# lunarring/latentblending

Measured on AMD Instinct MI355X. Metric: transition frames/sec, SDXL-Turbo 512x512 4-step 15-branch, higher is better.
Workload: dtype f16; 1 GPU; SDXL-Turbo 512x512, num_inference_steps=4, nmb_max_branches=15 (17 frames/transition), fp16, fixed_seeds=[420,421], anchors not recycled; frontier_width=16, hipgraphs=True, parallelism=single GPU

## Files before the change

include/lb_hip.h:

```cpp
#ifndef LB_HIP_H
#define LB_HIP_H

#include <stdint.h>

#ifdef __cplusplus
extern "C" {
#endif

typedef uint16_t lb_half;

int lb_version(void);
const char* lb_last_error_string(void);
int lb_device_info(int device, int* cu_count, long* lds_per_cu, char* arch, int arch_len);

int lb_slerp_pairs_f16(const void* const* p0, const void* const* p1, void* const* out,
                       const double* fracts, int npairs, long n, void* stream);
int lb_slerp_pairs_f32(const void* const* p0, const void* const* p1, void* const* out,
                       const double* fracts, int npairs, long n, void* stream);
int lb_slerp_pairs_f64(const void* const* p0, const void* const* p1, void* const* out,
                       const double* fracts, int npairs, long n, void* stream);
int lb_slerp_batched_f16(const void* p0, const void* p1, void* out, const double* fracts_dev,
                         long npairs, long n, void* stream);
int lb_slerp_strided_f16(const void* p0, long stride0, const void* p1, long stride1, void* out,
                         const double* fracts_dev, long npairs, long n, void* stream);


int lb_lerp_f16(const void* p0, const void* p1, void* out, long n, double fract, void* stream);
int lb_lerp_f32(const void* p0, const void* p1, void* out, long n, double fract, void* stream);

int lb_scale_model_input_f16(const void* x, void* out, const float* params_dev, long per_sample,
                             int batch, int dup_for_cfg, void* stream);
int lb_euler_step_f16(const void* x, const void* eps, const void* noise, void* out,
                      const float* params_dev, long per_sample, int batch, int cfg, int ancestral,
                      void* stream);
int lb_ddim_step_f16(const void* x, const void* eps, void* out, const float* params_dev, long per_sample, int batch,
                     int cfg, void* stream);

enum {
    LB_GEMM_OUT_F32 = 1,
    LB_GEMM_RES_F32 = 2,
    LB_GEMM_GEGLU = 4,
    LB_GEMM_TRANS_OUT = 8,
    LB_GEMM_SILU = 16,
    LB_GEMM_RELU = 32,
    LB_GEMM_QUICK_GELU = 128,
    LB_GEMM_GELU = 256,
    LB_GEMM_CH_STATS = 512,
    LB_GEMM_HALO_RAGGED = 1024,
    LB_GEMM_HALO_KSPLIT = 4096,
    LB_GEMM_C64 = 2048,
    LB_GEMM_LN_A = 64
};

typedef struct LbGemmParams {
    const lb_half* A;
    const lb_half* W;
    void* C;
    const float* bias;
    const void* residual;
    const lb_half* rowvec;
    float* partial;
    int M, N, K;
    int lda, ldw, ldc, ldr, ld_rowvec, rows_per_batch;
    float alpha;
    int flags;
    int conv;
    int Hin, Win, Cin, Hout, Wout, KH, KW, stride, pad;
    int ups;
    int ldx;
    int splitk;
    const void* zero_page;
    int scatter, sc_py, sc_px, reserved_;
    const float* ln_colsum;
    float ln_eps;
    int reserved2_;
    float* ch_stats;
    int ch_stats_rows;
} LbGemmParams;

int lb_gemm_f16(const LbGemmParams* params, void* stream);
long lb_gemm_workspace_bytes(int M, int N);
void lb_gemm_set_tuning(int tile, int splitk);
void lb_gemm_set_pp_auto(int on);
void lb_gemm_pp_set_group(int gm);
void lb_gemm_set_depth(int depth);
int lb_gemm_plan(const LbGemmParams* p, int* tile, int* splitk, long* blocks);
int lb_conv3x3_halo_f16(const LbGemmParams* params, void* stream);
int lb_conv3x3_narrow_f16(const LbGemmParams* params, void* stream);
void lb_conv_halo_set_persistent(int on);
void lb_conv_halo_plan(const LbGemmParams* params, int* kind, int* tile_w, long* items, long* grid);
#include "lb_hip_ksplit.h"
int lb_gemm_ch_stat_rows(const LbGemmParams* params);
int lb_upconv2x_halo_f16(const LbGemmParams* params, void* stream);
void lb_gemm_set_halo(int mode);
void lb_gemm_set_wide_store(int on);
void lb_gemm_set_t192_waves8(int on);
void lb_gemm_set_kgroups(int on);
void lb_gemm_set_lean_epilogue(int on);
void lb_gemm_set_variant(int variant, int stages);

void lb_groupnorm_set_l3_chunk(long bytes);
int lb_groupnorm_from_stats(const void* x, void* y, const float* gamma, const float* beta, const float* ch_stats,
                            void* workspace, int B, int HW, int C, int ldx, int ldy, int groups, float eps, int silu,
                            int x_is_f32, int stat_rows_per_sample, void* stream);
long lb_groupnorm_workspace_bytes(int B, int groups);
int lb_groupnorm_nhwc(const void* x, void* y, const float* gamma, const float* beta, void* workspace,
                      int B, int HW, int C, int ldx, int ldy, int groups, float eps, int silu,
                      int x_is_f32, void* stream);
int lb_groupnorm_plan(int HW, int C, int groups, int x_is_f32);
void lb_groupnorm_set_fused(int on);
int lb_layernorm_f16(const void* x, void* y, const float* gamma, const float* beta, int M, int C,
                     int ldx, int ldy, float eps, void* stream);
void lb_layernorm_set_form(int form);

typedef struct LbAttnParams {
    const lb_half* Q;
    const lb_half* K;
    const lb_half* V;
    lb_half* O;
    int B, H, Sq, Skv, Skv_valid;
    int ldq, ldk, ldv, ldo;
    float scale;
    int causal;
    const void* zero_page;
    int reserved_;
} LbAttnParams;
int lb_attn_fwd_d64(const LbAttnParams* params, void* stream);
int lb_attn_fwd_d512(const LbAttnParams* params, void* stream);
void lb_attn_set_tuning(int force);
int lb_softmax_rows_f16(void* x, int M, int N, int ld, float scale, void* stream);

int lb_sinusoid_f16(const float* vals_dev, int rows, int per_row, int val_stride, int dim, void* out,
                    int ld_out, int col_off, void* stream);
int lb_copy_cols_f16(const void* src, void* dst, long rows, int cols, int ld_src, int ld_dst,
                     int dst_off, void* stream);
int lb_cast_f16_to_f32(const void* x, void* y, long n, void* stream);
int lb_cast_f32_to_f16(const void* x, void* y, long n, float mul, void* stream);
int lb_nchw_to_nhwc_f16(const void* x, void* y, int B, int C, int HW, int ld, float mul, void* stream);
int lb_nhwc_to_nchw_f16(const void* x, void* y, int B, int C, int HW, int ld, void* stream);
int lb_postprocess_u8(const void* x, void* out_u8, long pixels, int ld, int x_is_f32, void* stream);
int lb_lpips_prep_u8(const void* img_u8, void* out_f16, long pixels, void* stream);
int lb_maxpool3s2_nhwc_f16(const void* x, void* y, int N, int H, int W, int C, void* stream);
int lb_lpips_tap(const void* const* feats_a, const void* const* feats_b, const float* lin, float* acc,
                 float* workspace, int npairs, int HW, int C, void* stream);
int lb_fill_f32(void* x, long n, float v, void* stream);
int lb_embed_tokens_f16(const int* ids_dev, const void* tok_emb, const void* pos_emb, void* out, int rows, int seq, int C,
                        int vocab, void* stream);
int lb_gather_rows_f16(const void* src, const int* rows_idx_dev, void* out, int n, int C, int ld_src, void* stream);
int lb_frames_lerp_u8(const void* frames, const int* left_dev, const double* w_dev, void* out, long n_out,
                      long frame_bytes, void* stream);
int lb_copy_d2d(void* dst, const void* src, long bytes, void* stream);

int lb_jpeg_dct_quant_u8(const void* frames_u8, const void* qtables_u16, void* coef_i16, int n, int H, int W, int subsampling,
                         void* stream);
long lb_jpeg_coefficient_count(int n, int H, int W, int subsampling);
int lb_jpeg_entropy(const void* coef_i16, void* workspace, void* out, long out_capacity, void* frame_bytes_i32, int n, int H, int W,
                    int subsampling, void* stream);
long lb_jpeg_workspace_bytes(int n, int H, int W, int subsampling);

int lb_resample_u8(const void* src, void* tmp, void* dst, int n, int Hin, int Win, int Hout, int Wout,
                   const int* start_x, const int* count_x, const int* coef_x, int kmax_x,
                   const int* start_y, const int* count_y, const int* coef_y, int kmax_y, void* stream);

void* lb_program_create(void);
void lb_program_destroy(void* prog);
int lb_program_begin_record(void* prog);
int lb_program_end_record(void* prog);
int lb_program_recording(void);
int lb_program_num_ops(void* prog);
const char* lb_program_op_name(void* prog, int i);
int lb_program_run(void* prog, void* stream);
int lb_program_run_range(void* prog, int begin, int end, void* stream);
int lb_program_instantiate(void* prog);
int lb_program_launch(void* prog, void* stream);
int lb_program_time_ops(void* prog, void* stream, float* ms_out);

#ifdef LB_STUDY_BUILD
void lb_slerp_set_study(int variant);
void lb_conv_halo_set_study(int bits);
void lb_gemm_set_policy(int disable_mask);
#endif

#ifdef __cplusplus
}
#endif
#endif
```

latentblending_amd/csrc/conv3_halo.hip:

```cpp
#include <type_traits>
#include "lb_common.h"
#include "lb_gemm.h"

typedef __attribute__((address_space(1))) const void* gptr_t;
typedef __attribute__((address_space(3))) void* lptr_t;

#ifndef LB_HALO_LEAN_ADDR
#define LB_HALO_LEAN_ADDR 1
#endif

template <int N> __device__ __forceinline__ void halo_wait_barrier() {
    asm volatile("s_waitcnt vmcnt(%0)\n\ts_barrier" ::"n"(N) : "memory");
}

template <int KS, int J> struct HaloSched {
    static constexpr int tap = KS == 3 ? J : (J < 3 ? 0 : 1);
};
template <int KS, int NR, int TAP> constexpr int halo_full_rounds_in_tap() {
    int n = 0;
    for (int j = 0; j < NR - 1; ++j) n += ((KS == 3 ? j : (j < 3 ? 0 : 1)) == TAP) ? 1 : 0;
    return n;
}

template <int BN, int TW, int KS = 3, bool RAG = false, bool KSP = false>
__global__ void __launch_bounds__(512) conv3x3_halo_kernel(const LbGemmParams p) {
    static_assert(!RAG || KS == 3, "ragged tiles exist for the 3x3 form only");
    static_assert(!KSP || (KS == 3 && !RAG), "the K-split form exists for the whole-tile 3x3 form only");
    constexpr int TH = 256 / TW;
    constexpr int NTAP = KS * KS;
    constexpr int HWP = TW + KS - 1;
    constexpr int HR = (TH + KS - 1) * HWP;
    constexpr int HRG = (HR + 7) / 8;
    constexpr int HRP = HRG * 8;
    constexpr int NR = (HRG + 7) / 8;
    constexpr int EXTRA = HRG - 8 * (NR - 1);
    constexpr int WI = BN * 8 / 512;
    constexpr int TM = 4, TN = BN / 32;
    static_assert(NR == (KS == 3 ? 6 : 5), "halo rounds: 6 for the 3x3 form, 5 for the 2x2 form");
    static_assert(EXTRA >= 1 && EXTRA <= 8, "the last halo round is a partial one");
    static_assert(WI == 2, "the vmcnt schedule assumes two weight loads per thread and step");
    extern __shared__ __attribute__((aligned(16))) f16 lds[];
    f16* const halo0 = lds;
    f16* const wring = lds + 2 * HRP * 64;

    const int tid = threadIdx.x, lane = tid & 63;
    const int wave = LB_HALO_LEAN_ADDR ? __builtin_amdgcn_readfirstlane(tid >> 6) : tid >> 6;
    const int wave_m = wave >> 1, wave_n = wave & 1;
    const int g = lane >> 4, l16 = lane & 15;

    const int n_blocks = (p.N + BN - 1) / BN;
    const int tiles_x = RAG ? (p.Win + TW - 1) / TW : p.Win / TW, tiles_y = RAG ? (p.Hin + TH - 1) / TH : p.Hin / TH;
    const int n_items = (p.M / (p.Hin * p.Win)) * tiles_x * tiles_y * (KS == 2 ? 4 : 1) * n_blocks;
    const int G = gridDim.x;
    int bid = blockIdx.x;
    {
        const int q = G / 8, r = G % 8, xcd = bid % 8, idx = bid / 8;
        bid = (xcd < r ? xcd * (q + 1) : r * (q + 1) + (xcd - r) * q) + idx;
    }
    const int n_tiles = KSP ? n_items / n_blocks : 0;
    const long n_units = KSP ? (long)n_items * (p.Cin / 64) : 0;
    const long u_lo = KSP ? (long)bid * n_units / G : 0, u_hi = KSP ? (long)(bid + 1) * n_units / G : 0;
    if constexpr (KSP)
        if (u_lo >= u_hi) return;
    const int first_item = KSP ? (int)(u_lo / (p.Cin / 64)) : bid;
    const int block_n = KSP ? first_item / n_tiles : bid % n_blocks;
    const int par_x = KS == 2 ? (bid / n_blocks) & 1 : 0;
    const int par_y = KS == 2 ? ((bid / n_blocks) >> 1) & 1 : 0;
    int n0 = block_n * BN;
    const int org_y = KS == 3 ? 1 : 1 - par_y, org_x = KS == 3 ? 1 : 1 - par_x;
    const lb_half* Wp = p.W + (KS == 2 ? (long)(par_y * 2 + par_x) * p.N * p.ldw : 0);
    const int nchunks = p.Cin / 64;
    const lb_half* zero = reinterpret_cast<const lb_half*>(p.zero_page);

    struct TileAt { int b, y0, x0; };
    auto tile_of = [&](int item) {
        int tile = KSP ? item % n_tiles : item / n_blocks;
        if (KS == 2) tile >>= 2;
        TileAt t;
        t.x0 = (tile % tiles_x) * TW;
        tile /= tiles_x;
        t.y0 = (tile % tiles_y) * TH;
        t.b = tile / tiles_y;
        return t;
    };

    const int r8 = lane >> 3;
    const int cl = (lane & 7) ^ r8;
    long h_off[NR];
    auto set_halo_offsets = [&](const TileAt& t, bool exists) {
#pragma unroll
        for (int j = 0; j < NR; ++j) {
            const int gidx = j * 8 + wave;
            const int row = gidx * 8 + r8;
            const int hy = row / HWP, hx = row - hy * HWP;
            const int y = t.y0 + hy - org_y, x = t.x0 + hx - org_x;
            const bool ok = exists && (j < NR - 1 || wave < EXTRA) && row < HR && y >= 0 && y < p.Hin && x >= 0 && x < p.Win;
            h_off[j] = ok ? ((long)(t.b * p.Hin + y) * p.Win + x) * p.ldx + cl * 8 : -1;
        }
    };
    long w_off[WI], w_offn[WI];
    unsigned w_off32[WI], w_off32n[WI];
    auto set_w_offsets = [&](int col_base, long (&o64)[WI], unsigned (&o32)[WI]) {
#pragma unroll
        for (int i = 0; i < WI; ++i) {
            const int n = col_base + (tid >> 3) + i * 64;
            o64[i] = n < p.N ? (long)n * p.ldw + cl * 8 : -1;
            o32[i] = (unsigned)(((long)(n < p.N ? n : p.N - 1) * p.ldw + cl * 8) * 2);
        }
    };
    set_w_offsets(n0, w_off, w_off32);
    if constexpr (KSP) set_w_offsets(n0, w_offn, w_off32n);

#ifdef LB_STUDY_BUILD
    const int study = p.reserved_;
#else
    constexpr int study = 0;
#endif
    auto issue_halo = [&](int j, int src_chunk, int buf) {
        const lb_half* src = h_off[j] >= 0 && !(study & 2) ? p.A + h_off[j] + (long)src_chunk * 64 : zero;
        const int gidx = j * 8 + wave;
        f16* dst = halo0 + buf * (HRP * 64) + gidx * 8 * 64;
        __builtin_amdgcn_global_load_lds((gptr_t)src, (lptr_t)dst, 16, 0, 0);
    };
    auto issue_weight = [&](int i, int chunk, bool exists, int tap, int slot, bool nxt_slab = false) {
        f16* dst = wring + slot * (BN * 64) + (wave * 8 + i * 64) * 64;
        if constexpr (LB_HALO_LEAN_ADDR) {
            if (!(study & 4)) {
                const char* base = reinterpret_cast<const char*>(Wp) + ((long)tap * p.Cin + (long)chunk * 64) * 2;
                const unsigned o32 = KSP && nxt_slab ? w_off32n[i] : w_off32[i];
                __builtin_amdgcn_global_load_lds((gptr_t)(base + (size_t)o32), (lptr_t)dst, 16, 0, 0);
                return;
            }
        }
        const long o64 = KSP && nxt_slab ? w_offn[i] : w_off[i];
        const bool live = o64 >= 0 && exists && !(study & 4);
        const lb_half* src = live ? Wp + o64 + (long)tap * p.Cin + (long)chunk * 64 : zero;
        __builtin_amdgcn_global_load_lds((gptr_t)src, (lptr_t)dst, 16, 0, 0);
    };

    int hbase[TM];
    int mloc[TM];
#pragma unroll
    for (int i = 0; i < TM; ++i) {
        const int m = wave_m * 64 + i * 16 + l16;
        const int py = m / TW, px = m - py * TW;
        hbase[i] = py * HWP + px;
        mloc[i] = py * p.Win + px;
    }
    f32x4 acc[TM][TN];
#pragma unroll
    for (int i = 0; i < TM; ++i)
#pragma unroll
        for (int j = 0; j < TN; ++j) acc[i][j] = (f32x4){0.f, 0.f, 0.f, 0.f};

    auto read_frags = [&](const f16* hb, const f16* wb, int shift, int s, f16x8 (&af)[TM], f16x8 (&wf)[TN]) {
        const int chunk = s * 4 + g;
        if constexpr (LB_HALO_LEAN_ADDR && TW == 32) {
            static_assert(TM == 4, "pairs (0, 1) and (2, 3)");
#pragma unroll
            for (int i = 0; i < TM; i += 2) {
                const int r = hbase[i] + shift;
                const f16* a = hb + r * 64 + ((chunk ^ (r & 7)) << 3);
                af[i] = *reinterpret_cast<const f16x8*>(a);
                af[i + 1] = *reinterpret_cast<const f16x8*>(a + 16 * 64);
            }
        } else {
#pragma unroll
            for (int i = 0; i < TM; ++i) {
                const int r = hbase[i] + shift;
                af[i] = *reinterpret_cast<const f16x8*>(hb + r * 64 + ((chunk ^ (r & 7)) << 3));
            }
        }
#pragma unroll
        for (int j = 0; j < TN; ++j) {
            const int r = j * 16 + l16;
            wf[j] = *reinterpret_cast<const f16x8*>(wb + (wave_n * (BN / 2) + r) * 64 + ((chunk ^ (r & 7)) << 3));
        }
    };
    auto mma_rows = [&](const f16x8 (&af)[TM], const f16x8 (&wf)[TN], int i_lo, int i_hi) {
#pragma unroll
        for (int i = i_lo; i < i_hi; ++i)
#pragma unroll
            for (int j = 0; j < TN; ++j)
                acc[i][j] = __builtin_amdgcn_mfma_f32_16x16x32_f16(wf[j], af[i], acc[i][j], 0, 0, 0);
    };

    int item = first_item;
    int c_lo = 0, c_end = nchunks;
    if constexpr (KSP) {
        c_lo = (int)(u_lo - (long)item * nchunks);
        c_end = (int)(u_hi - (long)item * nchunks < nchunks ? u_hi - (long)item * nchunks : nchunks);
    }
    TileAt cur = tile_of(item);
    set_halo_offsets(cur, true);
#pragma unroll
    for (int j = 0; j < NR; ++j)
        if (j < NR - 1 || wave < EXTRA) issue_halo(j, c_lo, 0);
#pragma unroll
    for (int t = 0; t < 3; ++t)
#pragma unroll
        for (int i = 0; i < WI; ++i) issue_weight(i, c_lo, true, t, t);

    auto step = [&](auto tap_c, int c, int cc, bool more) {
        constexpr int TAP = decltype(tap_c)::value;
        constexpr int P1 = (TAP + NTAP - 1) % NTAP, P2 = (TAP + NTAP - 2) % NTAP;
        constexpr int CNT = (2 + halo_full_rounds_in_tap<KS, NR, P1>()) + (2 + halo_full_rounds_in_tap<KS, NR, P2>());
        halo_wait_barrier<CNT>();
        const int slot = KS == 3 ? ((cc + TAP) & 3) : TAP;
        const f16* hb = halo0 + (cc & 1) * (HRP * 64);
        const f16* wb = wring + slot * (BN * 64);
        constexpr int KY = TAP / KS, KX = TAP % KS;
        int shift = KY * HWP + KX;
        asm volatile("" : "+v"(shift));
        const bool last = c + 1 == c_end;
        const int hc = last ? 0 : c + 1, hbuf = (cc + 1) & 1;
        constexpr int TAP3 = (TAP + 3) % NTAP;
        const bool wrap = (TAP + 3 >= NTAP) && last;
        const int c3 = wrap ? 0 : c + (TAP + 3) / NTAP;
        const bool w_exists = !wrap || more;
        const int slot3 = (slot + 3) & 3;
        f16x8 a0[TM], w0[TN], a1[TM], w1[TN];
        read_frags(hb, wb, shift, 0, a0, w0);
        if constexpr (HaloSched<KS, 0>::tap == TAP) issue_halo(0, hc, hbuf);
        if constexpr (NR > 2 && HaloSched<KS, 1>::tap == TAP) issue_halo(1, hc, hbuf);
        if constexpr (NR > 3 && HaloSched<KS, 2>::tap == TAP) issue_halo(2, hc, hbuf);
        if constexpr (NR > 4 && HaloSched<KS, 3>::tap == TAP) { if (NR - 1 > 3 || wave < EXTRA) issue_halo(3, hc, hbuf); }
        if constexpr (NR > 4 && HaloSched<KS, 4>::tap == TAP) { if (NR - 1 > 4 || wave < EXTRA) issue_halo(4, hc, hbuf); }
        if constexpr (NR > 5 && HaloSched<KS, 5>::tap == TAP) { if (wave < EXTRA) issue_halo(5, hc, hbuf); }
        __builtin_amdgcn_sched_barrier(0);
        mma_rows(a0, w0, 0, TM / 2);
        read_frags(hb, wb, shift, 1, a1, w1);
        __builtin_amdgcn_sched_barrier(0);
        issue_weight(0, c3, w_exists, TAP3, slot3, wrap);
        __builtin_amdgcn_sched_barrier(0);
        mma_rows(a0, w0, TM / 2, TM);
        __builtin_amdgcn_sched_barrier(0);
        issue_weight(1, c3, w_exists, TAP3, slot3, wrap);
        __builtin_amdgcn_sched_barrier(0);
        mma_rows(a1, w1, 0, TM);
    };

    LbGemmParams q = p;
    if constexpr (KS == 2) {
        q.scatter = 1;
        q.sc_py = par_y;
        q.sc_px = par_x;
    }

    int cc = 0;
    for (;;) {
        const int next_item = KSP ? item + 1 : item + G;
        const bool more = KSP ? (long)next_item * nchunks < u_hi : next_item < n_items;
        const TileAt nxt = tile_of(more ? next_item : item);
        const int n0_next = KSP && more ? (next_item / n_tiles) * BN : n0;
        for (int c = c_lo; c < c_end; ++c, ++cc) {
            if (c + 1 == c_end) {
                set_halo_offsets(nxt, more);
                if constexpr (KSP) set_w_offsets(n0_next, w_offn, w_off32n);
            }
            step(std::integral_constant<int, 0>{}, c, cc, more);
            step(std::integral_constant<int, 1>{}, c, cc, more);
            step(std::integral_constant<int, 2>{}, c, cc, more);
            step(std::integral_constant<int, 3>{}, c, cc, more);
            if constexpr (KS == 3) {
                step(std::integral_constant<int, 4>{}, c, cc, more);
                step(std::integral_constant<int, 5>{}, c, cc, more);
                step(std::integral_constant<int, 6>{}, c, cc, more);
                step(std::integral_constant<int, 7>{}, c, cc, more);
                step(std::integral_constant<int, 8>{}, c, cc, more);
            }
        }
        if constexpr (KSP) {
            if (c_lo != 0 || c_end != nchunks) {
                const long t0 = (long)item * nchunks;
                const int b_first = (int)(((t0 + 1) * G - 1) / n_units), b_last = (int)(((t0 + nchunks) * G - 1) / n_units);
                constexpr long SLAB = 256l * BN;
                int* const counters = reinterpret_cast<int*>(p.partial);
                float* const slabs = p.partial + (((long)n_items * 4 + 255) / 256) * 64;
                int tid_s = tid;
                asm volatile("" : "+v"(tid_s));
                typedef unsigned u32x4 __attribute__((ext_vector_type(4)));
                const __amdgpu_buffer_rsrc_t srs = __builtin_amdgcn_make_buffer_rsrc(slabs, 0, (int)(unsigned)(2l * G * SLAB * 4), 0x00020000);
                const int voff = tid_s * 16;
                const int mine = (2 * bid + (item == first_item ? 0 : 1)) * (int)(SLAB * 4);
#pragma unroll
                for (int i = 0; i < TM; ++i)
#pragma unroll
                    for (int j = 0; j < TN; ++j)
                        __builtin_amdgcn_raw_buffer_store_b128(__builtin_bit_cast(u32x4, acc[i][j]), srs, voff, mine + (i * TN + j) * 8192, 16);
                volatile int* const flag = reinterpret_cast<volatile int*>(lds + 2 * HRP * 64 + 4 * BN * 64);
                asm volatile("s_waitcnt vmcnt(0)" ::: "memory");
                __syncthreads();
                if (tid == 0) {
                    const int ticket = __hip_atomic_fetch_add(counters + item, 1, __ATOMIC_RELAXED, __HIP_MEMORY_SCOPE_AGENT);
                    const bool last_one = ticket == b_last - b_first;
                    if (last_one) __hip_atomic_store(counters + item, 0, __ATOMIC_RELAXED, __HIP_MEMORY_SCOPE_AGENT);
                    *flag = last_one ? 1 : 0;
                }
                __syncthreads();
                const bool reduce = __builtin_amdgcn_readfirstlane(*flag) != 0;
                if (!reduce) {
                    if (!more) break;
#pragma unroll
                    for (int i = 0; i < TM; ++i)
#pragma unroll
                        for (int j = 0; j < TN; ++j) acc[i][j] = (f32x4){0.f, 0.f, 0.f, 0.f};
                    item = next_item;
                    cur = nxt;
                    n0 = n0_next;
                    set_w_offsets(n0, w_off, w_off32);
                    c_lo = 0;
                    c_end = (int)(u_hi - (long)item * nchunks < nchunks ? u_hi - (long)item * nchunks : nchunks);
                    continue;
                }
#pragma unroll
                for (int i = 0; i < TM; ++i)
#pragma unroll
                    for (int j = 0; j < TN; ++j) acc[i][j] = (f32x4){0.f, 0.f, 0.f, 0.f};
                for (int b = b_first; b <= b_last; ++b) {
                    const bool first_tile_of_b = (long)b * n_units / G / nchunks == item;
                    const int src = (2 * b + (first_tile_of_b ? 0 : 1)) * (int)(SLAB * 4);
#pragma unroll
                    for (int i = 0; i < TM; ++i) {
                        f32x4 part[TN];
#pragma unroll
                        for (int j = 0; j < TN; ++j)
                            part[j] = __builtin_bit_cast(f32x4, __builtin_amdgcn_raw_buffer_load_b128(srs, voff, src + (i * TN + j) * 8192, 16));
#pragma unroll
                        for (int j = 0; j < TN; ++j) acc[i][j] += part[j];
                    }
                }
            }
        }
        const int mbase = (cur.b * p.Hin + cur.y0) * p.Win + cur.x0;
        int col0 = n0 + wave_n * (BN / 2) + 4 * g;
        asm volatile("" : "+v"(col0));
        bool overhang = false;
        if constexpr (RAG) overhang = cur.y0 + TH > p.Hin || cur.x0 + TW > p.Win;
        if (RAG && overhang && !(study & 1)) {
            int tid_o = tid;
            asm volatile("" : "+v"(tid_o));
            auto row_of = [&](int i) {
                const int ml = (tid_o >> 7) * 64 + i * 16 + (tid_o & 15), ly = ml / TW, lx = ml - ly * TW;
                return cur.y0 + ly < p.Hin && cur.x0 + lx < p.Win ? mbase + mloc[i] : p.M;
            };
            if (p.flags & LB_GEMM_CH_STATS) {
                const long stat_rows = (long)(n_items / n_blocks) * 4;
                float2* chst = reinterpret_cast<float2*>(p.ch_stats) + ((long)(KSP ? item % n_tiles : item / n_blocks) * 4 + wave_m);
                lb_gemm_tile_epilogue_rows_ln<TM, TN, false, false, true, true>(q, acc, row_of, col0, 0, (const LbLnRows<TM>*)nullptr, chst, stat_rows);
            } else {
                lb_gemm_tile_epilogue_rows<TM, TN, false>(q, acc, row_of, col0, 0);
            }
        } else if (!(study & 1)) {
            int tid_o = tid;
            asm volatile("" : "+v"(tid_o));
            auto out_rel = [&](int i) {
                if constexpr (KS == 3) return mloc[i];
                const int ml = (tid_o >> 7) * 64 + i * 16 + (tid_o & 15), ly = ml / TW, lx = ml - ly * TW;
                return 4 * ly * p.Win + 2 * lx;
            };
            const long out_lo = KS == 3 ? (long)mbase
                                        : ((long)(cur.b * 2 * p.Hin + 2 * cur.y0 + par_y)) * (2 * p.Win) + 2 * cur.x0 + par_x;
            const int row_hi = mbase + (TH - 1) * p.Win + TW;
            const int colw = col0 - 4 * ((tid_o & 63) >> 4);
            if (p.flags & LB_GEMM_CH_STATS) {
                const long stat_rows = (long)(n_items / n_blocks) * 4;
                float2* chst = reinterpret_cast<float2*>(p.ch_stats) + ((long)(KSP ? item % n_tiles : item / n_blocks) * 4 + wave_m);
                if (!lb_gemm_tile_epilogue_lean<TM, TN, true, true>(q, acc, [&](int i) { return mbase + mloc[i]; }, mbase, row_hi, out_rel,
                                                                    out_lo, cur.b, colw, chst, stat_rows))
                    lb_gemm_tile_epilogue_rows_ln<TM, TN, false, false, true>(q, acc, [&](int i) { return mbase + mloc[i]; }, col0, 0,
                                                                              (const LbLnRows<TM>*)nullptr, chst, stat_rows);
            } else {
                if (!lb_gemm_tile_epilogue_lean<TM, TN, false, true>(q, acc, [&](int i) { return mbase + mloc[i]; }, mbase, row_hi, out_rel,
                                                                     out_lo, cur.b, colw))
                    lb_gemm_tile_epilogue_rows<TM, TN, false>(q, acc, [&](int i) { return mbase + mloc[i]; }, col0, 0);
            }
        }
        else if (acc[0][0][0] == 12345.678f) *(float*)p.C = acc[1][1][1] + acc[2][2][2] + acc[3][3][3];
        if (!more) break;
#pragma unroll
        for (int i = 0; i < TM; ++i)
#pragma unroll
            for (int j = 0; j < TN; ++j) acc[i][j] = (f32x4){0.f, 0.f, 0.f, 0.f};
        item = next_item;
        cur = nxt;
        if constexpr (KSP) {
            n0 = n0_next;
            set_w_offsets(n0, w_off, w_off32);
            c_lo = 0;
            c_end = (int)(u_hi - (long)item * nchunks < nchunks ? u_hi - (long)item * nchunks : nchunks);
        }
    }
    asm volatile("s_waitcnt vmcnt(0)" ::: "memory");
}

static int g_halo_persistent = 1;
extern "C" void lb_conv_halo_set_persistent(int on) { g_halo_persistent = on; }
#ifdef LB_STUDY_BUILD
static int g_halo_study = 0;
extern "C" void lb_conv_halo_set_study(int bits) { g_halo_study = bits; }
#endif
static int halo_num_cus() {
    static int n = 0;
    if (!n) {
        int dev = 0;
        hipDeviceProp_t prop;
        n = (hipGetDevice(&dev) == hipSuccess && hipGetDeviceProperties(&prop, dev) == hipSuccess && prop.multiProcessorCount > 0)
                ? prop.multiProcessorCount : 256;
    }
    return n;
}

static void halo_grid(const LbGemmParams& p, int tw, int ks, long& items, long& grid) {
    const int th = 256 / tw;
    const long tiles = (long)(p.M / (p.Hin * p.Win)) * ((p.Hin + th - 1) / th) * ((p.Win + tw - 1) / tw) * (ks == 2 ? 4 : 1);
    const int n_blocks = (p.N + 127) / 128;
    items = tiles * n_blocks;
    const int period = n_blocks * (ks == 2 ? 4 : 1);
    grid = items;
    if (g_halo_persistent && period <= halo_num_cus() && items > halo_num_cus())
        grid = (long)(halo_num_cus() / period) * period;
}

int lb_upconv_halo_eligible(const LbGemmParams& p);
int lb_conv3x3_halo_eligible(const LbGemmParams& p);
long lb_conv_halo_stat_rows_total(const LbGemmParams& p) {
    int tw = 0, ks = 0;
    if ((tw = lb_upconv_halo_eligible(p)) != 0) ks = 2;
    else if ((tw = lb_conv3x3_halo_eligible(p)) != 0) ks = 3;
    if (!ks) return 0;
    long items, grid;
    halo_grid(p, tw, ks, items, grid);
    return items / ((p.N + 127) / 128) * 4;
}

template <int BN, int TW, int KS = 3, bool RAG = false, bool KSP = false>
static int launch_halo(const LbGemmParams& p, hipStream_t stream, long ksp_grid = 0) {
    constexpr int TH = 256 / TW;
    constexpr int HRP = (((TH + KS - 1) * (TW + KS - 1) + 7) / 8) * 8;
    constexpr int SMEM = (2 * HRP * 64 + 4 * BN * 64) * (int)sizeof(f16) + (KSP ? 16 : 0);
    static unsigned long long seen = 0;
    LB_ONCE_PER_DEVICE(seen)
        (void)hipFuncSetAttribute(reinterpret_cast<const void*>(conv3x3_halo_kernel<BN, TW, KS, RAG, KSP>),
                                  hipFuncAttributeMaxDynamicSharedMemorySize, SMEM);
    static_assert(BN == 128, "halo_grid assumes 128-channel blocks");
    long nblk, grid;
    halo_grid(p, TW, KS, nblk, grid);
    if (KSP) grid = ksp_grid;
    LbGemmParams pk = p;
#ifdef LB_STUDY_BUILD
    pk.reserved_ = g_halo_study;
#endif
    hipLaunchKernelGGL((conv3x3_halo_kernel<BN, TW, KS, RAG, KSP>), dim3((unsigned)grid), dim3(512), SMEM, stream, pk);
    return lb_check_launch(KS == 2 ? "lb_upconv2x_halo_f16" : "lb_conv3x3_halo_f16");
}

int lb_upconv_halo_eligible(const LbGemmParams& p) {
    if (!p.conv || p.scatter != 2 || p.KH != 2 || p.KW != 2 || p.stride != 1 || p.ups) return 0;
    if (p.Hout != p.Hin || p.Wout != p.Win || p.Cin % 64 != 0 || p.K != 4 * p.Cin) return 0;
    if (p.zero_page == nullptr || (p.flags & (LB_GEMM_GEGLU | LB_GEMM_TRANS_OUT)) || p.N % 4 != 0 || p.residual != nullptr) return 0;
    if (p.M % (p.Hin * p.Win) != 0) return 0;
    if ((long)p.N * p.ldw * 2 >= (1l << 32)) return 0;
    if (p.Win % 32 == 0 && p.Hin % 8 == 0) return 32;
    if (p.Win % 16 == 0 && p.Hin % 16 == 0) return 16;
    return 0;
}

static int halo_tiles_check(const LbGemmParams& p, int tw, int ks) {
    long items, grid;
    halo_grid(p, tw, ks, items, grid);
    LB_REQUIRE(items < (1l << 30), "halo conv: too many tiles for one launch");
    return 0;
}

int lb_upconv_halo_check(const LbGemmParams& p) {
    LB_REQUIRE(!(p.flags & LB_GEMM_CH_STATS) || (p.ch_stats != nullptr && p.ch_stats_rows == lb_conv_halo_stat_rows_total(p)),
               "halo upconv: LB_GEMM_CH_STATS needs ch_stats with ch_stats_rows = B * lb_gemm_ch_stat_rows()");
    return halo_tiles_check(p, lb_upconv_halo_eligible(p), 2);
}

int lb_upconv_halo_launch(LbGemmParams p, hipStream_t stream) {
    if (p.alpha == 0.f) p.alpha = 1.f;
    p.splitk = 1;
    return lb_upconv_halo_eligible(p) == 32 ? launch_halo<128, 32, 2>(p, stream) : launch_halo<128, 16, 2>(p, stream);
}

extern int g_lb_wide_store, g_lb_lean_epilogue;
extern "C" int lb_upconv2x_halo_f16(const LbGemmParams* pp, void* stream) {
    LbGemmParams p = *pp;
    p.flags &= ~LB_GEMM_C64;
    p.reserved2_ = (g_lb_wide_store & 1) | (g_lb_lean_epilogue ? 2 : 0);
    LB_REQUIRE(p.M > 0 && p.N > 0 && p.K > 0, "lb_upconv2x_halo_f16: empty problem");
    LB_REQUIRE(lb_upconv_halo_eligible(p) != 0,
               "lb_upconv2x_halo_f16: needs scatter = 2, KH = KW = 2, stride 1, Cin % 64 == 0, W % 16 == 0, zero page, no residual");
    LB_REQUIRE(p.ldw % 8 == 0 && p.ldx % 8 == 0 && p.ldc % 4 == 0, "lb_upconv2x_halo_f16: ldw / ldx multiples of 8, ldc multiple of 4");
    if (const int rc = lb_upconv_halo_check(p)) return rc;
    LB_DISPATCH("lb_upconv2x_halo_f16", lb_upconv_halo_launch(p, s));
}

int lb_conv3x3_halo_eligible(const LbGemmParams& p) {
    if (!p.conv || p.KH != 3 || p.KW != 3 || p.stride != 1 || p.pad != 1 || p.ups || p.scatter) return 0;
    if (p.Hout != p.Hin || p.Wout != p.Win || p.Cin % 64 != 0 || p.K != 9 * p.Cin) return 0;
    if (p.zero_page == nullptr || (p.flags & LB_GEMM_GEGLU) || p.N % 4 != 0) return 0;
    if (p.M % (p.Hin * p.Win) != 0) return 0;
    if ((long)p.N * p.ldw * 2 >= (1l << 32)) return 0;
    if (p.Win % 32 == 0 && p.Hin % 8 == 0) return 32;
    if (p.Win % 16 == 0 && p.Hin % 16 == 0) return 16;
    if (!(p.flags & LB_GEMM_HALO_RAGGED)) return 0;
    const long t32 = (long)((p.Win + 31) / 32) * ((p.Hin + 7) / 8), t16 = (long)((p.Win + 15) / 16) * ((p.Hin + 15) / 16);
    return t16 < t32 ? 16 : 32;
}
static bool halo3_ragged(const LbGemmParams& p, int tw) { return p.Win % tw != 0 || p.Hin % (256 / tw) != 0; }

static int g_halo_ksplit_mode = 1, g_halo_ksplit_grid = 0;
extern "C" void lb_conv_halo_set_ksplit(int mode, int grid) {
    g_halo_ksplit_mode = mode < 0 ? 1 : mode;
    g_halo_ksplit_grid = grid > 0 ? grid : 0;
}
static constexpr long HALO_KSPLIT_FIXUP_STEPS = 20;
static constexpr long HALO_KSPLIT_MARGIN_PCT = 5;
static void halo_ksplit_plan(const LbGemmParams& p, long& units, long& grid, int& split) {
    units = grid = 0;
    split = 0;
    if (!(p.flags & LB_GEMM_HALO_KSPLIT) || (p.flags & LB_GEMM_C64) || g_halo_ksplit_mode == 0) return;
    const int tw = lb_conv3x3_halo_eligible(p);
    if (!tw || halo3_ragged(p, tw) || p.Cin < 128) return;
    long items, ugrid;
    halo_grid(p, tw, 3, items, ugrid);
    const long nchunks = p.Cin / 64;
    if (items * nchunks >= (1l << 31)) return;
    units = items * nchunks;
    grid = g_halo_ksplit_grid > 0 ? g_halo_ksplit_grid : halo_num_cus();
    if (grid > units) grid = units;
    if (2 * grid * 256l * 128 * 4 >= (1l << 31)) {
        units = grid = 0;
        return;
    }
    if (g_halo_ksplit_mode >= 2) {
        split = 1;
        return;
    }
    const long unsplit_steps = (items + ugrid - 1) / ugrid * 9 * nchunks;
    const long split_steps = (units + grid - 1) / grid * 9 + HALO_KSPLIT_FIXUP_STEPS;
    split = split_steps * (100 + HALO_KSPLIT_MARGIN_PCT) <= unsplit_steps * 100 ? 1 : 0;
}
static long halo_ksplit_counter_bytes(long items) { return (items * 4 + 255) / 256 * 256; }
extern "C" void lb_conv_halo_ksplit_plan(const LbGemmParams* pp, long* units, long* grid, int* split) {
    long u = 0, g = 0;
    int s = 0;
    if (pp != nullptr && pp->M > 0 && pp->Hin > 0 && pp->Win > 0) halo_ksplit_plan(*pp, u, g, s);
    if (units) *units = u;
    if (grid) *grid = g;
    if (split) *split = s;
}
extern "C" long lb_conv_halo_ksplit_workspace_bytes(const LbGemmParams* pp) {
    long u = 0, g = 0;
    int s = 0;
    if (pp != nullptr && pp->M > 0 && pp->Hin > 0 && pp->Win > 0) halo_ksplit_plan(*pp, u, g, s);
    if (!s) return 0;
    return halo_ksplit_counter_bytes(u / (pp->Cin / 64)) + 2 * g * 256l * 128 * (long)sizeof(float);
}

long lb_conv3x3_halo_blocks(const LbGemmParams& p) {
    long tiles = (long)p.M / 256;
    if (const int tw = (p.flags & LB_GEMM_HALO_RAGGED) ? lb_conv3x3_halo_eligible(p) : 0)
        tiles = (long)(p.M / (p.Hin * p.Win)) * ((p.Hin + 256 / tw - 1) / (256 / tw)) * ((p.Win + tw - 1) / tw);
    return tiles * ((p.N + 127) / 128);
}

int lb_conv3x3_halo_check(const LbGemmParams& p) {
    LB_REQUIRE(!(p.flags & LB_GEMM_CH_STATS) || (p.ch_stats != nullptr && !(p.flags & LB_GEMM_TRANS_OUT)),
               "halo conv: LB_GEMM_CH_STATS needs ch_stats and a row-major output");
    LB_REQUIRE(!(p.flags & LB_GEMM_CH_STATS) || p.ch_stats_rows == lb_conv_halo_stat_rows_total(p),
               "halo conv: ch_stats_rows must be B * lb_gemm_ch_stat_rows() (the row blocks this launch writes per channel)");
    {
        long units, grid;
        int split;
        halo_ksplit_plan(p, units, grid, split);
        LB_REQUIRE(!split || p.partial != nullptr,
                   "halo conv: LB_GEMM_HALO_KSPLIT needs partial = a zeroed workspace of lb_conv_halo_ksplit_workspace_bytes()");
    }
    return halo_tiles_check(p, lb_conv3x3_halo_eligible(p), 3);
}

int lb_conv3x3_halo_launch(LbGemmParams p, hipStream_t stream) {
    if (p.alpha == 0.f) p.alpha = 1.f;
    p.splitk = 1;
    const int tw = lb_conv3x3_halo_eligible(p);
    if (halo3_ragged(p, tw)) return tw == 32 ? launch_halo<128, 32, 3, true>(p, stream) : launch_halo<128, 16, 3, true>(p, stream);
    long units, grid;
    int split;
    halo_ksplit_plan(p, units, grid, split);
    if (split && p.partial != nullptr)
        return tw == 32 ? launch_halo<128, 32, 3, false, true>(p, stream, grid) : launch_halo<128, 16, 3, false, true>(p, stream, grid);
    return tw == 32 ? launch_halo<128, 32>(p, stream) : launch_halo<128, 16>(p, stream);
}

extern "C" int lb_conv3x3_halo_f16(const LbGemmParams* pp, void* stream) {
    LbGemmParams p = *pp;
    p.flags &= ~LB_GEMM_C64;
    p.reserved2_ = (g_lb_wide_store & 1) | (g_lb_lean_epilogue ? 2 : 0);
    LB_REQUIRE(p.M > 0 && p.N > 0 && p.K > 0, "lb_conv3x3_halo_f16: empty problem");
    LB_REQUIRE(lb_conv3x3_halo_eligible(p) != 0,
               "lb_conv3x3_halo_f16: needs a 3x3 / stride 1 / pad 1 conv, Cin % 64 == 0, W % 16 == 0 (or LB_GEMM_HALO_RAGGED), zero page");
    LB_REQUIRE(p.ldw % 8 == 0 && p.ldx % 8 == 0 && (p.ldc % 4 == 0 || (p.flags & LB_GEMM_TRANS_OUT)),
               "lb_conv3x3_halo_f16: ldw / ldx multiples of 8, ldc multiple of 4");
    if (const int rc = lb_conv3x3_halo_check(p)) return rc;
    LB_DISPATCH("lb_conv3x3_halo_f16", lb_conv3x3_halo_launch(p, s));
}

extern "C" void lb_conv_halo_plan(const LbGemmParams* pp, int* kind, int* tile_w, long* items, long* grid) {
    LbGemmParams p = *pp;
    int k = 0, tw = 0;
    if (p.flags & LB_GEMM_C64) tw = 0;
    else if ((tw = lb_upconv_halo_eligible(p)) != 0) k = 2;
    else if ((tw = lb_conv3x3_halo_eligible(p)) != 0) k = 3;
    long it = 0, gr = 0;
    if (k) halo_grid(p, tw, k, it, gr);
    if (kind) *kind = k;
    if (tile_w) *tile_w = tw;
    if (items) *items = it;
    if (grid) *grid = gr;
}
```

latentblending_amd/csrc/conv3_narrow.hip:

```cpp
#include "lb_common.h"
#include "lb_gemm.h"

typedef __attribute__((address_space(1))) const void* gptr_t;
typedef __attribute__((address_space(3))) void* lptr_t;

#define NARROW_T 16
#define NARROW_HW (NARROW_T + 2)
#define NARROW_HR (NARROW_HW * NARROW_HW)
#define NARROW_HRG ((NARROW_HR + 7) / 8)
#define NARROW_LDS (NARROW_HRG * 8 * 64)

__global__ void __launch_bounds__(256, 2) conv3x3_narrow_kernel(const LbGemmParams p) {
    __shared__ __attribute__((aligned(16))) f16 halo[NARROW_LDS];
    const int tid = threadIdx.x, lane = tid & 63, wave = tid >> 6;
    const int g = lane >> 4, l16 = lane & 15;
    const int tiles_x = p.Win / NARROW_T, tiles_y = p.Hin / NARROW_T;
    int tile = blockIdx.x;
    const int x0 = (tile % tiles_x) * NARROW_T;
    tile /= tiles_x;
    const int y0 = (tile % tiles_y) * NARROW_T;
    const int b = tile / tiles_y;
    const lb_half* zero = reinterpret_cast<const lb_half*>(p.zero_page);
    const int nchunks = p.Cin / 64;

    constexpr int NR = (NARROW_HRG + 3) / 4;
    const int r8 = lane >> 3, cl = (lane & 7) ^ r8;
    int h_off[NR];
#pragma unroll
    for (int j = 0; j < NR; ++j) {
        const int gidx = j * 4 + wave;
        const int row = gidx * 8 + r8;
        const int hy = row / NARROW_HW, hx = row - hy * NARROW_HW;
        const int y = y0 + hy - 1, x = x0 + hx - 1;
        const bool ok = gidx < NARROW_HRG && row < NARROW_HR && y >= 0 && y < p.Hin && x >= 0 && x < p.Win;
        h_off[j] = ok ? (int)((((long)(b * p.Hin + y) * p.Win + x) * p.ldx >> 3) + cl) : -1;
    }
    const bool n_ok = l16 < p.N;
    const lb_half* wrow = p.W + (long)(n_ok ? l16 : 0) * p.ldw + g * 8;

    f32x4 acc[4];
#pragma unroll
    for (int i = 0; i < 4; ++i) acc[i] = (f32x4){0.f, 0.f, 0.f, 0.f};
    int hbase[4];
#pragma unroll
    for (int i = 0; i < 4; ++i) hbase[i] = (wave * 4 + i) * NARROW_HW + l16;

    const f16x8 zero8 = {0, 0, 0, 0, 0, 0, 0, 0};
    for (int c = 0; c < nchunks; ++c) {
        if (c) __syncthreads();
#pragma unroll
        for (int j = 0; j < NR; ++j) {
            const int gidx = j * 4 + wave;
            if (gidx < NARROW_HRG) {
                const lb_half* src = h_off[j] >= 0 ? p.A + (long)h_off[j] * 8 + (long)c * 64 : zero;
                __builtin_amdgcn_global_load_lds((gptr_t)src, (lptr_t)(halo + gidx * 8 * 64), 16, 0, 0);
            }
        }
        f16x8 wf[9][2];
#pragma unroll
        for (int tap = 0; tap < 9; ++tap)
#pragma unroll
            for (int s = 0; s < 2; ++s)
                wf[tap][s] = n_ok ? *reinterpret_cast<const f16x8*>(wrow + (long)tap * p.Cin + c * 64 + s * 32) : zero8;
        asm volatile("s_waitcnt vmcnt(0)" ::: "memory");
        __syncthreads();
#pragma unroll
        for (int tap = 0; tap < 9; ++tap) {
            const int shift = (tap / 3) * NARROW_HW + tap % 3;
#pragma unroll
            for (int s = 0; s < 2; ++s) {
                const int chunk = s * 4 + g;
#pragma unroll
                for (int i = 0; i < 4; ++i) {
                    const int r = hbase[i] + shift;
                    const f16x8 af = *reinterpret_cast<const f16x8*>(halo + r * 64 + ((chunk ^ (r & 7)) << 3));
                    acc[i] = __builtin_amdgcn_mfma_f32_16x16x32_f16(wf[tap][s], af, acc[i], 0, 0, 0);
                }
            }
        }
    }
    const int n = 4 * g;
    if (n < p.N) {
        f32x4 bias = {0.f, 0.f, 0.f, 0.f};
        if (p.bias) bias = *reinterpret_cast<const f32x4*>(p.bias + n);
#pragma unroll
        for (int i = 0; i < 4; ++i) {
            const long m = ((long)(b * p.Hin + y0 + wave * 4 + i)) * p.Win + x0 + l16;
            float o[4];
#pragma unroll
            for (int r = 0; r < 4; ++r) o[r] = acc[i][r] * p.alpha + bias[r];
            if (p.flags & LB_GEMM_OUT_F32)
                *reinterpret_cast<f32x4*>((float*)p.C + m * p.ldc + n) = (f32x4){o[0], o[1], o[2], o[3]};
            else
                *reinterpret_cast<f16x4*>((f16*)p.C + m * p.ldc + n) = (f16x4){(f16)o[0], (f16)o[1], (f16)o[2], (f16)o[3]};
        }
    }
}

int lb_conv3x3_narrow_eligible(const LbGemmParams& p) {
    if (!p.conv || p.KH != 3 || p.KW != 3 || p.stride != 1 || p.pad != 1 || p.ups || p.scatter) return 0;
    if (p.Hout != p.Hin || p.Wout != p.Win || p.Cin % 64 != 0 || p.K != 9 * p.Cin) return 0;
    if (p.N > 16 || p.N % 4 != 0 || p.zero_page == nullptr) return 0;
    if (p.flags & ~(LB_GEMM_OUT_F32 | LB_GEMM_HALO_KSPLIT)) return 0;
    if (p.residual != nullptr || p.rowvec != nullptr) return 0;
    if (p.Win % NARROW_T != 0 || p.Hin % NARROW_T != 0 || p.M % (p.Hin * p.Win) != 0) return 0;
    if ((long)p.M * p.ldx >= (1l << 34)) return 0;
    return 1;
}

static long narrow_tiles(const LbGemmParams& p) {
    return (long)(p.M / (p.Hin * p.Win)) * (p.Hin / NARROW_T) * (p.Win / NARROW_T);
}

int lb_conv3x3_narrow_check(const LbGemmParams& p) {
    LB_REQUIRE(narrow_tiles(p) < (1l << 31), "conv3x3 narrow: too many tiles for one launch");
    return 0;
}

int lb_conv3x3_narrow_launch(LbGemmParams p, hipStream_t stream) {
    if (p.alpha == 0.f) p.alpha = 1.f;
    const long tiles = narrow_tiles(p);
    hipLaunchKernelGGL(conv3x3_narrow_kernel, dim3((unsigned)tiles), dim3(256), 0, stream, p);
    return lb_check_launch("lb_conv3x3_narrow_f16");
}

extern "C" int lb_conv3x3_narrow_f16(const LbGemmParams* pp, void* stream) {
    LbGemmParams p = *pp;
    p.flags &= ~LB_GEMM_C64;
    LB_REQUIRE(p.M > 0 && p.N > 0 && p.K > 0, "lb_conv3x3_narrow_f16: empty problem");
    LB_REQUIRE(lb_conv3x3_narrow_eligible(p) != 0,
               "lb_conv3x3_narrow_f16: needs a 3x3 / stride 1 / pad 1 conv, N <= 16, Cin % 64 == 0, H and W multiples of 16, bias-only epilogue");
    LB_REQUIRE(p.ldw % 8 == 0 && p.ldx % 8 == 0 && p.ldc % 4 == 0, "lb_conv3x3_narrow_f16: ldw / ldx multiples of 8, ldc multiple of 4");
    if (const int rc = lb_conv3x3_narrow_check(p)) return rc;
    LB_DISPATCH("lb_conv3x3_narrow_f16", lb_conv3x3_narrow_launch(p, s));
}
```

latentblending_amd/csrc/gemm.hip:

```cpp
#include "lb_common.h"
#include "lb_gemm.h"

#define BK 64

template <int N> struct Int { static constexpr int value = N; };

template <int BM, int BN, bool CONV, bool GEGLU, int D>
__global__ void __launch_bounds__(256) gemm_f16_kernel(const LbGemmParams p) {
    constexpr int AI = BM * 8 / 256;
    constexpr int WI = BN * 8 / 256;
    constexpr int TM = BM / 32;
    constexpr int TN = BN / 32;
    __shared__ __attribute__((aligned(16))) f16 lds[2 * (BM + BN) * BK];
    f16* const As = lds;
    f16* const Ws = lds + 2 * BM * BK;

    const int tid = threadIdx.x;
    const int lane = tid & 63, wave = tid >> 6;
    const int wave_m = wave >> 1, wave_n = wave & 1;
    const int g = lane >> 4, l16 = lane & 15;

    const int n_blocks = GEGLU ? (p.N / 2 + BN / 2 - 1) / (BN / 2) : (p.N + BN - 1) / BN;
    int bid = blockIdx.x;
    {
// ... 297 lines not shown
    switch (depth) {
        case 1: launch_variant<BM, BN, 1>(p, grid, stream); break;
        case 2: launch_variant<BM, BN, 2>(p, grid, stream); break;
        case 3: launch_variant<BM, BN, 3>(p, grid, stream); break;
        default: launch_variant<BM, BN, 4>(p, grid, stream); break;
    }
}

static int default_depth(const LbGemmParams& p, int tile) {
    if (tile == 1) return p.conv ? 1 : 3;
    if (tile == 2) return 3;
    return 4;
}

static int gemm_launch_impl(LbGemmParams p, int tile, int depth, int variant, int stages, dim3 grid,
                            hipStream_t stream) {
    if (tile == 9) {
        lb_gemm_launch_pp(p, grid, stream);
    } else if (variant == 1 && p.zero_page != nullptr) {
        lb_gemm_launch_glds(p, tile, stages, grid, stream);
    } else {
        if (depth <= 0) depth = default_depth(p, tile);
        if (tile == 1) launch_depth<128, 128>(p, depth, grid, stream);
        else if (tile == 2) launch_depth<128, 64>(p, depth, grid, stream);
        else launch_depth<64, 64>(p, depth, grid, stream);
    }
    int rc = lb_check_launch("lb_gemm_f16");
    if (rc) return rc;
    if (p.splitk > 1) {
        const long quads = (long)p.M * (p.N / 4);
        long gsz = (quads + 255) / 256;
        if (gsz > 2048) gsz = 2048;
        hipLaunchKernelGGL(gemm_splitk_reduce_kernel, dim3((unsigned)gsz), dim3(256), 0, stream, p);
        rc = lb_check_launch("lb_gemm_f16(split-K reduce)");
    }
    return rc;
}

static void gemm_plan(const LbGemmParams& p, int& tile_out, int& splitk_out, long& nblk_out) {
    const bool geglu = (p.flags & LB_GEMM_GEGLU) != 0;
    const int n_eff = geglu ? p.N / 2 : p.N;

    auto blocks = [&](int bm, int bn) {
        const int bn_eff = geglu ? bn / 2 : bn;
        return (long)((p.M + bm - 1) / bm) * ((n_eff + bn_eff - 1) / bn_eff);
    };
    int tile = g_force_tile;
    if (tile == 9 && !lb_gemm_pp_eligible(p)) tile = 0;
    if (!tile) {
        const long b128 = blocks(128, 128);
        tile = b128 >= 700 ? 1 : (b128 >= 224 ? (g_variant == 1 ? 2 : 1) : 3);
        if (n_eff <= 64) tile = 3;
        if (g_variant == 1 && p.zero_page != nullptr) {
            const long b256 = blocks(256, 128);
            const int unit = geglu ? 64 : 128;
            const int n_pad = (n_eff + unit - 1) / unit * unit;
            const bool n_fits = (long)n_pad * 10 <= (long)n_eff * 11;
            const bool allow4 = !(g_policy_off & 1) && !(p.conv && (g_policy_off & 16));
            const bool allow5 = !(g_policy_off & 2) && !(p.conv ? (g_policy_off & 4) : (g_policy_off & 8));
            if (allow4 && n_fits && (b256 >= 1024 || (!p.conv && b256 >= 160 && p.K >= 1024))) tile = 4;
            const long b512 = blocks(256, 256);
            const long rounds4 = (b256 + 255) / 256, rounds5 = (b512 + 255) / 256;
            if (allow5 && (b512 >= 1024 || (b512 >= 160 && p.K >= 1024)) && rounds5 * 174 < rounds4 * 100) tile = 5;
            if ((g_policy_off & 32) && !geglu && !p.conv && (tile == 4 || tile == 5) && n_fits) {
                const long b192 = blocks(192, 128);
                const long rounds7 = (b192 + 255) / 256;
                const long cur = tile == 5 ? rounds5 * 174 : rounds4 * 100;
                if (b192 >= 160 && rounds7 * 78 < cur) tile = g_t192_waves8 ? 10 : 7;
            }
            if (!(g_policy_off & 64) && !geglu && !p.conv && tile == 4 && n_fits && b256 < 224) {
                const long b192 = blocks(192, 128);
                if (b192 <= 256 && b192 * 10 >= b256 * 13) tile = g_t192_waves8 ? 10 : 7;
            }
        }
    }
    if (!g_force_tile && g_t192_waves8 && geglu && !p.conv && (tile == 1 || tile == 2 || tile == 4) && p.M <= 2048 && g_variant == 1 &&
        p.zero_page != nullptr && blocks(192, 128) <= 448 && p.K >= 512)
        tile = 10;
    if (tile >= 4 && tile != 9 && (g_variant != 1 || p.zero_page == nullptr)) tile = 1;
    if (!g_force_tile && g_pp_auto && lb_gemm_pp_eligible(p)) {
        const int bn_out = geglu ? 128 : 256;
        const long n_pad = (long)((n_eff + bn_out - 1) / bn_out) * bn_out;
        const long b9 = blocks(256, 256);
        if (b9 >= 192 && (p.K >= 1024 || b9 >= 1024) && n_pad * 4 <= (long)n_eff * 5) tile = 9;
    }
    if (!g_force_tile && tile == 3 && !geglu && p.partial != nullptr && (p.K + BK - 1) / BK >= 64) {
        const long b64 = blocks(64, 64);
        if (b64 > 256 && b64 <= 640 && blocks(128, 64) <= 256) tile = 2;
    }
    const int bm = (tile == 7 || tile == 10) ? 192 : (tile == 11 ? 64 : (tile >= 4 ? 256 : (tile == 3 ? 64 : 128)));
    const int bn = (tile == 5 || tile == 9) ? 256 : ((tile == 1 || tile == 4 || tile == 7 || tile == 10) ? 128 : 64);
    const long nblk = blocks(bm, bn);
    int splitk = 1;
    if (!geglu && p.partial != nullptr && !(p.flags & LB_GEMM_LN_A)) {
        const int k_tiles = (p.K + BK - 1) / BK;
        if (g_force_splitk) splitk = g_force_splitk;
        else if (nblk <= 256) {
            splitk = (int)((640 + nblk - 1) / nblk);
            const int max_by_k = k_tiles / 16 > 0 ? k_tiles / 16 : 1;
            if (splitk > max_by_k) splitk = max_by_k;
            if (splitk > 16) splitk = 16;
        }
        if (splitk > k_tiles) splitk = k_tiles;
        if (splitk < 1) splitk = 1;
        if (tile == 9 && !g_force_splitk) splitk = 1;
        if (tile >= 4 && tile != 11 && !g_force_splitk) splitk = 1;
    }
    if (!g_force_tile && g_kgroups && tile == 3 && splitk == 1 && !p.conv && g_variant == 1 && p.zero_page != nullptr && nblk <= 200 &&
        (p.K + BK - 1) / BK >= 8)
        tile = 11;
    tile_out = tile;
    splitk_out = splitk;
    nblk_out = nblk;
}

extern "C" int lb_gemm_plan(const LbGemmParams* pp, int* tile, int* splitk, long* blocks) {
    LB_REQUIRE(pp != nullptr && pp->M > 0 && pp->N > 0 && pp->K > 0, "lb_gemm_plan: empty problem");
    int t = 0, sk = 1;
    long nb = 0;
    if (pp->flags & LB_GEMM_C64) {
        if (const int rc = lb_conv3_c64_check(*pp)) return rc;
        long items = 0;
        t = 12;
        lb_conv3_c64_grid(*pp, items, nb);
    }
    else if (g_halo != 0 && !g_force_tile && lb_conv3x3_narrow_eligible(*pp)) { t = 8; nb = (long)pp->M / 256; }
    else if (use_halo(*pp)) { t = 6; nb = lb_conv3x3_halo_blocks(*pp); }
    else if (pp->flags & LB_GEMM_HALO_KSPLIT) {
        LbGemmParams q = *pp;
        q.flags &= ~LB_GEMM_HALO_KSPLIT;
        q.partial = nullptr;
        gemm_plan(q, t, sk, nb);
    }
    else gemm_plan(*pp, t, sk, nb);
    if (tile) *tile = t;
    if (splitk) *splitk = sk;
    if (blocks) *blocks = nb;
    return 0;
}

long lb_conv_halo_stat_rows_total(const LbGemmParams& p);
extern "C" int lb_gemm_ch_stat_rows(const LbGemmParams* pp) {
    if (pp == nullptr || !pp->conv || pp->M <= 0 || pp->Hout <= 0 || pp->Wout <= 0) return 0;
    if (pp->flags & LB_GEMM_C64) return 0;
    const LbGemmParams& p = *pp;
    bool halo;
    if (p.scatter == 2) halo = lb_upconv_halo_eligible(p) != 0;
    else halo = !(g_halo != 0 && !g_force_tile && lb_conv3x3_narrow_eligible(p)) && use_halo(p);
    if (!halo) return 0;
    const long samples = (long)p.M / ((long)p.Hout * p.Wout);
    return samples > 0 ? (int)(lb_conv_halo_stat_rows_total(p) / samples) : 0;
}

extern "C" int lb_gemm_f16(const LbGemmParams* pp, void* stream) {
    LbGemmParams p = *pp;
    const bool geglu = (p.flags & LB_GEMM_GEGLU) != 0;
    LB_REQUIRE(p.M > 0 && p.N > 0 && p.K > 0, "lb_gemm_f16: empty problem");
    LB_REQUIRE(p.K % 8 == 0 && p.ldw % 8 == 0, "lb_gemm_f16: K and ldw must be multiples of 8");
    LB_REQUIRE(p.N % 4 == 0 && (geglu ? p.N % 8 == 0 : true), "lb_gemm_f16: N must be a multiple of 4");
    LB_REQUIRE(p.ldc % 4 == 0 || (p.flags & LB_GEMM_TRANS_OUT), "lb_gemm_f16: ldc must be a multiple of 4");
    if (p.conv) {
        LB_REQUIRE(p.Cin % 8 == 0 && p.ldx % 8 == 0, "lb_gemm_f16: conv Cin/ldx must be multiples of 8");
        LB_REQUIRE(p.K == p.KH * p.KW * p.Cin, "lb_gemm_f16: conv K != KH*KW*Cin");
        LB_REQUIRE(p.M % (p.Hout * p.Wout) == 0, "lb_gemm_f16: conv M must be B*Hout*Wout");
        if (p.scatter)
            LB_REQUIRE(p.KH == 2 && p.KW == 2 && p.stride == 1 && p.ups == 0 && p.Hout == p.Hin && p.Wout == p.Win &&
                           !(p.flags & (LB_GEMM_TRANS_OUT | LB_GEMM_GEGLU)) && p.residual == nullptr,
                       "lb_gemm_f16: sub-pixel conv needs KH=KW=2, stride 1, Hout=Hin, no residual");
    } else {
        LB_REQUIRE(p.lda % 8 == 0, "lb_gemm_f16: lda must be a multiple of 8");
    }
    if (p.flags & LB_GEMM_LN_A) {
        LB_REQUIRE(!p.conv && p.ln_colsum != nullptr && p.zero_page != nullptr && g_variant == 1,
                   "lb_gemm_f16: LB_GEMM_LN_A needs a plain / GEGLU GEMM of the direct-to-LDS family with ln_colsum");
        LB_REQUIRE(p.lda >= p.K && !(p.flags & LB_GEMM_TRANS_OUT), "lb_gemm_f16: LB_GEMM_LN_A normalises whole rows of A");
    }
    if (p.alpha == 0.f) p.alpha = 1.f;
    p.reserved2_ = (g_lb_wide_store & 1) | (g_lb_lean_epilogue ? 2 : 0);
    if (p.flags & LB_GEMM_C64) {
        if (const int rc = lb_conv3_c64_check(p)) return rc;
        LB_DISPATCH("conv3x3_c64", lb_conv3_c64_launch(p, s));
    }
    if (p.scatter == 2) {
        LB_REQUIRE(lb_upconv_halo_eligible(p) != 0, "lb_gemm_f16: scatter = 2 needs Cin % 64 == 0, W % 16 == 0, stacked [4][N][K] weights");
        if (const int rc = lb_upconv_halo_check(p)) return rc;
        LB_DISPATCH("lb_upconv2x_halo_f16", lb_upconv_halo_launch(p, s));
    }
    if (g_halo != 0 && !g_force_tile && lb_conv3x3_narrow_eligible(p)) {
        if (const int rc = lb_conv3x3_narrow_check(p)) return rc;
        LB_DISPATCH("lb_conv3x3_narrow_f16", lb_conv3x3_narrow_launch(p, s));
    }
    if (use_halo(p)) {
        if (const int rc = lb_conv3x3_halo_check(p)) return rc;
        LB_DISPATCH("lb_conv3x3_halo_f16", lb_conv3x3_halo_launch(p, s));
    }
    if (p.flags & LB_GEMM_HALO_KSPLIT) {
        p.flags &= ~LB_GEMM_HALO_KSPLIT;
        p.partial = nullptr;
    }
    LB_REQUIRE(!(p.flags & LB_GEMM_CH_STATS), "lb_gemm_f16: LB_GEMM_CH_STATS is implemented by the halo-tile conv kernels only "
                                              "(check lb_gemm_plan == 6 / lb_conv_halo_plan before asking for it)");
    int tile = 0, splitk = 1;
    long nblk = 0;
    gemm_plan(p, tile, splitk, nblk);
    p.splitk = splitk;
    const int depth = g_depth, variant = g_variant;
    int stages = g_stages;
    if (variant == 1) {
        lb_gemm_glds_init();
        if (stages == 0)
            stages = (tile == 3 || tile == 4 || tile == 7 || tile == 10 || tile == 11) ? 3 : 2;
    }
    const dim3 grid((unsigned)nblk, 1, (unsigned)splitk);
    LB_DISPATCH("lb_gemm_f16", gemm_launch_impl(p, tile, depth, variant, stages, grid, s));
}
```

latentblending_amd/csrc/lb_common.h:

```cpp
#pragma once
#include <hip/hip_runtime.h>
#include <hip/hip_fp16.h>
#include <stdint.h>

#define LB_WAVE 64

typedef _Float16 f16;
typedef f16 f16x4 __attribute__((ext_vector_type(4)));
typedef f16 f16x8 __attribute__((ext_vector_type(8)));
typedef float f32x4 __attribute__((ext_vector_type(4)));

extern "C" const char* lb_last_error_string(void);
void lb_set_error(const char* what, hipError_t e);

#ifdef __cplusplus
#include <functional>
#include <mutex>
bool lb_recording();
void lb_record(const char* name, std::function<int(hipStream_t)> fn);
#define LB_DISPATCH(NAME, CALL)                                                   \
    do {                                                                          \
        if (lb_recording()) {                                                     \
            lb_record(NAME, [=](hipStream_t s) -> int { return CALL; });          \
            return 0;                                                             \
        }                                                                         \
        hipStream_t s = (hipStream_t)stream;                                      \
        return CALL;                                                              \
    } while (0)
#define LB_DISPATCH_STMT(NAME, STMT) \
    LB_DISPATCH(NAME, ([&]() -> int { STMT; return lb_check_launch(NAME); })())
#endif

static inline int lb_check_launch(const char* what) {
    hipError_t e = hipGetLastError();
    if (e != hipSuccess) lb_set_error(what, e);
    return (int)e;
}

struct LbFirstCallOnDevice {
    std::unique_lock<std::mutex> lock;
    bool first;
    explicit LbFirstCallOnDevice(unsigned long long& seen) : lock(mutex()) {
        int dev = 0;
        (void)hipGetDevice(&dev);
        const unsigned long long bit = 1ull << (dev & 63);
        first = (seen & bit) == 0;
        seen |= bit;
    }
    static std::mutex& mutex() {
        static std::mutex m;
        return m;
    }
};
#define LB_ONCE_PER_DEVICE(seen) if (LbFirstCallOnDevice lb_once_guard_{seen}; lb_once_guard_.first)

#define LB_REQUIRE(cond, what)                                   \
    do {                                                         \
        if (!(cond)) {                                           \
            lb_set_error(what, hipErrorInvalidValue);            \
            return (int)hipErrorInvalidValue;                    \
        }                                                        \
    } while (0)

__device__ __forceinline__ float lb_wave_sum(float v) {
#pragma unroll
    for (int off = 32; off > 0; off >>= 1) v += __shfl_xor(v, off, LB_WAVE);
    return v;
}

__device__ __forceinline__ float lb_wave_sum_dpp(float v) {
    {
        const unsigned u = __float_as_uint(v);
        const auto r = __builtin_amdgcn_permlane32_swap(u, u, false, false);
        v = __uint_as_float(r[0]) + __uint_as_float(r[1]);
    }
    {
        const unsigned u = __float_as_uint(v);
        const auto r = __builtin_amdgcn_permlane16_swap(u, u, false, false);
        v = __uint_as_float(r[0]) + __uint_as_float(r[1]);
    }
    v += __uint_as_float(__builtin_amdgcn_update_dpp(0u, __float_as_uint(v), 0x128, 0xf, 0xf, false));
    v += __uint_as_float(__builtin_amdgcn_update_dpp(0u, __float_as_uint(v), 0x124, 0xf, 0xf, false));
    v += __uint_as_float(__builtin_amdgcn_update_dpp(0u, __float_as_uint(v), 0x4e, 0xf, 0xf, false));
    v += __uint_as_float(__builtin_amdgcn_update_dpp(0u, __float_as_uint(v), 0xb1, 0xf, 0xf, false));
    return v;
}

__device__ __forceinline__ double lb_wave_sum(double v) {
#pragma unroll
    for (int off = 32; off > 0; off >>= 1) v += __shfl_xor(v, off, LB_WAVE);
    return v;
}

__device__ __forceinline__ float lb_wave_max(float v) {
#pragma unroll
    for (int off = 32; off > 0; off >>= 1) v = fmaxf(v, __shfl_xor(v, off, LB_WAVE));
    return v;
}

__device__ __forceinline__ f16 lb_f64_to_f16(double x) {
    const float f = (float)x;
    const double r = x - (double)f;
    unsigned u = __float_as_uint(f);
    const bool finite_nz = (u & 0x7fffffffu) - 1u < 0x7f7fffffu;
    if (finite_nz && r != 0.0) {
        if ((r < 0.0) != (f < 0.0f)) u -= 1u;
        u |= 1u;
    }
    return (f16)__uint_as_float(u);
}

__device__ __forceinline__ float lb_silu(float x) {
    return x * __builtin_amdgcn_rcpf(1.0f + __builtin_amdgcn_exp2f(x * -1.44269504088896340736f));
}

__device__ __forceinline__ float lb_erf(float x) {
    const float ax = __builtin_fabsf(x);
    const float t = __builtin_amdgcn_rcpf(__builtin_fmaf(0.3275911f, ax, 1.0f));
    float p = __builtin_fmaf(1.061405429f, t, -1.453152027f);
    p = __builtin_fmaf(p, t, 1.421413741f);
    p = __builtin_fmaf(p, t, -0.284496736f);
    p = __builtin_fmaf(p, t, 0.254829592f);
    const float e = __builtin_amdgcn_exp2f(ax * ax * -1.44269504088896340736f);
    const float r = __builtin_fmaf(-p * t, e, 1.0f);
    return __builtin_copysignf(r, x);
}

__device__ __forceinline__ float lb_quick_gelu(float x) {
    return x * __builtin_amdgcn_rcpf(1.0f + __builtin_amdgcn_exp2f(x * (-1.702f * 1.44269504088896340736f)));
}

__device__ __forceinline__ float lb_gelu_erf(float x) {
    return 0.5f * x * (1.0f + lb_erf(x * 0.70710678118654752440f));
}
```

latentblending_amd/csrc/norm.hip:

```cpp
#include "lb_common.h"

#define GN_MAX_GROUPS 32
#define GN_MAX_CHUNKS 256

template <typename T> struct Vec8 { typedef T type __attribute__((ext_vector_type(8))); };

template <typename T>
__device__ __forceinline__ void load8(const T* p, float (&v)[8]);
template <>
__device__ __forceinline__ void load8<f16>(const f16* p, float (&v)[8]) {
    const f16x8 x = *reinterpret_cast<const f16x8*>(p);
#pragma unroll
    for (int j = 0; j < 8; ++j) v[j] = (float)x[j];
}
template <>
__device__ __forceinline__ void load8<float>(const float* p, float (&v)[8]) {
    const f32x4 a = *reinterpret_cast<const f32x4*>(p);
    const f32x4 b = *reinterpret_cast<const f32x4*>(p + 4);
#pragma unroll
    for (int j = 0; j < 4; ++j) { v[j] = a[j]; v[4 + j] = b[j]; }
}

template <typename T, int VPT>
__global__ void __launch_bounds__(256) gn_partial_kernel(const T* __restrict__ x,
                                                         double* __restrict__ partial, int HW, int C,
                                                         int ldx, int groups, int chunk_px) {
    extern __shared__ __attribute__((aligned(16))) float gn_lds[];
    const int vecs = C >> 3;
    const int rows = VPT == 1 ? 256 / vecs : 1;
    const int tid = threadIdx.x;
    const int chunk = blockIdx.x, b = blockIdx.y, nchunk = gridDim.x;
    const int px_begin = chunk * chunk_px;
    int px_end = px_begin + chunk_px;
    if (px_end > HW) px_end = HW;
    const int r = VPT == 1 ? tid / vecs : 0;
    const bool active = VPT == 1 ? tid < rows * vecs : true;
    float* lsum = gn_lds;
    float* lsq = gn_lds + rows * C;

#pragma unroll
    for (int j = 0; j < VPT; ++j) {
        const int v = VPT == 1 ? tid % vecs : tid + j * 256;
        float s[8] = {0, 0, 0, 0, 0, 0, 0, 0}, q[8] = {0, 0, 0, 0, 0, 0, 0, 0};
        if (active && v < vecs) {
            const T* base = x + ((long)b * HW) * ldx + v * 8;
            int px = px_begin + r;
            for (; px + 3 * rows < px_end; px += 4 * rows) {
                float v0[8], v1[8], v2[8], v3[8];
                load8<T>(base + (long)px * ldx, v0);
                load8<T>(base + (long)(px + rows) * ldx, v1);
                load8<T>(base + (long)(px + 2 * rows) * ldx, v2);
                load8<T>(base + (long)(px + 3 * rows) * ldx, v3);
#pragma unroll
                for (int e = 0; e < 8; ++e) {
                    s[e] += v0[e]; q[e] += v0[e] * v0[e];
                    s[e] += v1[e]; q[e] += v1[e] * v1[e];
                    s[e] += v2[e]; q[e] += v2[e] * v2[e];
                    s[e] += v3[e]; q[e] += v3[e] * v3[e];
                }
            }
            for (; px < px_end; px += rows) {
                float val[8];
                load8<T>(base + (long)px * ldx, val);
#pragma unroll
                for (int e = 0; e < 8; ++e) { s[e] += val[e]; q[e] += val[e] * val[e]; }
            }
#pragma unroll
            for (int e = 0; e < 8; ++e) {
                lsum[r * C + v * 8 + e] = s[e];
                lsq[r * C + v * 8 + e] = q[e];
            }
        }
    }
    __syncthreads();
    if (tid < groups) {
        const int cpg = C / groups;
        double s = 0, q = 0;
        for (int rr = 0; rr < rows; ++rr)
            for (int c = tid * cpg; c < (tid + 1) * cpg; ++c) {
                s += (double)lsum[rr * C + c];
                q += (double)lsq[rr * C + c];
            }
        double* out = partial + (((long)b * nchunk + chunk) * groups + tid) * 2;
        out[0] = s;
        out[1] = q;
    }
}

template <typename T>
__global__ void __launch_bounds__(256) gn_apply_kernel(const T* __restrict__ x,
                                                       const double* __restrict__ partial,
                                                       const float* __restrict__ gamma,
                                                       const float* __restrict__ beta,
                                                       f16* __restrict__ y, int HW, int C, int ldx,
                                                       int ldy, int groups, int nchunk, float eps,
                                                       int silu, int chunk_px) {
    __shared__ float mean_s[GN_MAX_GROUPS], rstd_s[GN_MAX_GROUPS];
    __shared__ double fold_s[8][GN_MAX_GROUPS], fold_q[8][GN_MAX_GROUPS];
    const int b = blockIdx.y, tid = threadIdx.x;
    const int cpg = C / groups;
    {
        const int grp = tid & 31, sub = tid >> 5;
        if (grp < groups) {
            double s = 0, q = 0;
            for (int c = sub; c < nchunk; c += 8) {
                const double* pp = partial + (((long)b * nchunk + c) * groups + grp) * 2;
                s += pp[0];
                q += pp[1];
            }
            fold_s[sub][grp] = s;
            fold_q[sub][grp] = q;
        }
    }
    __syncthreads();
    if (tid < groups) {
        double s = 0, q = 0;
#pragma unroll
        for (int sub = 0; sub < 8; ++sub) { s += fold_s[sub][tid]; q += fold_q[sub][tid]; }
        const double cnt = (double)HW * cpg;
        const double mean = s / cnt;
        double var = q / cnt - mean * mean;
        if (var < 0) var = 0;
        mean_s[tid] = (float)mean;
        rstd_s[tid] = (float)(1.0 / sqrt(var + (double)eps));
    }
    __syncthreads();
    const int vecs = C >> 3;
    const int rows = vecs <= 256 ? 256 / vecs : 1;
    const int px_begin = blockIdx.x * chunk_px;
    int px_end = px_begin + chunk_px;
    if (px_end > HW) px_end = HW;
    const int r = vecs <= 256 ? tid / vecs : 0;
    if (vecs <= 256 && tid >= rows * vecs) return;
    for (int v = vecs <= 256 ? tid % vecs : tid; v < vecs; v += 256) {
        const int c0 = v * 8;
        float sc[8], sh[8];
#pragma unroll
        for (int e = 0; e < 8; ++e) {
            const int grp = (c0 + e) / cpg;
            const float a = rstd_s[grp] * gamma[c0 + e];
            sc[e] = a;
            sh[e] = beta[c0 + e] - mean_s[grp] * a;
        }
        const T* src = x + ((long)b * HW) * ldx + c0;
        f16* dst = y + ((long)b * HW) * ldy + c0;
        auto finish = [&](const float (&val)[8], int px) {
            f16x8 o;
#pragma unroll
            for (int e = 0; e < 8; ++e) {
                float t = __builtin_fmaf(val[e], sc[e], sh[e]);
                if (silu) t = lb_silu(t);
                o[e] = (f16)t;
            }
            *reinterpret_cast<f16x8*>(dst + (long)px * ldy) = o;
        };
        int px = px_begin + r;
        for (; px + 3 * rows < px_end; px += 4 * rows) {
            float v0[8], v1[8], v2[8], v3[8];
            load8<T>(src + (long)px * ldx, v0);
            load8<T>(src + (long)(px + rows) * ldx, v1);
            load8<T>(src + (long)(px + 2 * rows) * ldx, v2);
            load8<T>(src + (long)(px + 3 * rows) * ldx, v3);
            finish(v0, px);
            finish(v1, px + rows);
            finish(v2, px + 2 * rows);
            finish(v3, px + 3 * rows);
        }
        for (; px < px_end; px += rows) {
            float val[8];
            load8<T>(src + (long)px * ldx, val);
            finish(val, px);
        }
        if (vecs <= 256) break;
    }
}

extern "C" long lb_groupnorm_workspace_bytes(int B, int groups) {
    return (long)B * GN_MAX_CHUNKS * groups * 2 * (long)sizeof(double);
}

static int groupnorm_impl(const void* x, void* y, const float* gamma, const float* beta,
                          void* workspace, int B, int HW, int C, int ldx, int ldy, int groups,
                          float eps, int silu, int x_is_f32, hipStream_t stream) {
    LB_REQUIRE(C % 8 == 0 && ldx % 8 == 0 && ldy % 8 == 0, "lb_groupnorm_nhwc: C/ld multiple of 8");
    LB_REQUIRE(groups > 0 && groups <= GN_MAX_GROUPS && C % groups == 0, "lb_groupnorm_nhwc: groups");
    const int vecs = C / 8;
    int want = (2048 + B - 1) / B;
    if (want > GN_MAX_CHUNKS) want = GN_MAX_CHUNKS;
    if (want < 16) want = 16;
    int chunk_px = (HW + want - 1) / want;
    if (chunk_px < 32) chunk_px = 32;
    const int nchunk = (HW + chunk_px - 1) / chunk_px;
    double* partial = (double*)workspace;
    const int vpt = vecs <= 256 ? 1 : 2;
    const int rows = vpt == 1 ? 256 / vecs : 1;
    const size_t lds = (size_t)2 * rows * C * sizeof(float);
    dim3 grid1(nchunk, B);
#define GN_PART(T, V) hipLaunchKernelGGL((gn_partial_kernel<T, V>), grid1, dim3(256), lds, stream, \
                                         (const T*)x, partial, HW, C, ldx, groups, chunk_px)
    if (x_is_f32) { if (vpt == 1) GN_PART(float, 1); else GN_PART(float, 2); }
    else          { if (vpt == 1) GN_PART(f16, 1);   else GN_PART(f16, 2); }
#undef GN_PART
    int rc = lb_check_launch("lb_groupnorm_nhwc(partial)");
    if (rc) return rc;
    int want2 = (4096 + B - 1) / B;
    int apx = (HW + want2 - 1) / want2;
    const int min_px = 4 * rows;
    if (apx < min_px) apx = min_px;
    const int achunks = (HW + apx - 1) / apx;
    dim3 grid2((unsigned)achunks, B);
    if (x_is_f32)
        hipLaunchKernelGGL((gn_apply_kernel<float>), grid2, dim3(256), 0, stream, (const float*)x,
                           partial, gamma, beta, (f16*)y, HW, C, ldx, ldy, groups, nchunk, eps, silu, apx);
    else
        hipLaunchKernelGGL((gn_apply_kernel<f16>), grid2, dim3(256), 0, stream, (const f16*)x,
                           partial, gamma, beta, (f16*)y, HW, C, ldx, ldy, groups, nchunk, eps, silu, apx);
    return lb_check_launch("lb_groupnorm_nhwc(apply)");
}

static long g_gn_l3_bytes = 0;
extern "C" void lb_groupnorm_set_l3_chunk(long bytes) { g_gn_l3_bytes = bytes; }

static int groupnorm_chunked(const void* x, void* y, const float* gamma, const float* beta, void* workspace,
                             int B, int HW, int C, int ldx, int ldy, int groups, float eps, int silu,
                             int x_is_f32, hipStream_t stream) {
    const long elt = x_is_f32 ? 4 : 2;
    const long sample_bytes = (long)HW * ldx * elt;
    long nb = B;
    if (g_gn_l3_bytes > 0 && sample_bytes * B > g_gn_l3_bytes) {
        nb = g_gn_l3_bytes / sample_bytes;
        if (nb < 1) nb = 1;
    }
    for (long b0 = 0; b0 < B; b0 += nb) {
        const int bn = (int)(B - b0 < nb ? B - b0 : nb);
        const int rc = groupnorm_impl((const char*)x + b0 * sample_bytes, (f16*)y + b0 * (long)HW * ldy, gamma, beta,
                                      (double*)workspace + b0 * GN_MAX_CHUNKS * groups * 2, bn, HW, C, ldx, ldy,
                                      groups, eps, silu, x_is_f32, stream);
        if (rc) return rc;
    }
    return 0;
}

template <int NPX>
__global__ void __launch_bounds__(256) gn_fused_kernel(const f16* __restrict__ x, const float* __restrict__ gamma,
                                                       const float* __restrict__ beta, f16* __restrict__ y, int HW, int C, int ldx,
                                                       int ldy, int cpg, int SL, float eps, int silu) {
    extern __shared__ __attribute__((aligned(16))) double gnf_lds[];
    const int vps = SL >> 3, rows = 256 / vps;
    const int tid = threadIdx.x, b = blockIdx.y, c_slab = blockIdx.x * SL;
    const bool active = tid < rows * vps;
    const int r = active ? tid / vps : 0, slot = active ? tid - r * vps : 0;
    const int c0 = c_slab + slot * 8;
    const f16* src = x + ((long)b * HW) * ldx + c0;
    f16x8 raw[NPX];
#pragma unroll
    for (int k = 0; k < NPX; ++k) {
        const int px = min(r + k * rows, HW - 1);
        raw[k] = *reinterpret_cast<const f16x8*>(src + (long)px * ldx);
    }
    __builtin_amdgcn_sched_barrier(0);
    const f32x4 g0 = *reinterpret_cast<const f32x4*>(gamma + c0), g1 = *reinterpret_cast<const f32x4*>(gamma + c0 + 4);
    const f32x4 b0 = *reinterpret_cast<const f32x4*>(beta + c0), b1 = *reinterpret_cast<const f32x4*>(beta + c0 + 4);
    __builtin_amdgcn_sched_barrier(0);
    float sm[8] = {0, 0, 0, 0, 0, 0, 0, 0}, sq[8] = {0, 0, 0, 0, 0, 0, 0, 0};
#pragma unroll
    for (int k = 0; k < NPX; ++k) {
        const bool ok = active && r + k * rows < HW;
#pragma unroll
        for (int e = 0; e < 8; ++e) {
            const float v = ok ? (float)raw[k][e] : 0.f;
            sm[e] += v;
            sq[e] += v * v;
        }
    }
    double* lsum = gnf_lds;
    double* lsq = gnf_lds + rows * SL;
    if (active) {
#pragma unroll
        for (int e = 0; e < 8; ++e) {
            lsum[r * SL + slot * 8 + e] = (double)sm[e];
            lsq[r * SL + slot * 8 + e] = (double)sq[e];
        }
    }
    __syncthreads();
    double* csum = gnf_lds + 2 * rows * SL;
    if (tid < 2 * SL) {
        const double* col = (tid < SL ? lsum : lsq) + (tid < SL ? tid : tid - SL);
        double a = 0;
        for (int rr = 0; rr < rows; ++rr) a += col[rr * SL];
        csum[tid] = a;
    }
    __syncthreads();
    const int ngrp = SL / cpg;
    float* stat = reinterpret_cast<float*>(csum + 2 * SL);
    if (tid < ngrp) {
        double a = 0, q = 0;
        for (int c = tid * cpg; c < (tid + 1) * cpg; ++c) { a += csum[c]; q += csum[SL + c]; }
        const double cnt = (double)HW * cpg;
        const double mean = a / cnt;
        double var = q / cnt - mean * mean;
        if (var < 0) var = 0;
        stat[2 * tid] = (float)mean;
        stat[2 * tid + 1] = (float)(1.0 / sqrt(var + (double)eps));
    }
    __syncthreads();
    if (!active) return;
    float sc[8], sh[8];
#pragma unroll
    for (int e = 0; e < 8; ++e) {
        const int grp = (slot * 8 + e) / cpg;
        const float gam = e < 4 ? g0[e & 3] : g1[e & 3], bet = e < 4 ? b0[e & 3] : b1[e & 3];
        const float a = stat[2 * grp + 1] * gam;
        sc[e] = a;
        sh[e] = bet - stat[2 * grp] * a;
    }
    f16* dst = y + ((long)b * HW) * ldy + c0;
#pragma unroll
    for (int k = 0; k < NPX; ++k) {
        const int px = r + k * rows;
        f16x8 o;
#pragma unroll
        for (int e = 0; e < 8; ++e) {
            float t = __builtin_fmaf((float)raw[k][e], sc[e], sh[e]);
            if (silu) t = lb_silu(t);
            o[e] = (f16)t;
        }
        if (px < HW) *reinterpret_cast<f16x8*>(dst + (long)px * ldy) = o;
    }
}

static int g_gn_fused = 1;
extern "C" void lb_groupnorm_set_fused(int on) { g_gn_fused = on; }

static int gn_fused_plan(int HW, int C, int groups, int x_is_f32, int* npx_out) {
    if (!g_gn_fused || x_is_f32) return 0;
    const int cpg = C / groups;
    int SL = cpg;
    while (SL % 8) SL += cpg;
    if (SL > 120 || C % SL) return 0;
    const int rows = 256 / (SL / 8);
    const int npx = (HW + rows - 1) / rows;
    if (npx > 24) return 0;
    *npx_out = npx <= 8 ? 8 : (npx <= 16 ? 16 : 24);
    return SL;
}

extern "C" int lb_groupnorm_plan(int HW, int C, int groups, int x_is_f32) {
    int npx = 0;
    return (groups > 0 && C > 0 && C % groups == 0 && C % 8 == 0 && gn_fused_plan(HW, C, groups, x_is_f32, &npx)) ? 1 : 0;
}

static int groupnorm_fused(const void* x, void* y, const float* gamma, const float* beta, int B, int HW, int C, int ldx, int ldy,
                           int groups, float eps, int silu, int SL, int npx, hipStream_t s) {
    const int cpg = C / groups, rows = 256 / (SL / 8);
    const size_t smem = (size_t)(2 * rows * SL + 2 * SL) * sizeof(double) + 16 * sizeof(float);
    const dim3 grid(C / SL, B);
#define LB_GNF_ARGS (const f16*)x, gamma, beta, (f16*)y, HW, C, ldx, ldy, cpg, SL, eps, silu
    if (npx == 8) hipLaunchKernelGGL(gn_fused_kernel<8>, grid, dim3(256), smem, s, LB_GNF_ARGS);
    else if (npx == 16) hipLaunchKernelGGL(gn_fused_kernel<16>, grid, dim3(256), smem, s, LB_GNF_ARGS);
    else hipLaunchKernelGGL(gn_fused_kernel<24>, grid, dim3(256), smem, s, LB_GNF_ARGS);
#undef LB_GNF_ARGS
    return lb_check_launch("lb_groupnorm_nhwc(fused)");
}

extern "C" int lb_groupnorm_nhwc(const void* x, void* y, const float* gamma, const float* beta,
                                 void* workspace, int B, int HW, int C, int ldx, int ldy, int groups,
                                 float eps, int silu, int x_is_f32, void* stream) {
    LB_REQUIRE(B > 0 && HW > 0 && C > 0, "lb_groupnorm_nhwc: sizes");
    LB_REQUIRE(C % 8 == 0 && ldx % 8 == 0 && ldy % 8 == 0, "lb_groupnorm_nhwc: C/ld multiple of 8");
    LB_REQUIRE(groups > 0 && groups <= GN_MAX_GROUPS && C % groups == 0, "lb_groupnorm_nhwc: groups");
    LB_REQUIRE(C <= 4096, "lb_groupnorm_nhwc: C <= 4096");
    int npx = 0;
    const int SL = gn_fused_plan(HW, C, groups, x_is_f32, &npx);
    if (SL) LB_DISPATCH("lb_groupnorm_nhwc", groupnorm_fused(x, y, gamma, beta, B, HW, C, ldx, ldy, groups, eps, silu, SL, npx, s));
    LB_DISPATCH("lb_groupnorm_nhwc", groupnorm_chunked(x, y, gamma, beta, workspace, B, HW, C, ldx, ldy, groups,
                                                       eps, silu, x_is_f32, s));
}

__global__ void __launch_bounds__(256) gn_fold_stats_kernel(const float2* __restrict__ ch_stats, double* __restrict__ partial,
                                                            int C, int groups, int rows_per_sample, long total_rows) {
    __shared__ double red_s[256], red_q[256];
    const int grp = blockIdx.x, b = blockIdx.y, tid = threadIdx.x;
    const int cpg = C / groups;
    double s = 0, q = 0;
    for (int c = 0; c < cpg; ++c) {
        const float2* run = ch_stats + (long)(grp * cpg + c) * total_rows + (long)b * rows_per_sample;
        for (int r = tid; r < rows_per_sample; r += 256) {
            const float2 v = run[r];
            s += (double)v.x;
            q += (double)v.y;
        }
    }
    red_s[tid] = s;
    red_q[tid] = q;
    __syncthreads();
    for (int w = 128; w > 0; w >>= 1) {
        if (tid < w) { red_s[tid] += red_s[tid + w]; red_q[tid] += red_q[tid + w]; }
        __syncthreads();
    }
    if (tid == 0) {
        double* out = partial + ((long)b * groups + grp) * 2;
        out[0] = red_s[0];
        out[1] = red_q[0];
    }
}

static int groupnorm_from_stats_impl(const void* x, void* y, const float* gamma, const float* beta, const float* ch_stats,
                                     void* workspace, int B, int HW, int C, int ldx, int ldy, int groups, float eps, int silu,
                                     int x_is_f32, int rows_per_sample, hipStream_t stream) {
    double* partial = (double*)workspace;
    hipLaunchKernelGGL(gn_fold_stats_kernel, dim3(groups, B), dim3(256), 0, stream, (const float2*)ch_stats, partial, C, groups,
                       rows_per_sample, (long)B * rows_per_sample);
    int rc = lb_check_launch("lb_groupnorm_from_stats(fold)");
    if (rc) return rc;
    const int vecs = C / 8;
    const int rows = vecs <= 256 ? 256 / vecs : 1;
    int want2 = (4096 + B - 1) / B;
    int apx = (HW + want2 - 1) / want2;
    const int min_px = 4 * rows;
    if (apx < min_px) apx = min_px;
    const int achunks = (HW + apx - 1) / apx;
    dim3 grid2((unsigned)achunks, B);
    if (x_is_f32)
        hipLaunchKernelGGL((gn_apply_kernel<float>), grid2, dim3(256), 0, stream, (const float*)x,
                           partial, gamma, beta, (f16*)y, HW, C, ldx, ldy, groups, 1, eps, silu, apx);
    else
        hipLaunchKernelGGL((gn_apply_kernel<f16>), grid2, dim3(256), 0, stream, (const f16*)x,
                           partial, gamma, beta, (f16*)y, HW, C, ldx, ldy, groups, 1, eps, silu, apx);
    return lb_check_launch("lb_groupnorm_from_stats(apply)");
}

extern "C" int lb_groupnorm_from_stats(const void* x, void* y, const float* gamma, const float* beta, const float* ch_stats,
                                       void* workspace, int B, int HW, int C, int ldx, int ldy, int groups, float eps,
                                       int silu, int x_is_f32, int stat_rows_per_sample, void* stream) {
    LB_REQUIRE(B > 0 && HW > 0 && C > 0 && stat_rows_per_sample > 0 && ch_stats != nullptr, "lb_groupnorm_from_stats: sizes");
    LB_REQUIRE(C % 8 == 0 && ldx % 8 == 0 && ldy % 8 == 0 && C <= 4096, "lb_groupnorm_from_stats: C/ld multiple of 8, C <= 4096");
    LB_REQUIRE(groups > 0 && groups <= GN_MAX_GROUPS && C % groups == 0, "lb_groupnorm_from_stats: groups");
    LB_DISPATCH("lb_groupnorm_from_stats", groupnorm_from_stats_impl(x, y, gamma, beta, ch_stats, workspace, B, HW, C, ldx, ldy,
                                                                     groups, eps, silu, x_is_f32, stat_rows_per_sample, s));
}

__global__ void __launch_bounds__(256) layernorm_kernel(const f16* __restrict__ x,
                                                        const float* __restrict__ gamma,
                                                        const float* __restrict__ beta,
                                                        f16* __restrict__ y, int M, int C, int ldx,
                                                        int ldy, float eps) {
    const int row = blockIdx.x * 4 + (threadIdx.x >> 6);
    const int lane = threadIdx.x & 63;
    if (row >= M) return;
    const int vecs = C >> 3;
    float val[4][8];
    float s = 0.f;
#pragma unroll
    for (int j = 0; j < 4; ++j) {
        const int v = lane + j * 64;
        if (v < vecs) {
            load8<f16>(x + (long)row * ldx + v * 8, val[j]);
#pragma unroll
            for (int e = 0; e < 8; ++e) s += val[j][e];
        }
    }
    const float mean = lb_wave_sum(s) / (float)C;
    float q = 0.f;
#pragma unroll
    for (int j = 0; j < 4; ++j) {
        const int v = lane + j * 64;
        if (v < vecs) {
#pragma unroll
            for (int e = 0; e < 8; ++e) { const float d = val[j][e] - mean; q += d * d; }
        }
    }
    const float rstd = rsqrtf(lb_wave_sum(q) / (float)C + eps);
#pragma unroll
    for (int j = 0; j < 4; ++j) {
        const int v = lane + j * 64;
        if (v < vecs) {
            const int c0 = v * 8;
            f16x8 o;
#pragma unroll
            for (int e = 0; e < 8; ++e)
                o[e] = (f16)((val[j][e] - mean) * rstd * gamma[c0 + e] + beta[c0 + e]);
            *reinterpret_cast<f16x8*>(y + (long)row * ldy + c0) = o;
        }
    }
}

template <int NV>
__global__ void __launch_bounds__(256) layernorm_rows_kernel(const f16* __restrict__ x, const float* __restrict__ gamma,
                                                             const float* __restrict__ beta, f16* __restrict__ y, int M, int C,
                                                             int ldx, int ldy, float eps) {
    const int row = blockIdx.x * 4 + (threadIdx.x >> 6);
    const int lane = threadIdx.x & 63;
    if (row >= M) return;
    const int vecs = C >> 3;
    f16x8 raw[NV];
    f32x4 gm[NV][2], bt[NV][2];
    bool ok[NV];
    int vc[NV];
#pragma unroll
    for (int j = 0; j < NV; ++j) {
        const int v = lane + j * 64;
        ok[j] = v < vecs;
        vc[j] = ok[j] ? v : 0;
        raw[j] = *reinterpret_cast<const f16x8*>(x + (long)row * ldx + vc[j] * 8);
    }
    __builtin_amdgcn_sched_barrier(0);
#pragma unroll
    for (int j = 0; j < NV; ++j) {
        gm[j][0] = *reinterpret_cast<const f32x4*>(gamma + vc[j] * 8);
        gm[j][1] = *reinterpret_cast<const f32x4*>(gamma + vc[j] * 8 + 4);
        bt[j][0] = *reinterpret_cast<const f32x4*>(beta + vc[j] * 8);
        bt[j][1] = *reinterpret_cast<const f32x4*>(beta + vc[j] * 8 + 4);
    }
    __builtin_amdgcn_sched_barrier(0);
    float val[NV][8];
    float s = 0.f;
#pragma unroll
    for (int j = 0; j < NV; ++j)
#pragma unroll
        for (int e = 0; e < 8; ++e) {
            val[j][e] = (float)raw[j][e];
            s += ok[j] ? val[j][e] : 0.f;
        }
    const float mean = lb_wave_sum_dpp(s) / (float)C;
    float q = 0.f;
#pragma unroll
    for (int j = 0; j < NV; ++j)
#pragma unroll
        for (int e = 0; e < 8; ++e) {
            const float d = val[j][e] - mean;
            q = ok[j] ? __builtin_fmaf(d, d, q) : q;
        }
    const float rstd = rsqrtf(lb_wave_sum_dpp(q) / (float)C + eps);
#pragma unroll
    for (int j = 0; j < NV; ++j) {
        f16x8 o;
#pragma unroll
        for (int e = 0; e < 8; ++e)
            o[e] = (f16)((val[j][e] - mean) * rstd * gm[j][e >> 2][e & 3] + bt[j][e >> 2][e & 3]);
        *reinterpret_cast<f16x8*>(y + (long)row * ldy + vc[j] * 8) = o;
    }
}

static int g_ln_form = 1;
extern "C" void lb_layernorm_set_form(int form) { g_ln_form = form; }

extern "C" int lb_layernorm_f16(const void* x, void* y, const float* gamma, const float* beta, int M,
                                int C, int ldx, int ldy, float eps, void* stream) {
    LB_REQUIRE(M > 0 && C > 0 && C % 8 == 0 && C <= 2048, "lb_layernorm_f16: C multiple of 8, <= 2048");
    LB_REQUIRE(ldx % 8 == 0 && ldy % 8 == 0, "lb_layernorm_f16: ld multiple of 8");
    const int form = g_ln_form;
    const int nv = (C / 8 + 63) / 64;
    const dim3 grid((M + 3) / 4), block(256);
#define LB_LN_ARGS (const f16*)x, gamma, beta, (f16*)y, M, C, ldx, ldy, eps
    if (form == 0) LB_DISPATCH_STMT("lb_layernorm_f16", hipLaunchKernelGGL(layernorm_kernel, grid, block, 0, s, LB_LN_ARGS));
    if (nv == 1) LB_DISPATCH_STMT("lb_layernorm_f16", hipLaunchKernelGGL(layernorm_rows_kernel<1>, grid, block, 0, s, LB_LN_ARGS));
    if (nv == 2) LB_DISPATCH_STMT("lb_layernorm_f16", hipLaunchKernelGGL(layernorm_rows_kernel<2>, grid, block, 0, s, LB_LN_ARGS));
    if (nv == 3) LB_DISPATCH_STMT("lb_layernorm_f16", hipLaunchKernelGGL(layernorm_rows_kernel<3>, grid, block, 0, s, LB_LN_ARGS));
    LB_DISPATCH_STMT("lb_layernorm_f16", hipLaunchKernelGGL(layernorm_rows_kernel<4>, grid, block, 0, s, LB_LN_ARGS));
#undef LB_LN_ARGS
}
```

latentblending_amd/hip/lib.py:

```python
from __future__ import annotations

import ctypes as C
import os

import torch

_HERE = os.path.dirname(os.path.abspath(__file__))
LIB_PATH = os.environ.get("LB_HIP_LIBRARY") or os.path.join(_HERE, "liblbhip.so")

c_void_pp = C.POINTER(C.c_void_p)


class LbGemmParams(C.Structure):
    _fields_ = [
        ("A", C.c_void_p), ("W", C.c_void_p), ("C", C.c_void_p), ("bias", C.c_void_p),
        ("residual", C.c_void_p), ("rowvec", C.c_void_p), ("partial", C.c_void_p),
        ("M", C.c_int), ("N", C.c_int), ("K", C.c_int),
        ("lda", C.c_int), ("ldw", C.c_int), ("ldc", C.c_int), ("ldr", C.c_int),
        ("ld_rowvec", C.c_int), ("rows_per_batch", C.c_int),
        ("alpha", C.c_float), ("flags", C.c_int),
        ("conv", C.c_int), ("Hin", C.c_int), ("Win", C.c_int), ("Cin", C.c_int),
        ("Hout", C.c_int), ("Wout", C.c_int), ("KH", C.c_int), ("KW", C.c_int),
        ("stride", C.c_int), ("pad", C.c_int), ("ups", C.c_int), ("ldx", C.c_int),
        ("splitk", C.c_int), ("zero_page", C.c_void_p),
        ("scatter", C.c_int), ("sc_py", C.c_int), ("sc_px", C.c_int), ("reserved_", C.c_int),
        ("ln_colsum", C.c_void_p), ("ln_eps", C.c_float), ("reserved2_", C.c_int), ("ch_stats", C.c_void_p), ("ch_stats_rows", C.c_int),
    ]


class LbAttnParams(C.Structure):
    _fields_ = [
        ("Q", C.c_void_p), ("K", C.c_void_p), ("V", C.c_void_p), ("O", C.c_void_p),
        ("B", C.c_int), ("H", C.c_int), ("Sq", C.c_int), ("Skv", C.c_int), ("Skv_valid", C.c_int),
        ("ldq", C.c_int), ("ldk", C.c_int), ("ldv", C.c_int), ("ldo", C.c_int),
        ("scale", C.c_float), ("causal", C.c_int), ("zero_page", C.c_void_p), ("reserved_", C.c_int),
    ]


GEMM_OUT_F32, GEMM_RES_F32, GEMM_GEGLU, GEMM_TRANS_OUT, GEMM_SILU, GEMM_RELU, GEMM_LN_A = 1, 2, 4, 8, 16, 32, 64
GEMM_QUICK_GELU, GEMM_GELU, GEMM_CH_STATS = 128, 256, 512
GEMM_HALO_RAGGED = 1024
GEMM_HALO_KSPLIT = 4096
GEMM_C64 = 2048

_vp, _i, _l, _f, _d = C.c_void_p, C.c_int, C.c_long, C.c_float, C.c_double

SIGNATURES = {
    "lb_version": (_i, []),
    "lb_last_error_string": (C.c_char_p, []),
    "lb_device_info": (_i, [_i, C.POINTER(_i), C.POINTER(_l), C.c_char_p, _i]),
    "lb_slerp_pairs_f16": (_i, [c_void_pp, c_void_pp, c_void_pp, C.POINTER(_d), _i, _l, _vp]),
    "lb_slerp_pairs_f32": (_i, [c_void_pp, c_void_pp, c_void_pp, C.POINTER(_d), _i, _l, _vp]),
    "lb_slerp_pairs_f64": (_i, [c_void_pp, c_void_pp, c_void_pp, C.POINTER(_d), _i, _l, _vp]),
    "lb_slerp_batched_f16": (_i, [_vp, _vp, _vp, _vp, _l, _l, _vp]),
    "lb_slerp_strided_f16": (_i, [_vp, _l, _vp, _l, _vp, _vp, _l, _l, _vp]),
    "lb_lerp_f16": (_i, [_vp, _vp, _vp, _l, _d, _vp]),
    "lb_lerp_f32": (_i, [_vp, _vp, _vp, _l, _d, _vp]),
    "lb_scale_model_input_f16": (_i, [_vp, _vp, _vp, _l, _i, _i, _vp]),
    "lb_euler_step_f16": (_i, [_vp, _vp, _vp, _vp, _vp, _l, _i, _i, _i, _vp]),
    "lb_ddim_step_f16": (_i, [_vp, _vp, _vp, _vp, _l, _i, _i, _vp]),
    "lb_gemm_f16": (_i, [C.POINTER(LbGemmParams), _vp]),
    "lb_gemm_workspace_bytes": (_l, [_i, _i]),
    "lb_gemm_set_tuning": (None, [_i, _i]),
    "lb_gemm_set_depth": (None, [_i]),
    "lb_gemm_set_variant": (None, [_i, _i]),
    "lb_gemm_set_wide_store": (None, [_i]),
    "lb_gemm_set_lean_epilogue": (None, [_i]),
    "lb_gemm_set_t192_waves8": (None, [_i]),
    "lb_gemm_set_kgroups": (None, [_i]),
    "lb_gemm_pp_set_group": (None, [_i]),
    "lb_gemm_set_pp_auto": (None, [_i]),
    "lb_gemm_set_halo": (None, [_i]),
    "lb_conv3x3_halo_f16": (_i, [C.POINTER(LbGemmParams), _vp]),
    "lb_conv3x3_narrow_f16": (_i, [C.POINTER(LbGemmParams), _vp]),
    "lb_upconv2x_halo_f16": (_i, [C.POINTER(LbGemmParams), _vp]),
    "lb_conv_halo_set_persistent": (None, [_i]),
    "lb_gemm_ch_stat_rows": (_i, [C.POINTER(LbGemmParams)]),
    "lb_conv_halo_plan": (None, [C.POINTER(LbGemmParams), C.POINTER(C.c_int), C.POINTER(C.c_int), C.POINTER(C.c_long), C.POINTER(C.c_long)]),
    "lb_gemm_plan": (_i, [C.POINTER(LbGemmParams), C.POINTER(C.c_int), C.POINTER(C.c_int), C.POINTER(C.c_long)]),
    "lb_groupnorm_workspace_bytes": (_l, [_i, _i]),
    "lb_groupnorm_set_l3_chunk": (None, [_l]),
    "lb_groupnorm_nhwc": (_i, [_vp, _vp, _vp, _vp, _vp, _i, _i, _i, _i, _i, _i, _f, _i, _i, _vp]),
    "lb_groupnorm_from_stats": (_i, [_vp, _vp, _vp, _vp, _vp, _vp, _i, _i, _i, _i, _i, _i, _f, _i, _i, _i, _vp]),
    "lb_layernorm_f16": (_i, [_vp, _vp, _vp, _vp, _i, _i, _i, _i, _f, _vp]),
    "lb_attn_fwd_d64": (_i, [C.POINTER(LbAttnParams), _vp]),
    "lb_attn_fwd_d512": (_i, [C.POINTER(LbAttnParams), _vp]),
    "lb_attn_set_tuning": (None, [_i]),
    "lb_layernorm_set_form": (None, [_i]),
    "lb_groupnorm_set_fused": (None, [_i]),
    "lb_groupnorm_plan": (_i, [_i, _i, _i, _i]),
    "lb_softmax_rows_f16": (_i, [_vp, _i, _i, _i, _f, _vp]),
    "lb_sinusoid_f16": (_i, [_vp, _i, _i, _i, _i, _vp, _i, _i, _vp]),
    "lb_copy_cols_f16": (_i, [_vp, _vp, _l, _i, _i, _i, _i, _vp]),
    "lb_cast_f16_to_f32": (_i, [_vp, _vp, _l, _vp]),
    "lb_cast_f32_to_f16": (_i, [_vp, _vp, _l, _f, _vp]),
    "lb_nchw_to_nhwc_f16": (_i, [_vp, _vp, _i, _i, _i, _i, _f, _vp]),
    "lb_nhwc_to_nchw_f16": (_i, [_vp, _vp, _i, _i, _i, _i, _vp]),
    "lb_postprocess_u8": (_i, [_vp, _vp, _l, _i, _i, _vp]),
    "lb_lpips_prep_u8": (_i, [_vp, _vp, _l, _vp]),
    "lb_maxpool3s2_nhwc_f16": (_i, [_vp, _vp, _i, _i, _i, _i, _vp]),
    "lb_lpips_tap": (_i, [c_void_pp, c_void_pp, _vp, _vp, _vp, _i, _i, _i, _vp]),
    "lb_fill_f32": (_i, [_vp, _l, _f, _vp]),
    "lb_embed_tokens_f16": (_i, [_vp, _vp, _vp, _vp, _i, _i, _i, _i, _vp]),
    "lb_frames_lerp_u8": (_i, [_vp, _vp, _vp, _vp, _l, _l, _vp]),
    "lb_gather_rows_f16": (_i, [_vp, _vp, _vp, _i, _i, _i, _vp]),
    "lb_copy_d2d": (_i, [_vp, _vp, _l, _vp]),
    "lb_jpeg_dct_quant_u8": (_i, [_vp, _vp, _vp, _i, _i, _i, _i, _vp]),
    "lb_jpeg_coefficient_count": (_l, [_i, _i, _i, _i]),
    "lb_jpeg_entropy": (_i, [_vp, _vp, _vp, _l, _vp, _i, _i, _i, _i, _vp]),
    "lb_jpeg_workspace_bytes": (_l, [_i, _i, _i, _i]),
    "lb_resample_u8": (_i, [_vp, _vp, _vp, _i, _i, _i, _i, _i, _vp, _vp, _vp, _i, _vp, _vp, _vp, _i, _vp]),
    "lb_program_create": (_vp, []),
    "lb_program_destroy": (None, [_vp]),
    "lb_program_begin_record": (_i, [_vp]),
    "lb_program_end_record": (_i, [_vp]),
    "lb_program_recording": (_i, []),
    "lb_program_num_ops": (_i, [_vp]),
    "lb_program_op_name": (C.c_char_p, [_vp, _i]),
    "lb_program_run": (_i, [_vp, _vp]),
    "lb_program_run_range": (_i, [_vp, _i, _i, _vp]),
    "lb_program_instantiate": (_i, [_vp]),
    "lb_program_launch": (_i, [_vp, _vp]),
    "lb_program_time_ops": (_i, [_vp, _vp, C.POINTER(C.c_float)]),
}

STUDY_SIGNATURES = {
    "lb_slerp_set_study": (None, [_i]),
    "lb_gemm_set_policy": (None, [_i]),
    "lb_conv_halo_set_study": (None, [_i]),
}

HOST_SIGNATURES = {
    "lb_conv_halo_ksplit_plan": (None, [C.POINTER(LbGemmParams), C.POINTER(C.c_long), C.POINTER(C.c_long), C.POINTER(C.c_int)]),
    "lb_conv_halo_ksplit_workspace_bytes": (_l, [C.POINTER(LbGemmParams)]),
    "lb_conv_halo_set_ksplit": (None, [_i, _i]),
}

_NO_CHECK = {"lb_version", "lb_last_error_string", "lb_gemm_workspace_bytes", "lb_jpeg_coefficient_count", "lb_jpeg_workspace_bytes",
             "lb_groupnorm_workspace_bytes", "lb_groupnorm_set_l3_chunk", "lb_conv_halo_set_persistent", "lb_conv_halo_plan","lb_gemm_ch_stat_rows", "lb_conv_halo_set_study", "lb_gemm_set_tuning", "lb_gemm_set_depth", "lb_gemm_set_variant", "lb_gemm_set_wide_store", "lb_gemm_set_lean_epilogue", "lb_gemm_set_t192_waves8", "lb_gemm_set_kgroups", "lb_gemm_pp_set_group", "lb_gemm_set_pp_auto", "lb_gemm_set_policy", "lb_gemm_set_halo", "lb_attn_set_tuning", "lb_layernorm_set_form", "lb_groupnorm_set_fused", "lb_groupnorm_plan", "lb_slerp_set_study", "lb_program_create",
             "lb_program_destroy", "lb_program_recording", "lb_program_num_ops", "lb_program_op_name"}


def _load():
    if not os.path.isfile(LIB_PATH):
        raise ImportError(
            f"latentblending_amd: {LIB_PATH} is missing. Build it with "
            "`python -c 'import __graft_entry__ as g; g.build()'` (hipcc, gfx950). "
            "There is no CPU fallback for the kernel path.")
    return C.CDLL(LIB_PATH, mode=C.RTLD_GLOBAL)


_lib = _load()


class _Api:
    pass


def _wrap(name, fn):
    def checked(*args):
        rc = fn(*args)
        if rc != 0:
            msg = _lib.lb_last_error_string()
            raise RuntimeError(f"{name} failed ({rc}): {msg.decode() if msg else '?'}")
        return rc
    checked.__name__ = name
    return checked


api = _Api()
for _name, (_res, _args) in SIGNATURES.items():
    _fn = getattr(_lib, _name)
    _fn.restype = _res
    _fn.argtypes = _args
    setattr(api, _name, _fn if _name in _NO_CHECK else _wrap(_name, _fn))
for _name, (_res, _args) in HOST_SIGNATURES.items():
    _fn = getattr(_lib, _name)
    _fn.restype = _res
    _fn.argtypes = _args
    setattr(api, _name, _fn)
for _name, (_res, _args) in STUDY_SIGNATURES.items():
    _fn = getattr(_lib, _name, None)
    if _fn is not None:
        _fn.restype = _res
        _fn.argtypes = _args
        setattr(api, _name, _fn)

if os.environ.get("LB_GEMM_WIDE_STORE"):
    api.lb_gemm_set_wide_store(int(os.environ["LB_GEMM_WIDE_STORE"]))
if os.environ.get("LB_GEMM_LEAN_EPILOGUE"):
    api.lb_gemm_set_lean_epilogue(int(os.environ["LB_GEMM_LEAN_EPILOGUE"]))
if os.environ.get("LB_GEMM_PP_AUTO"):
    api.lb_gemm_set_pp_auto(int(os.environ["LB_GEMM_PP_AUTO"]))
```

latentblending_amd/hip/ops.py:

```python
from __future__ import annotations

import ctypes as C
from typing import List, Optional, Sequence

import torch

from . import lib
from .lib import api, LbGemmParams, LbAttnParams

F16, F32, F64 = torch.float16, torch.float32, torch.float64


def stream_ptr() -> int:
    return torch.cuda.current_stream().cuda_stream


def _ptr(t: Optional[torch.Tensor]) -> Optional[int]:
    return None if t is None else t.data_ptr()


def _own_buffer(wrapper: str, what: str) -> None:
    if api.lb_program_recording():
        raise RuntimeError(f"{wrapper}: called while a program is recording without a caller-owned {what}; "
                           f"pass one in (and keep it alive as long as the program) or call lib.api directly")
# ... 165 lines not shown


def subpixel_upsample_weights(w: torch.Tensor, cin_pad: Optional[int] = None):
    cout, cin, _, _ = w.shape
    cp = cin_pad or (cin + 7) // 8 * 8
    w = w.float()
    rows = {0: [w[:, :, 0], w[:, :, 1] + w[:, :, 2]], 1: [w[:, :, 0] + w[:, :, 1], w[:, :, 2]]}
    out = {}
    for py in (0, 1):
        for px in (0, 1):
            k = torch.zeros(cout, 2, 2, cp, dtype=torch.float32, device=w.device)
            for a in (0, 1):
                r = rows[py][a]
                cols = [r[:, :, 0], r[:, :, 1] + r[:, :, 2]] if px == 0 else [r[:, :, 0] + r[:, :, 1], r[:, :, 2]]
                for b in (0, 1):
                    k[:, a, b, :cin] = cols[b]
            out[(py, px)] = k.reshape(cout, 4 * cp).to(F16).contiguous()
    return out


def gemm(A: torch.Tensor, W: torch.Tensor, bias=None, residual=None, rowvec=None, rows_per_batch=0,
         flags: int = 0, alpha: float = 1.0, out: Optional[torch.Tensor] = None, splitk_ws: bool = True,
         conv: Optional[dict] = None, M: Optional[int] = None, ln=None, ch_stats: Optional[torch.Tensor] = None,
         workspace: Optional[torch.Tensor] = None) -> torch.Tensor:
    p = LbGemmParams()
    N, K = W.shape
    dev = A.device
    if conv is not None:
        B, H, Wd, Cin = A.shape
        ups = int(conv.get("ups", 0))
        kh, kw, st, pad = conv["KH"], conv["KW"], conv.get("stride", 1), conv.get("pad", 0)
        hout = ((H << ups) + 2 * pad - kh) // st + 1
        wout = ((Wd << ups) + 2 * pad - kw) // st + 1
        Mv = B * hout * wout
        p.conv, p.Hin, p.Win, p.Cin, p.Hout, p.Wout = 1, H, Wd, Cin, hout, wout
        p.KH, p.KW, p.stride, p.pad, p.ups, p.ldx = kh, kw, st, pad, ups, A.stride(2)
        out_shape = (B, hout, wout)
        if "parity" in conv:
            if conv["parity"] == "all":
                p.scatter = 2
            else:
                p.scatter, p.sc_py, p.sc_px = 1, int(conv["parity"][0]), int(conv["parity"][1])
            hout, wout = H, Wd
            Mv = B * H * Wd
            p.Hout, p.Wout = H, Wd
    else:
        Mv = M if M is not None else A.shape[0]
        p.lda = A.stride(0)
        out_shape = (Mv,)
    n_out = N // 2 if flags & lib.GEMM_GEGLU else N
    if out is None:
        odt = F32 if flags & lib.GEMM_OUT_F32 else F16
        if flags & lib.GEMM_TRANS_OUT:
            out = torch.empty(n_out, Mv, dtype=odt, device=dev)
        else:
            out = torch.empty(out_shape + (n_out,), dtype=odt, device=dev)
    p.A, p.W, p.C = A.data_ptr(), W.data_ptr(), out.data_ptr()
    p.bias, p.residual, p.rowvec = _ptr(bias), _ptr(residual), _ptr(rowvec)
    p.M, p.N, p.K, p.ldw = Mv, N, K, W.stride(0)
    p.ldc = out.stride(0) if (flags & lib.GEMM_TRANS_OUT) else out.stride(-2)
    if residual is not None:
        p.ldr = residual.stride(-2)
    if rowvec is not None:
        p.ld_rowvec, p.rows_per_batch = rowvec.stride(0), rows_per_batch
    p.alpha, p.flags = alpha, flags
    zp = zero_page(dev)
    p.zero_page = zp.data_ptr()
    if ln is not None:
        p.flags |= lib.GEMM_LN_A
        p.ln_colsum, p.ln_eps = ln[0].data_ptr(), float(ln[1])
    if ch_stats is not None:
        p.flags |= lib.GEMM_CH_STATS
        p.ch_stats, p.ch_stats_rows = ch_stats.data_ptr(), ch_stats.shape[1]
    ws = None
    if splitk_ws and not (flags & lib.GEMM_GEGLU) and ln is None:
        ws = workspace
        if ws is None:
            _own_buffer("gemm", "split-K `workspace` (or splitk_ws=False)")
            ws = torch.empty(api.lb_gemm_workspace_bytes(Mv, N) // 4, dtype=F32, device=dev)
        assert ws.numel() * ws.element_size() >= api.lb_gemm_workspace_bytes(Mv, N), "gemm: split-K workspace too small"
        p.partial = ws.data_ptr()
    if conv is not None and conv.get("halo"):
        api.lb_conv3x3_halo_f16(C.byref(p), stream_ptr())
    else:
        api.lb_gemm_f16(C.byref(p), stream_ptr())
    return out


def fold_layernorm(w: torch.Tensor, bias: Optional[torch.Tensor], gamma: torch.Tensor, beta: torch.Tensor):
    wf = (w.double() * gamma.double()[None, :]).to(F16)
    b2 = w.double() @ beta.double()
    if bias is not None:
        b2 = b2 + bias.double()
    return wf, wf.double().sum(dim=1).to(F32), b2.to(F32)


def groupnorm_nhwc(x: torch.Tensor, gamma: torch.Tensor, beta: torch.Tensor, groups: int, eps: float,
                   silu: bool, ldx: Optional[int] = None, ldy: Optional[int] = None,
                   out: Optional[torch.Tensor] = None, workspace: Optional[torch.Tensor] = None) -> torch.Tensor:
    B, C = x.shape[0], x.shape[-1]
    HW = x.numel() // (B * C)
    y = torch.empty(x.shape, dtype=F16, device=x.device) if out is None else out
    ws = _groupnorm_workspace("groupnorm_nhwc", workspace, B, groups, x.device)
    api.lb_groupnorm_nhwc(x.data_ptr(), y.data_ptr(), gamma.data_ptr(), beta.data_ptr(), ws.data_ptr(),
                          B, HW, C, C if ldx is None else ldx, C if ldy is None else ldy, groups, eps, int(silu),
                          int(x.dtype == F32), stream_ptr())
    return y


def _groupnorm_workspace(wrapper: str, workspace: Optional[torch.Tensor], B: int, groups: int, device) -> torch.Tensor:
    nbytes = api.lb_groupnorm_workspace_bytes(B, groups)
    if workspace is None:
        _own_buffer(wrapper, "`workspace`")
        return torch.empty(nbytes // 8, dtype=F64, device=device)
    assert workspace.numel() * workspace.element_size() >= nbytes, f"{wrapper}: workspace too small"
    return workspace


def conv_halo_plan(B: int, H: int, W: int, cin: int, cout: int, ks: int = 3, flags: int = 0):
    p = LbGemmParams()
    p.flags = flags
    p.conv, p.M, p.N, p.K = 1, B * H * W, cout, ks * ks * cin
    p.Hin, p.Win, p.Hout, p.Wout, p.Cin, p.KH, p.KW, p.stride, p.ldx = H, W, H, W, cin, ks, ks, 1, cin
    p.pad, p.scatter = (1, 0) if ks == 3 else (0, 2)
    p.zero_page = 64
    kind, tw, items, grid = C.c_int(), C.c_int(), C.c_long(), C.c_long()
    api.lb_conv_halo_plan(C.byref(p), C.byref(kind), C.byref(tw), C.byref(items), C.byref(grid))
    return kind.value, tw.value, items.value, grid.value


def conv_ch_stat_rows(B: int, H: int, W: int, cin: int, cout: int, ks: int = 3, flags: int = 0) -> int:
    p = LbGemmParams()
    p.flags = flags
    p.conv, p.M, p.N, p.K = 1, B * H * W, cout, ks * ks * cin
    p.Hin, p.Win, p.Hout, p.Wout, p.Cin, p.KH, p.KW, p.stride, p.ldx = H, W, H, W, cin, ks, ks, 1, cin
    p.pad, p.scatter = (1, 0) if ks == 3 else (0, 2)
    p.zero_page = 64
    return int(api.lb_gemm_ch_stat_rows(C.byref(p)))


def groupnorm_from_stats(x: torch.Tensor, gamma: torch.Tensor, beta: torch.Tensor, groups: int, eps: float, silu: bool,
                         ch_stats: torch.Tensor, rows_per_sample: int, ldx: Optional[int] = None, ldy: Optional[int] = None,
                         out: Optional[torch.Tensor] = None, workspace: Optional[torch.Tensor] = None) -> torch.Tensor:
    B, C_ = x.shape[0], x.shape[-1]
    HW = x.numel() // (B * C_)
    y = torch.empty(x.shape, dtype=F16, device=x.device) if out is None else out
    ws = _groupnorm_workspace("groupnorm_from_stats", workspace, B, groups, x.device)
    api.lb_groupnorm_from_stats(x.data_ptr(), y.data_ptr(), gamma.data_ptr(), beta.data_ptr(), ch_stats.data_ptr(), ws.data_ptr(),
                                B, HW, C_, C_ if ldx is None else ldx, C_ if ldy is None else ldy, groups, eps, int(silu),
                                int(x.dtype == F32), rows_per_sample, stream_ptr())
    return y


def layernorm(x: torch.Tensor, gamma: torch.Tensor, beta: torch.Tensor, eps: float = 1e-5) -> torch.Tensor:
    M, Cc = x.shape
    y = torch.empty_like(x)
    api.lb_layernorm_f16(x.data_ptr(), y.data_ptr(), gamma.data_ptr(), beta.data_ptr(), M, Cc,
                         x.stride(0), y.stride(0), eps, stream_ptr())
    return y


_ZERO_PAGES = {}


def zero_page(device) -> torch.Tensor:
    key = str(device)
    if key not in _ZERO_PAGES:
        _ZERO_PAGES[key] = torch.zeros(64, dtype=torch.uint8, device=device)
    return _ZERO_PAGES[key]


def attention_d64(q: torch.Tensor, k: torch.Tensor, v: torch.Tensor, B: int, H: int, Sq: int, Skv: int,
                  skv_valid: Optional[int] = None, ldq=None, ldk=None, ldv=None,
                  out: Optional[torch.Tensor] = None, causal: bool = False) -> torch.Tensor:
    p = LbAttnParams()
    if out is None:
        out = torch.empty(B * Sq, H * 64, dtype=F16, device=q.device)
    p.Q, p.K, p.V, p.O = q.data_ptr(), k.data_ptr(), v.data_ptr(), out.data_ptr()
    p.B, p.H, p.Sq, p.Skv, p.Skv_valid = B, H, Sq, Skv, skv_valid or Skv
    p.ldq, p.ldk, p.ldv, p.ldo = ldq or q.stride(0), ldk or k.stride(0), ldv or v.stride(0), out.stride(0)
    p.scale = 0.125
    p.causal = int(causal)
    p.zero_page = zero_page(q.device).data_ptr()
    api.lb_attn_fwd_d64(C.byref(p), stream_ptr())
    return out


def attention_d512(q: torch.Tensor, k: torch.Tensor, v: torch.Tensor, B: int, H: int, Sq: int, Skv: int,
                   skv_valid: Optional[int] = None, out: Optional[torch.Tensor] = None) -> torch.Tensor:
    p = LbAttnParams()
    if out is None:
        out = torch.empty(B * Sq, H * 512, dtype=F16, device=q.device)
    p.Q, p.K, p.V, p.O = q.data_ptr(), k.data_ptr(), v.data_ptr(), out.data_ptr()
    p.B, p.H, p.Sq, p.Skv, p.Skv_valid = B, H, Sq, Skv, skv_valid or Skv
    p.ldq, p.ldk, p.ldv, p.ldo = q.stride(0), k.stride(0), v.stride(0), out.stride(0)
    p.scale = 512.0 ** -0.5
    p.causal = 0
    p.zero_page = zero_page(q.device).data_ptr()
    api.lb_attn_fwd_d512(C.byref(p), stream_ptr())
    return out


def softmax_rows_(x: torch.Tensor, scale: float = 1.0) -> torch.Tensor:
    M, N = x.shape
    api.lb_softmax_rows_f16(x.data_ptr(), M, N, x.stride(0), scale, stream_ptr())
    return x


def sinusoid(vals: torch.Tensor, dim: int, out: Optional[torch.Tensor] = None, col_off: int = 0) -> torch.Tensor:
    rows, per_row = vals.shape
    if out is None:
        out = torch.empty(rows, per_row * dim, dtype=F16, device=vals.device)
    api.lb_sinusoid_f16(vals.data_ptr(), rows, per_row, vals.stride(0), dim, out.data_ptr(), out.stride(0),
                        col_off, stream_ptr())
    return out


def copy_cols(src: torch.Tensor, dst: torch.Tensor, dst_off: int):
    rows = src.numel() // src.shape[-1]
    api.lb_copy_cols_f16(src.data_ptr(), dst.data_ptr(), rows, src.shape[-1], src.stride(-2), dst.stride(-2),
                         dst_off, stream_ptr())


def nchw_to_nhwc(x: torch.Tensor, ld: int, mul: float = 1.0) -> torch.Tensor:
    B, Cc, H, W = x.shape
    y = torch.empty(B, H, W, ld, dtype=F16, device=x.device)
    x = _operand("nchw_to_nhwc", x, x.contiguous())
    api.lb_nchw_to_nhwc_f16(x.data_ptr(), y.data_ptr(), B, Cc, H * W, ld, mul, stream_ptr())
    return y


def nhwc_to_nchw(x: torch.Tensor, channels: int) -> torch.Tensor:
    B, H, W, ld = x.shape
    y = torch.empty(B, channels, H, W, dtype=F16, device=x.device)
    api.lb_nhwc_to_nchw_f16(x.data_ptr(), y.data_ptr(), B, channels, H * W, ld, stream_ptr())
    return y


def postprocess_u8(x: torch.Tensor) -> torch.Tensor:
    B, H, W, ld = x.shape
    out = torch.empty(B, H, W, 3, dtype=torch.uint8, device=x.device)
    api.lb_postprocess_u8(x.data_ptr(), out.data_ptr(), B * H * W, ld, int(x.dtype == F32), stream_ptr())
    return out


def maxpool3s2(x: torch.Tensor) -> torch.Tensor:
    N, H, W, Cc = x.shape
    y = torch.empty(N, (H - 3) // 2 + 1, (W - 3) // 2 + 1, Cc, dtype=F16, device=x.device)
    api.lb_maxpool3s2_nhwc_f16(x.data_ptr(), y.data_ptr(), N, H, W, Cc, stream_ptr())
    return y


def frames_lerp_u8(frames: torch.Tensor, left, weights, out: Optional[torch.Tensor] = None, tables=None) -> torch.Tensor:
    assert frames.dtype == torch.uint8 and frames.is_contiguous()
    n_out = len(left)
    fb = frames[0].numel()
    if tables is None:
        _own_buffer("frames_lerp_u8", "`tables` (left, weights) on the device")
        left_d = torch.tensor(list(left), dtype=torch.int32, device=frames.device)
        w_d = torch.tensor(list(weights), dtype=F64, device=frames.device)
    else:
        left_d, w_d = tables
        assert left_d.dtype == torch.int32 and w_d.dtype == F64 and left_d.numel() >= n_out and w_d.numel() >= n_out
    if out is None:
        out = torch.empty((n_out,) + tuple(frames.shape[1:]), dtype=torch.uint8, device=frames.device)
    for k0 in range(0, n_out, 65535):
        k1 = min(n_out, k0 + 65535)
        api.lb_frames_lerp_u8(frames.data_ptr(), left_d[k0:].data_ptr(), w_d[k0:].data_ptr(), out[k0:].data_ptr(), k1 - k0, fb,
                              stream_ptr())
    return out


def cast_f16_to_f32(x: torch.Tensor, out: Optional[torch.Tensor] = None) -> torch.Tensor:
    assert x.dtype == F16 and x.is_contiguous()
    if out is None:
        out = torch.empty(x.shape, dtype=F32, device=x.device)
    api.lb_cast_f16_to_f32(x.data_ptr(), out.data_ptr(), x.numel(), stream_ptr())
    return out


def cast_f32_to_f16(x: torch.Tensor, mul: float = 1.0, out: Optional[torch.Tensor] = None) -> torch.Tensor:
    assert x.dtype == F32 and x.is_contiguous()
    if out is None:
        out = torch.empty(x.shape, dtype=F16, device=x.device)
    api.lb_cast_f32_to_f16(x.data_ptr(), out.data_ptr(), x.numel(), float(mul), stream_ptr())
    return out


def fill_f32_(x: torch.Tensor, value: float) -> torch.Tensor:
    assert x.dtype == F32 and x.is_contiguous()
    api.lb_fill_f32(x.data_ptr(), x.numel(), float(value), stream_ptr())
    return x


def lpips_prep_u8(img: torch.Tensor, out: Optional[torch.Tensor] = None) -> torch.Tensor:
    assert img.dtype == torch.uint8 and img.is_contiguous() and img.shape[-1] == 3
    if out is None:
        out = torch.empty(tuple(img.shape[:-1]) + (8,), dtype=F16, device=img.device)
    api.lb_lpips_prep_u8(img.data_ptr(), out.data_ptr(), img.numel() // 3, stream_ptr())
    return out


def lpips_tap(feats_a: Sequence[torch.Tensor], feats_b: Sequence[torch.Tensor], lin: torch.Tensor, acc: torch.Tensor,
              workspace: Optional[torch.Tensor] = None) -> torch.Tensor:
    assert len(feats_a) == len(feats_b) and 0 < len(feats_a) <= 16 and acc.dtype == F32 and acc.numel() >= len(feats_a)
    hw, c = feats_a[0].shape[-2], feats_a[0].shape[-1]
# ... 176 lines not shown
```

latentblending_amd/native/runtime.py:

```python
from __future__ import annotations

import contextlib
import ctypes as C
from typing import Dict, List, Optional, Tuple

import torch

from ..hip import lib
from ..hip.lib import api, LbGemmParams, LbAttnParams
from .geometry import use_ragged_halo

F16, F32 = torch.float16, torch.float32


class Arena:
    def __init__(self, device):
        self.device = device
        self.free: Dict[int, List[torch.Tensor]] = {}
        self.all: List[torch.Tensor] = []
        self.bytes_allocated = 0

    @staticmethod
    def _cls(nbytes: int) -> int:
        return max(512, (nbytes + 511) // 512 * 512)

    def alloc(self, shape, dtype=F16) -> torch.Tensor:
        n = 1
        for s in shape:
            n *= int(s)
        esz = torch.empty((), dtype=dtype).element_size()
        cls = self._cls(n * esz)
        pool = self.free.get(cls)
        if pool:
            raw = pool.pop()
        else:
            raw = torch.empty(cls, dtype=torch.uint8, device=self.device)
            self.all.append(raw)
            self.bytes_allocated += cls
        t = raw[: n * esz].view(dtype).view(*shape)
        t._lb_raw = raw
        return t

    def release(self, t: Optional[torch.Tensor]) -> None:
        if t is None:
            return
        st = getattr(t, "_lb_chstats", None)
        if st is not None:
            t._lb_chstats = None
            self.release(st[0])
        raw = getattr(t, "_lb_raw", None)
        if raw is None:
            return
        t._lb_raw = None
        self.free.setdefault(raw.numel(), []).append(raw)


class Program:
    def __init__(self, name: str = "program"):
        self.name = name
        self.handle = api.lb_program_create()
        self.keep: List[object] = []
        self.graph_ready = False

    def __del__(self):
        try:
            if self.handle:
                api.lb_program_destroy(self.handle)
                self.handle = None
        except Exception:
            pass

    @contextlib.contextmanager
    def record(self):
        api.lb_program_begin_record(self.handle)
        self.graph_ready = False
        try:
            yield self
        finally:
            api.lb_program_end_record(self.handle)

    @property
    def num_ops(self) -> int:
        return api.lb_program_num_ops(self.handle)

    def op_names(self) -> List[str]:
        return [api.lb_program_op_name(self.handle, i).decode() for i in range(self.num_ops)]

    def run(self, stream: Optional[int] = None) -> None:
        api.lb_program_run(self.handle, stream if stream is not None else _stream())

    def run_range(self, begin: int, end: int, stream: Optional[int] = None) -> None:
        api.lb_program_run_range(self.handle, begin, end, stream if stream is not None else _stream())

    def instantiate(self) -> None:
        api.lb_program_instantiate(self.handle)
        self.graph_ready = True

    def launch(self, stream: Optional[int] = None) -> None:
        api.lb_program_launch(self.handle, stream if stream is not None else _stream())

    def time_ops(self, stream: Optional[int] = None) -> List[float]:
        n = self.num_ops
        buf = (C.c_float * n)()
        api.lb_program_time_ops(self.handle, stream if stream is not None else _stream(), buf)
        return list(buf)


def _stream() -> int:
    return torch.cuda.current_stream().cuda_stream


def _p(t: Optional[torch.Tensor]) -> Optional[int]:
    return None if t is None else t.data_ptr()


class Emitter:

    def __init__(self, arena: Arena):
        self.arena = arena
        self.device = arena.device
        self.ws_gemm: Optional[torch.Tensor] = None
        self.ws_gn: Optional[torch.Tensor] = None
        self.gemm_log: List[dict] = []
        self.attn_log: List[dict] = []
        self.norm_log: List[dict] = []
        self._retired: List[torch.Tensor] = []
        self.zero_page = torch.zeros(64, dtype=torch.uint8, device=self.device)
        self.ragged_halo = False
        self.halo_ksplit = True
        self.ws_ksplit: Optional[torch.Tensor] = None

    def _ragged_flag(self, p: LbGemmParams) -> int:
        if not self.ragged_halo or not p.conv or p.KH != 3 or p.KW != 3 or p.stride != 1 or p.scatter or p.ups or p.N <= 16:
            return 0
        kind, tw = C.c_int(), C.c_int()
        flags = p.flags
        p.flags = flags & ~lib.GEMM_HALO_RAGGED
        api.lb_conv_halo_plan(C.byref(p), C.byref(kind), None, None, None)
        plain = kind.value
        p.flags = flags | lib.GEMM_HALO_RAGGED
        api.lb_conv_halo_plan(C.byref(p), C.byref(kind), C.byref(tw), None, None)
        p.flags = flags
        return lib.GEMM_HALO_RAGGED if use_ragged_halo(True, plain, kind.value, p.Hin, p.Win, tw.value) else 0

    def _gemm_ws(self, M: int, N: int) -> Optional[torch.Tensor]:
        if ((M + 63) // 64) * ((N + 63) // 64) > 640:
            return None
        need = api.lb_gemm_workspace_bytes(M, N) // 4
        if self.ws_gemm is None or self.ws_gemm.numel() < need:
            if self.ws_gemm is not None:
                self._retired.append(self.ws_gemm)
            self.ws_gemm = torch.empty(max(need, 1 << 22), dtype=F32, device=self.device)
        return self.ws_gemm

    _KSPLIT_COUNTER_BYTES = 1 << 20

    def _halo_ksplit(self, p: LbGemmParams) -> bool:
        if not self.halo_ksplit or not p.conv or p.KH != 3 or p.KW != 3 or p.stride != 1 or p.scatter or p.ups:
            return False
        tile, sk, nb = C.c_int(), C.c_int(), C.c_long()
        api.lb_gemm_plan(C.byref(p), C.byref(tile), C.byref(sk), C.byref(nb))
        if tile.value != 6:
            return False
        flags = p.flags
        p.flags = flags | lib.GEMM_HALO_KSPLIT
        units, grid, split = C.c_long(), C.c_long(), C.c_int()
        api.lb_conv_halo_ksplit_plan(C.byref(p), C.byref(units), C.byref(grid), C.byref(split))
        need = int(api.lb_conv_halo_ksplit_workspace_bytes(C.byref(p)))
        if not split.value or need <= 0:
            p.flags = flags
            return False
        counters = ((units.value // (p.Cin // 64)) * 4 + 255) // 256 * 256
        slabs = need - counters
        assert slabs > 0 and slabs % (256 * 128 * 4) == 0, (need, counters)
        if counters > self._KSPLIT_COUNTER_BYTES:
            p.flags = flags
            return False
        total = self._KSPLIT_COUNTER_BYTES + slabs
        if self.ws_ksplit is None or self.ws_ksplit.numel() < total:
            if self.ws_ksplit is not None:
                self._retired.append(self.ws_ksplit)
            self.ws_ksplit = torch.zeros(total, dtype=torch.uint8, device=self.device)
        p.partial = self.ws_ksplit.data_ptr() + self._KSPLIT_COUNTER_BYTES - counters
        return True

    def _gn_ws(self, B: int, groups: int) -> torch.Tensor:
        need = api.lb_groupnorm_workspace_bytes(B, groups) // 8
        if self.ws_gn is None or self.ws_gn.numel() < need:
            if self.ws_gn is not None:
                self._retired.append(self.ws_gn)
            self.ws_gn = torch.empty(need, dtype=torch.float64, device=self.device)
        return self.ws_gn

    def gemm(self, A: torch.Tensor, W: torch.Tensor, out: torch.Tensor, *, M: int, bias=None,
             residual=None, rowvec=None, rows_per_batch: int = 0, flags: int = 0, alpha: float = 1.0,
             lda: Optional[int] = None, ldc: Optional[int] = None, ldr: Optional[int] = None,
             ld_rowvec: Optional[int] = None, conv: Optional[dict] = None, splitk: bool = True,
             ln: Optional[Tuple[torch.Tensor, float]] = None, ch_stats: Optional[torch.Tensor] = None):
        p = LbGemmParams()
        N, K = W.shape
        p.A, p.W, p.C = A.data_ptr(), W.data_ptr(), out.data_ptr()
        p.bias, p.residual, p.rowvec = _p(bias), _p(residual), _p(rowvec)
        p.M, p.N, p.K, p.ldw = M, N, K, W.stride(0)
        n_out = N // 2 if flags & lib.GEMM_GEGLU else N
        if conv is not None:
            p.conv = 1
            for k in ("Hin", "Win", "Cin", "Hout", "Wout", "KH", "KW", "stride", "pad", "ups", "ldx"):
                setattr(p, k, int(conv[k]))
            if conv.get("parity") == "all":
                p.scatter = 2
            elif "parity" in conv:
                p.scatter, p.sc_py, p.sc_px = 1, int(conv["parity"][0]), int(conv["parity"][1])
        else:
            p.lda = lda if lda is not None else K
        p.ldc = ldc if ldc is not None else (M if flags & lib.GEMM_TRANS_OUT else n_out)
        p.ldr = ldr if ldr is not None else n_out
        if rowvec is not None:
            p.ld_rowvec, p.rows_per_batch = ld_rowvec if ld_rowvec is not None else N, rows_per_batch
        p.alpha, p.flags = alpha, flags
        p.zero_page = self.zero_page.data_ptr()
        if ln is not None:
            p.flags |= lib.GEMM_LN_A
            p.ln_colsum, p.ln_eps = ln[0].data_ptr(), float(ln[1])
        if ch_stats is not None:
            assert conv is not None and ch_stats.dtype == F32
            p.flags |= lib.GEMM_CH_STATS
            p.ch_stats, p.ch_stats_rows = ch_stats.data_ptr(), ch_stats.shape[1]
        if splitk and not (flags & lib.GEMM_GEGLU) and ln is None:
            p.partial = _p(self._gemm_ws(M, N))
        if self.ragged_halo:
            p.flags |= self._ragged_flag(p)
        if conv is not None:
            self._halo_ksplit(p)
        api.lb_gemm_f16(C.byref(p), _stream())
        mult = 4.0 if p.scatter == 2 else 1.0
        self.gemm_log.append({"M": M, "N": N, "K": K, "flops": mult * 2.0 * M * N * K, "conv": conv is not None,
                              "bytes": mult * 2.0 * (N * K + M * n_out) + (2.0 * M * K if conv is None else 0.0)})
        return out

    def plan(self, M: int, N: int, K: int, flags: int = 0) -> Tuple[int, int]:
        p = LbGemmParams()
        p.M, p.N, p.K, p.flags = M, N, K, flags
        p.zero_page = self.zero_page.data_ptr()
        if not (flags & lib.GEMM_GEGLU):
            p.partial = _p(self._gemm_ws(M, N))
        t, sk, nb = C.c_int(), C.c_int(), C.c_long()
        api.lb_gemm_plan(C.byref(p), C.byref(t), C.byref(sk), C.byref(nb))
        return t.value, sk.value

    def halo_stat_rows(self, B: int, H: int, W: int, cin: int, cout: int, ks: int = 3) -> int:
        p = LbGemmParams()
        p.conv, p.M, p.N, p.K = 1, B * H * W, cout, ks * ks * cin
        p.Hin, p.Win, p.Hout, p.Wout, p.Cin, p.KH, p.KW, p.stride, p.ldx = H, W, H, W, cin, ks, ks, 1, cin
        p.pad, p.scatter = (1, 0) if ks == 3 else (0, 2)
        p.zero_page = self.zero_page.data_ptr()
        if ks == 2 and not self.upconv_one_launch(B, H, W, cin, cout):
            return 0
        if self.ragged_halo:
            p.flags |= self._ragged_flag(p)
        return int(api.lb_gemm_ch_stat_rows(C.byref(p)))

    @staticmethod
    def upconv_one_launch(B: int, H: int, W: int, cin: int, cout: int) -> bool:
        shape_ok = cin % 64 == 0 and ((W % 32 == 0 and H % 8 == 0) or (W % 16 == 0 and H % 16 == 0))
        blocks = B * (H * W // 256) * 4 * ((cout + 127) // 128)
        return shape_ok and blocks >= 96

    def groupnorm(self, x: torch.Tensor, out: torch.Tensor, gamma, beta, *, B: int, HW: int, C_: int,
                  eps: float, silu: bool, groups: int = 32, ldx: Optional[int] = None,
                  ch_stats: Optional[Tuple[torch.Tensor, int]] = None):
        if ch_stats is not None:
            api.lb_groupnorm_from_stats(x.data_ptr(), out.data_ptr(), gamma.data_ptr(), beta.data_ptr(), ch_stats[0].data_ptr(),
                                        self._gn_ws(B, groups).data_ptr(), B, HW, C_, ldx or C_, C_, groups, eps, int(silu),
                                        int(x.dtype == F32), int(ch_stats[1]), _stream())
            self.norm_log.append({"op": "lb_groupnorm_from_stats", "bytes": float(B * HW * C_) * (x.element_size() + 2)})
            return out
        api.lb_groupnorm_nhwc(x.data_ptr(), out.data_ptr(), gamma.data_ptr(), beta.data_ptr(),
                              self._gn_ws(B, groups).data_ptr(), B, HW, C_, ldx or C_, C_, groups, eps,
                              int(silu), int(x.dtype == F32), _stream())
        one = bool(api.lb_groupnorm_plan(HW, C_, groups, int(x.dtype == F32)))
        self.norm_log.append({"op": "lb_groupnorm_nhwc", "bytes": float(B * HW * C_) * ((1 if one else 2) * x.element_size() + 2), "one_launch": one})
        return out

    def layernorm(self, x, out, gamma, beta, *, M: int, C_: int, eps: float = 1e-5):
        api.lb_layernorm_f16(x.data_ptr(), out.data_ptr(), gamma.data_ptr(), beta.data_ptr(), M, C_, C_, C_,
                             eps, _stream())
        self.norm_log.append({"op": "lb_layernorm_f16", "bytes": float(M * C_) * 4})
        return out

    def attention(self, q_ptr: int, k_ptr: int, v_ptr: int, out: torch.Tensor, *, B, H, Sq, Skv, valid,
                  ldq, ldk, ldv, ldo, causal: bool = False, head_dim: int = 64):
        assert head_dim in (64, 512) and not (causal and head_dim == 512)
        p = LbAttnParams()
        p.Q, p.K, p.V, p.O = q_ptr, k_ptr, v_ptr, out.data_ptr()
        p.B, p.H, p.Sq, p.Skv, p.Skv_valid = B, H, Sq, Skv, valid
        p.ldq, p.ldk, p.ldv, p.ldo = ldq, ldk, ldv, ldo
        p.scale = float(head_dim) ** -0.5
        p.causal = int(causal)
        p.zero_page = self.zero_page.data_ptr()
        (api.lb_attn_fwd_d512 if head_dim == 512 else api.lb_attn_fwd_d64)(C.byref(p), _stream())
        self.attn_log.append({"flops": 4.0 * B * H * Sq * valid * head_dim, "Sq": Sq, "Skv": Skv, "head_dim": head_dim})
        return out

    def copy_cols(self, src, dst, *, rows, cols, ld_src, ld_dst, dst_off):
        api.lb_copy_cols_f16(src.data_ptr(), dst.data_ptr(), rows, cols, ld_src, ld_dst, dst_off, _stream())

    def copy(self, dst: torch.Tensor, src: torch.Tensor):
        assert dst.numel() * dst.element_size() == src.numel() * src.element_size()
        api.lb_copy_d2d(dst.data_ptr(), src.data_ptr(), src.numel() * src.element_size(), _stream())
```

latentblending_amd/native/vae.py:

```python
from __future__ import annotations

from dataclasses import dataclass
from typing import Dict, Tuple

import torch

from ..hip import lib
from ..hip.lib import api
from .geometry import latent_hw
from .runtime import Arena, Emitter, Program, F16, F32, _stream
from .unet import _pad

STREAM_SCALE = 1.0 / 16.0


@dataclass
class VAEConfig:
    latent_channels: int = 4
    out_channels: int = 3
    block_channels: Tuple[int, ...] = (128, 256, 512, 512)
    layers_per_block: int = 2
    norm_groups: int = 32
    scaling_factor: float = 0.13025
    force_upcast: bool = True
    stream_fp16_scaled: bool = True
    fuse_gn_stats: bool = True
    fused_mid_attention: bool = True

    @property
    def scale_factor(self) -> int:
        return 2 ** (len(self.block_channels) - 1)


class NativeVAEDecoder:
    def __init__(self, cfg: VAEConfig, provider, device="cuda"):
        self.cfg, self.device = cfg, torch.device(device)
        self.w: Dict[str, torch.Tensor] = {}
        self._load(provider)

    def _dev(self, t, dtype):
        return t.to(device=self.device, dtype=dtype).contiguous()

    def _conv(self, pv, name, cin, cout, k, gain=1.0):
        w = pv.weight(name + ".weight", (cout, cin, k, k), cin * k * k, gain)
        cin_p, cout_p = _pad(cin, 8), _pad(cout, 4)
        packed = torch.zeros(cout_p, k, k, cin_p, dtype=torch.float32)
        packed[:cout, :, :, :cin] = w.permute(0, 2, 3, 1)
        self.w[name + ".weight"] = self._dev(packed.reshape(cout_p, k * k * cin_p), F16)
        b = torch.zeros(cout_p, dtype=torch.float32)
        b[:cout] = pv.bias(name + ".bias", cout)
        self.w[name + ".bias"] = self._dev(b, F32)

    def _upconv(self, pv, name, c):
        from ..hip.ops import subpixel_upsample_weights
        w = pv.weight(name + ".weight", (c, c, 3, 3), c * 9, 1.0)
        subs = subpixel_upsample_weights(w, _pad(c, 8))
        for (py, px), k in subs.items():
            self.w[f"{name}.weight.sub{py}{px}"] = k.to(self.device)
        self.w[f"{name}.weight.sub4"] = torch.stack([subs[(0, 0)], subs[(0, 1)], subs[(1, 0)], subs[(1, 1)]]).to(self.device).contiguous()
        self.w[name + ".bias"] = self._dev(pv.bias(name + ".bias", c), F32)

    def _norm(self, pv, name, c):
        self.w[name + ".weight"] = self._dev(pv.norm_weight(name + ".weight", c), F32)
        self.w[name + ".bias"] = self._dev(pv.bias(name + ".bias", c), F32)

    def _resnet(self, pv, p, cin, cout):
        self._norm(pv, p + ".norm1", cin)
        self._conv(pv, p + ".conv1", cin, cout, 3)
        self._norm(pv, p + ".norm2", cout)
        self._conv(pv, p + ".conv2", cout, cout, 3, gain=0.5)
        if cin != cout:
            w = pv.weight(p + ".conv_shortcut.weight", (cout, cin, 1, 1), cin, 1.0)
            self.w[p + ".conv_shortcut.weight"] = self._dev(w.reshape(cout, cin), F16)
            self.w[p + ".conv_shortcut.bias"] = self._dev(pv.bias(p + ".conv_shortcut.bias", cout), F32)

    def _load(self, pv):
        cfg = self.cfg
        rev = list(reversed(cfg.block_channels))
        top = rev[0]
        self._conv(pv, "post_quant_conv", cfg.latent_channels, cfg.latent_channels, 1)
        self._conv(pv, "decoder.conv_in", cfg.latent_channels, top, 3)
        self._resnet(pv, "decoder.mid_block.resnets.0", top, top)
        a = "decoder.mid_block.attentions.0"
        self._norm(pv, a + ".group_norm", top)
        for nm in ("to_q", "to_k"):
            self.w[f"{a}.{nm}.weight"] = self._dev(pv.weight(f"{a}.{nm}.weight", (top, top), top), F16)
            self.w[f"{a}.{nm}.bias"] = self._dev(pv.bias(f"{a}.{nm}.bias", top), F32)
        wv = pv.weight(a + ".to_v.weight", (top, top), top)
        bv = pv.bias(a + ".to_v.bias", top)
        wo = pv.weight(a + ".to_out.0.weight", (top, top), top, 0.5)
        bo = pv.bias(a + ".to_out.0.bias", top)
        self.w[a + ".to_v.weight"] = self._dev(wv, F16)
        self.w[a + ".to_out.0.weight"] = self._dev(wo, F16)
        self.w[a + ".to_out.0.bias"] = self._dev(bo + wo.half().float() @ bv, F32)
        if top == 512:
            self.w[a + ".qkv.weight"] = torch.cat([self.w[a + ".to_q.weight"], self.w[a + ".to_k.weight"], self.w[a + ".to_v.weight"]], 0).contiguous()
            self.w[a + ".qkv.bias"] = torch.cat([self.w[a + ".to_q.bias"], self.w[a + ".to_k.bias"],
                                                 torch.zeros_like(self.w[a + ".to_q.bias"])], 0).contiguous()
        self._resnet(pv, "decoder.mid_block.resnets.1", top, top)
        prev = top
        for ui, c in enumerate(rev):
            for li in range(cfg.layers_per_block + 1):
                self._resnet(pv, f"decoder.up_blocks.{ui}.resnets.{li}", prev, c)
                prev = c
            if ui < len(rev) - 1:
                self._upconv(pv, f"decoder.up_blocks.{ui}.upsamplers.0.conv", c)
        self._norm(pv, "decoder.conv_norm_out", rev[-1])
        self._conv(pv, "decoder.conv_out", rev[-1], cfg.out_channels, 3, gain=0.5)
        for key in [k for k in self.w if k.endswith(".bias")]:
            self.w[key + "_s"] = self.w[key] * STREAM_SCALE

    def build(self, B: int, L, ragged_halo: bool = True) -> "VAEProgram":
        return VAEProgram(self, B, L, ragged_halo=ragged_halo)


class VAEProgram:

    def __init__(self, net: NativeVAEDecoder, B: int, L, ragged_halo: bool = True):
        cfg = net.cfg
        H, W = latent_hw(L)
        self.net, self.B, self.H, self.W = net, B, H, W
        self.L = H if H == W else None
        self.scaled = bool(cfg.stream_fp16_scaled)
        self.fuse_gn_stats = bool(getattr(cfg, "fuse_gn_stats", True))
        self.fused_mid_attention = bool(getattr(cfg, "fused_mid_attention", True))
        dev = net.device
        self.arena = Arena(dev)
        self.em = Emitter(self.arena)
        self.ragged_halo = self.em.ragged_halo = bool(ragged_halo) and H != W
        SH, SW = H * cfg.scale_factor, W * cfg.scale_factor
        self.z_in = torch.zeros(B, cfg.latent_channels, H, W, dtype=F16, device=dev)
        self.frames = torch.zeros(B, SH, SW, 3, dtype=torch.uint8, device=dev)
        self.image_f32 = torch.zeros(B, SH, SW, _pad(cfg.out_channels, 4), dtype=F32, device=dev)
        self._pq = torch.zeros(B, H, W, _pad(cfg.latent_channels, 8), dtype=F16, device=dev)
        self.prog = Program("vae-decode")
        with self.prog.record():
            self._emit()

    def _stats_for(self, out, B, H, W, cin_p, cout_p, ks=3):
        rows = self.em.halo_stat_rows(B, H, W, cin_p, cout_p, ks) if self.fuse_gn_stats else 0
        if not rows:
            return None
        buf = self.arena.alloc((cout_p, B * rows, 2), F32)
        out._lb_chstats = (buf, rows)
        return buf

    def _stream_conv(self, x, name, B, H, W, cin, cout, *, residual=None, out=None, stats=True):
        w, sc = self.net.w, self.scaled
        cin_p, cout_p = _pad(cin, 8), _pad(cout, 4)
        if out is None:
            out = self.arena.alloc((B, H, W, cout_p), F16 if sc else F32)
        flags = 0 if sc else (lib.GEMM_OUT_F32 | (lib.GEMM_RES_F32 if residual is not None else 0))
        st = self._stats_for(out, B, H, W, cin_p, cout_p) if stats else None
        self.em.gemm(x, w[name + ".weight"], out, M=B * H * W, bias=w[name + (".bias_s" if sc else ".bias")],
                     residual=residual, flags=flags, alpha=STREAM_SCALE if sc else 1.0, ch_stats=st,
                     conv=dict(Hin=H, Win=W, Cin=cin_p, Hout=H, Wout=W, KH=3, KW=3, stride=1, pad=1, ups=0, ldx=cin_p))
        return out

    def _gn(self, x, out, name, B, HW, c, silu):
        w = self.net.w
        eps = 1e-6 * (STREAM_SCALE * STREAM_SCALE if self.scaled else 1.0)
        st = getattr(x, "_lb_chstats", None)
        self.em.groupnorm(x, out, w[name + ".weight"], w[name + ".bias"], B=B, HW=HW, C_=c, eps=eps, silu=silu,
                          groups=self.net.cfg.norm_groups, ch_stats=st)
        if st is not None:
            self.arena.release(st[0])
            x._lb_chstats = None

    def _stream_as_operand(self, x, B, H, W, c):
        if self.scaled:
            return x, False
        x16 = self.arena.alloc((B, H, W, c))
        api.lb_cast_f32_to_f16(x.data_ptr(), x16.data_ptr(), x.numel(), STREAM_SCALE, _stream())
        return x16, True

    def _resnet(self, x, p, B, H, W, cin, cout):
        em, w, ar, sc = self.em, self.net.w, self.arena, self.scaled
        n1 = ar.alloc((B, H, W, cin))
        self._gn(x, n1, p + ".norm1", B, H * W, cin, True)
        h = self._stream_conv(n1, p + ".conv1", B, H, W, cin, cout)
        ar.release(n1)
        n2 = ar.alloc((B, H, W, cout))
        self._gn(h, n2, p + ".norm2", B, H * W, cout, True)
        ar.release(h)
        if cin != cout:
            x16, owned = self._stream_as_operand(x, B, H, W, cin)
            xs = ar.alloc((B, H, W, cout), F16 if sc else F32)
            em.gemm(x16, w[p + ".conv_shortcut.weight"], xs, M=B * H * W,
                    bias=w[p + (".conv_shortcut.bias_s" if sc else ".conv_shortcut.bias")],
                    flags=0 if sc else lib.GEMM_OUT_F32, alpha=1.0 if sc else 1.0 / STREAM_SCALE)
            if owned:
                ar.release(x16)
        else:
            xs = x
        out = self._stream_conv(n2, p + ".conv2", B, H, W, cout, cout, residual=xs)
        ar.release(n2)
        if xs is not x:
            ar.release(xs)
        return out

    def _mid_attention(self, h, B, H, W, c):
        em, w, ar, sc = self.em, self.net.w, self.arena, self.scaled
        a = "decoder.mid_block.attentions.0"
        S = H * W
        n = ar.alloc((B * S, c))
        self._gn(h, n, a + ".group_norm", B, S, c, False)
        if self.fused_mid_attention and (a + ".qkv.weight") in w:
            qkv = ar.alloc((B * S, 3 * c))
            em.gemm(n, w[a + ".qkv.weight"], qkv, M=B * S, bias=w[a + ".qkv.bias"])
            ar.release(n)
            o = ar.alloc((B * S, c))
            em.attention(qkv.data_ptr(), qkv.data_ptr() + 2 * c, qkv.data_ptr() + 4 * c, o, B=B, H=1, Sq=S, Skv=S, valid=S,
                         ldq=3 * c, ldk=3 * c, ldv=3 * c, ldo=c, head_dim=512)
            ar.release(qkv)
            return self._attn_out(o, h, B, S)
        q, k = ar.alloc((B * S, c)), ar.alloc((B * S, c))
        em.gemm(n, w[a + ".to_q.weight"], q, M=B * S, bias=w[a + ".to_q.bias"])
        em.gemm(n, w[a + ".to_k.weight"], k, M=B * S, bias=w[a + ".to_k.bias"])
        vt = ar.alloc((c, B * S))
        em.gemm(w[a + ".to_v.weight"], n, vt, M=c)
        ar.release(n)
        o = ar.alloc((B * S, c))
        scores = ar.alloc((S, S))
        for b in range(B):
            qb, kb, ob = q[b * S:(b + 1) * S], k[b * S:(b + 1) * S], o[b * S:(b + 1) * S]
            em.gemm(qb, kb, scores, M=S, alpha=float(c) ** -0.5)
            api.lb_softmax_rows_f16(scores.data_ptr(), S, S, S, 1.0, _stream())
            em.gemm(scores, vt[:, b * S:(b + 1) * S], ob, M=S, lda=S)
        ar.release(scores); ar.release(q); ar.release(k); ar.release(vt)
        return self._attn_out(o, h, B, S)

    def _attn_out(self, o, h, B, S):
        em, w, ar, sc = self.em, self.net.w, self.arena, self.scaled
        a = "decoder.mid_block.attentions.0"
        em.gemm(o, w[a + ".to_out.0.weight"], h, M=B * S, bias=w[a + (".to_out.0.bias_s" if sc else ".to_out.0.bias")],
                residual=h, flags=0 if sc else (lib.GEMM_OUT_F32 | lib.GEMM_RES_F32), alpha=STREAM_SCALE if sc else 1.0)
        ar.release(o)
        return h

    def _emit(self):
        net, cfg, em, w, ar, B, LH, LW = self.net, self.net.cfg, self.em, self.net.w, self.arena, self.B, self.H, self.W
        sc = self.scaled
        rev = list(reversed(cfg.block_channels))
        top, lc = rev[0], cfg.latent_channels
        lc_p = _pad(lc, 8)
        z8 = ar.alloc((B, LH, LW, lc_p))
        api.lb_nchw_to_nhwc_f16(self.z_in.data_ptr(), z8.data_ptr(), B, lc, LH * LW, lc_p, 1.0 / cfg.scaling_factor,
                                _stream())
        em.gemm(z8, w["post_quant_conv.weight"], self._pq, M=B * LH * LW, bias=w["post_quant_conv.bias"], ldc=lc_p)
        ar.release(z8)
        h = self._stream_conv(self._pq, "decoder.conv_in", B, LH, LW, lc, top)
        nxt = self._resnet(h, "decoder.mid_block.resnets.0", B, LH, LW, top, top); ar.release(h); h = nxt
        h = self._mid_attention(h, B, LH, LW, top)
        nxt = self._resnet(h, "decoder.mid_block.resnets.1", B, LH, LW, top, top); ar.release(h); h = nxt
        sh, sw, prev = LH, LW, top
        for ui, c in enumerate(rev):
            for li in range(cfg.layers_per_block + 1):
                nxt = self._resnet(h, f"decoder.up_blocks.{ui}.resnets.{li}", B, sh, sw, prev, c)
                ar.release(h); h = nxt
                prev = c
            if ui < len(rev) - 1:
                h16, owned = self._stream_as_operand(h, B, sh, sw, c)
                name = f"decoder.up_blocks.{ui}.upsamplers.0.conv"
                up = ar.alloc((B, 2 * sh, 2 * sw, c), F16 if sc else F32)
                one = em.upconv_one_launch(B, sh, sw, c, c)
                if one:
                    em.gemm(h16, w[f"{name}.weight.sub4"][0], up, M=B * sh * sw,
                            bias=w[name + (".bias_s" if sc else ".bias")], ldc=c,
                            flags=0 if sc else lib.GEMM_OUT_F32, alpha=1.0 if sc else 1.0 / STREAM_SCALE,
                            ch_stats=self._stats_for(up, B, sh, sw, c, c, ks=2),
                            conv=dict(Hin=sh, Win=sw, Cin=c, Hout=sh, Wout=sw, KH=2, KW=2, stride=1, pad=0,
                                      ups=0, ldx=c, parity="all"))
                for py in (() if one else (0, 1)):
                    for px in (0, 1):
                        em.gemm(h16, w[f"{name}.weight.sub{py}{px}"], up, M=B * sh * sw,
                                bias=w[name + (".bias_s" if sc else ".bias")], ldc=c,
                                flags=0 if sc else lib.GEMM_OUT_F32, alpha=1.0 if sc else 1.0 / STREAM_SCALE,
                                conv=dict(Hin=sh, Win=sw, Cin=c, Hout=sh, Wout=sw, KH=2, KW=2, stride=1, pad=0,
                                          ups=0, ldx=c, parity=(py, px)))
                if owned:
                    ar.release(h16)
                ar.release(h)
                h = up
                sh, sw = 2 * sh, 2 * sw
        n = ar.alloc((B, sh, sw, rev[-1]))
        self._gn(h, n, "decoder.conv_norm_out", B, sh * sw, rev[-1], True)
        ar.release(h)
        cin_p = _pad(rev[-1], 8)
        em.gemm(n, w["decoder.conv_out.weight"], self.image_f32, M=B * sh * sw, bias=w["decoder.conv_out.bias"],
                flags=lib.GEMM_OUT_F32,
                conv=dict(Hin=sh, Win=sw, Cin=cin_p, Hout=sh, Wout=sw, KH=3, KW=3, stride=1, pad=1, ups=0, ldx=cin_p))
        ar.release(n)
        api.lb_postprocess_u8(self.image_f32.data_ptr(), self.frames.data_ptr(), B * sh * sw,
                              _pad(cfg.out_channels, 4), 1, _stream())

    def decode(self, z: torch.Tensor) -> torch.Tensor:
        self.z_in.copy_(z)
        self.prog.launch()
        return self.frames
```

Before: 127.3 frames/s.

## Fold VAE decoder GroupNorm+SiLU into the A-operand load of 3x3 convs

Adds a GN_A mode to the halo and narrow 3x3 conv kernels. A per-(sample, channel) scale/shift table is built from the channel stats, and the kernels apply GroupNorm and SiLU in LDS to the halo tile after it loads. The VAE resnet blocks and conv_out now feed the raw activation plus this table instead of writing and re-reading a normalized tensor. A policy limits the fused halo path to narrow-N convs with many tiles per block and falls back to a separate GroupNorm otherwise. This saves one full activation write and read per norm, at the cost of extra LDS, an extra per-tile transform in the pipeline, and possible occupancy or scheduling loss.

New measurement: 128.7 frames/s (median of 6 runs). 1.01x the previous value.

```diff
diff --git a/include/lb_hip.h b/include/lb_hip.h
--- a/include/lb_hip.h
+++ b/include/lb_hip.h
@@ -49,6 +49,7 @@
     LB_GEMM_HALO_RAGGED = 1024,
     LB_GEMM_HALO_KSPLIT = 4096,
     LB_GEMM_C64 = 2048,
+    LB_GEMM_GN_A = 8192,
     LB_GEMM_LN_A = 64
 };
 
@@ -76,6 +77,8 @@
     int reserved2_;
     float* ch_stats;
     int ch_stats_rows;
+    const float* gn_table;
+    int gn_silu;
 } LbGemmParams;
 
 int lb_gemm_f16(const LbGemmParams* params, void* stream);
@@ -90,6 +93,7 @@
 void lb_conv_halo_set_persistent(int on);
 void lb_conv_halo_plan(const LbGemmParams* params, int* kind, int* tile_w, long* items, long* grid);
 #include "lb_hip_ksplit.h"
+#include "lb_hip_gn_a.h"
 int lb_gemm_ch_stat_rows(const LbGemmParams* params);
 int lb_upconv2x_halo_f16(const LbGemmParams* params, void* stream);
 void lb_gemm_set_halo(int mode);
diff --git a/include/lb_hip_gn_a.h b/include/lb_hip_gn_a.h
--- /dev/null
+++ b/include/lb_hip_gn_a.h
@@ -0,0 +1,13 @@
+#ifndef LB_HIP_GN_A_H
+#define LB_HIP_GN_A_H
+#ifdef __cplusplus
+extern "C" {
+#endif
+int lb_groupnorm_affine_from_stats(const float* ch_stats, const float* gamma, const float* beta, float* table, int B, int HW,
+                                   int C, int groups, float eps, int stat_rows_per_sample, void* stream);
+void lb_conv_halo_gn_a_plan(const LbGemmParams* params, int* fuse, int* kind);
+void lb_conv_halo_set_gn_a(int mode, int grid);
+#ifdef __cplusplus
+}
+#endif
+#endif
diff --git a/latentblending_amd/csrc/conv3_halo.hip b/latentblending_amd/csrc/conv3_halo.hip
--- a/latentblending_amd/csrc/conv3_halo.hip
+++ b/latentblending_amd/csrc/conv3_halo.hip
@@ -11,6 +11,9 @@
 
 template <int N> __device__ __forceinline__ void halo_wait_barrier() {
     asm volatile("s_waitcnt vmcnt(%0)\n\ts_barrier" ::"n"(N) : "memory");
+}
+template <int N> __device__ __forceinline__ void halo_wait_barrier_lds() {
+    asm volatile("s_waitcnt vmcnt(%0) lgkmcnt(0)\n\ts_barrier" ::"n"(N) : "memory");
 }
 
 template <int KS, int J> struct HaloSched {
@@ -22,10 +25,13 @@
     return n;
 }
 
-template <int BN, int TW, int KS = 3, bool RAG = false, bool KSP = false>
+template <bool GNA, int TAP> constexpr int halo_gna_loads_in_tap() { return GNA && TAP == 0 ? 1 : 0; }
+
+template <int BN, int TW, int KS = 3, bool RAG = false, bool KSP = false, bool GNA = false>
 __global__ void __launch_bounds__(512) conv3x3_halo_kernel(const LbGemmParams p) {
     static_assert(!RAG || KS == 3, "ragged tiles exist for the 3x3 form only");
     static_assert(!KSP || (KS == 3 && !RAG), "the K-split form exists for the whole-tile 3x3 form only");
+    static_assert(!GNA || (KS == 3 && !RAG && !KSP), "the GroupNorm-on-A form exists for the whole-tile unsplit 3x3 form only");
     constexpr int TH = 256 / TW;
     constexpr int NTAP = KS * KS;
     constexpr int HWP = TW + KS - 1;
@@ -138,6 +144,30 @@
         __builtin_amdgcn_global_load_lds((gptr_t)src, (lptr_t)dst, 16, 0, 0);
     };
 
+    f16* const gn_area = wring + 4 * BN * 64 + wave * 512;
+    auto issue_gn_table = [&](int b_req, int chunk) {
+        const float* src = p.gn_table + ((long)b_req * p.Cin + chunk * 64) * 2 + (lane & 31) * 4;
+        __builtin_amdgcn_global_load_lds((gptr_t)src, (lptr_t)gn_area, 16, 0, 0);
+    };
+    auto gn_transform = [&](int j, int buf) {
+        if (h_off[j] >= 0) {
+            f16* pc = halo0 + buf * (HRP * 64) + (j * 8 + wave) * 8 * 64 + lane * 8;
+            const f32x4* tb = reinterpret_cast<const f32x4*>(gn_area) + cl * 4;
+            const f32x4 t0 = tb[0], t1 = tb[1], t2 = tb[2], t3 = tb[3];
+            const f16x8 v = *reinterpret_cast<const f16x8*>(pc);
+            f16x8 o;
+            o[0] = lb_gn_apply((float)v[0], t0[0], t0[1], p.gn_silu);
+            o[1] = lb_gn_apply((float)v[1], t0[2], t0[3], p.gn_silu);
+            o[2] = lb_gn_apply((float)v[2], t1[0], t1[1], p.gn_silu);
+            o[3] = lb_gn_apply((float)v[3], t1[2], t1[3], p.gn_silu);
+            o[4] = lb_gn_apply((float)v[4], t2[0], t2[1], p.gn_silu);
+            o[5] = lb_gn_apply((float)v[5], t2[2], t2[3], p.gn_silu);
+            o[6] = lb_gn_apply((float)v[6], t3[0], t3[1], p.gn_silu);
+            o[7] = lb_gn_apply((float)v[7], t3[2], t3[3], p.gn_silu);
+            *reinterpret_cast<f16x8*>(pc) = o;
+        }
+    };
+
     int hbase[TM];
     int mloc[TM];
 #pragma unroll
@@ -193,6 +223,7 @@
     }
     TileAt cur = tile_of(item);
     set_halo_offsets(cur, true);
+    if constexpr (GNA) issue_gn_table(cur.b, c_lo);
 #pragma unroll
     for (int j = 0; j < NR; ++j)
         if (j < NR - 1 || wave < EXTRA) issue_halo(j, c_lo, 0);
@@ -200,12 +231,19 @@
     for (int t = 0; t < 3; ++t)
 #pragma unroll
         for (int i = 0; i < WI; ++i) issue_weight(i, c_lo, true, t, t);
-
-    auto step = [&](auto tap_c, int c, int cc, bool more) {
+    if constexpr (GNA) {
+        asm volatile("s_waitcnt vmcnt(%0)" ::"n"(3 * WI) : "memory");
+#pragma unroll
+        for (int j = 0; j < NR; ++j) gn_transform(j, 0);
+    }
+
+    auto step = [&](auto tap_c, int c, int cc, bool more, int gn_b = 0) {
         constexpr int TAP = decltype(tap_c)::value;
         constexpr int P1 = (TAP + NTAP - 1) % NTAP, P2 = (TAP + NTAP - 2) % NTAP;
-        constexpr int CNT = (2 + halo_full_rounds_in_tap<KS, NR, P1>()) + (2 + halo_full_rounds_in_tap<KS, NR, P2>());
-        halo_wait_barrier<CNT>();
+        constexpr int CNT = (2 + halo_full_rounds_in_tap<KS, NR, P1>() + halo_gna_loads_in_tap<GNA, P1>()) +
+                            (2 + halo_full_rounds_in_tap<KS, NR, P2>() + halo_gna_loads_in_tap<GNA, P2>());
+        if constexpr (GNA) halo_wait_barrier_lds<CNT>();
+        else halo_wait_barrier<CNT>();
         const int slot = KS == 3 ? ((cc + TAP) & 3) : TAP;
         const f16* hb = halo0 + (cc & 1) * (HRP * 64);
         const f16* wb = wring + slot * (BN * 64);
@@ -221,6 +259,7 @@
         const int slot3 = (slot + 3) & 3;
         f16x8 a0[TM], w0[TN], a1[TM], w1[TN];
         read_frags(hb, wb, shift, 0, a0, w0);
+        if constexpr (GNA && TAP == 0) issue_gn_table(gn_b, hc);
         if constexpr (HaloSched<KS, 0>::tap == TAP) issue_halo(0, hc, hbuf);
         if constexpr (NR > 2 && HaloSched<KS, 1>::tap == TAP) issue_halo(1, hc, hbuf);
         if constexpr (NR > 3 && HaloSched<KS, 2>::tap == TAP) issue_halo(2, hc, hbuf);
@@ -235,6 +274,10 @@
         __builtin_amdgcn_sched_barrier(0);
         mma_rows(a0, w0, TM / 2, TM);
         __builtin_amdgcn_sched_barrier(0);
+        if constexpr (GNA && TAP >= 3) {
+            gn_transform(TAP - 3, hbuf);
+            __builtin_amdgcn_sched_barrier(0);
+        }
         issue_weight(1, c3, w_exists, TAP3, slot3, wrap);
         __builtin_amdgcn_sched_barrier(0);
         mma_rows(a1, w1, 0, TM);
@@ -258,7 +301,7 @@
                 set_halo_offsets(nxt, more);
                 if constexpr (KSP) set_w_offsets(n0_next, w_offn, w_off32n);
             }
-            step(std::integral_constant<int, 0>{}, c, cc, more);
+            step(std::integral_constant<int, 0>{}, c, cc, more, GNA ? (c + 1 == c_end ? nxt.b : cur.b) : 0);
             step(std::integral_constant<int, 1>{}, c, cc, more);
             step(std::integral_constant<int, 2>{}, c, cc, more);
             step(std::integral_constant<int, 3>{}, c, cc, more);
@@ -434,24 +477,33 @@
     return items / ((p.N + 127) / 128) * 4;
 }
 
-template <int BN, int TW, int KS = 3, bool RAG = false, bool KSP = false>
+static int g_halo_gn_a_mode = 1, g_halo_gn_a_grid = 0;
+
+template <int BN, int TW, int KS = 3, bool RAG = false, bool KSP = false, bool GNA = false>
 static int launch_halo(const LbGemmParams& p, hipStream_t stream, long ksp_grid = 0) {
     constexpr int TH = 256 / TW;
     constexpr int HRP = (((TH + KS - 1) * (TW + KS - 1) + 7) / 8) * 8;
-    constexpr int SMEM = (2 * HRP * 64 + 4 * BN * 64) * (int)sizeof(f16) + (KSP ? 16 : 0);
+    constexpr int SMEM = (2 * HRP * 64 + 4 * BN * 64) * (int)sizeof(f16) + (KSP ? 16 : 0) + (GNA ? 8 * 1024 : 0);
+    static_assert(SMEM <= 160 * 1024, "LDS of one CU");
     static unsigned long long seen = 0;
     LB_ONCE_PER_DEVICE(seen)
-        (void)hipFuncSetAttribute(reinterpret_cast<const void*>(conv3x3_halo_kernel<BN, TW, KS, RAG, KSP>),
+        (void)hipFuncSetAttribute(reinterpret_cast<const void*>(conv3x3_halo_kernel<BN, TW, KS, RAG, KSP, GNA>),
                                   hipFuncAttributeMaxDynamicSharedMemorySize, SMEM);
     static_assert(BN == 128, "halo_grid assumes 128-channel blocks");
     long nblk, grid;
     halo_grid(p, TW, KS, nblk, grid);
     if (KSP) grid = ksp_grid;
+    if (GNA && g_halo_gn_a_grid > 0) {
+        const long period = (p.N + BN - 1) / BN;
+        grid = g_halo_gn_a_grid / period * period;
+        if (grid < period) grid = period;
+        if (grid > nblk) grid = nblk;
+    }
     LbGemmParams pk = p;
 #ifdef LB_STUDY_BUILD
     pk.reserved_ = g_halo_study;
 #endif
-    hipLaunchKernelGGL((conv3x3_halo_kernel<BN, TW, KS, RAG, KSP>), dim3((unsigned)grid), dim3(512), SMEM, stream, pk);
+    hipLaunchKernelGGL((conv3x3_halo_kernel<BN, TW, KS, RAG, KSP, GNA>), dim3((unsigned)grid), dim3(512), SMEM, stream, pk);
     return lb_check_launch(KS == 2 ? "lb_upconv2x_halo_f16" : "lb_conv3x3_halo_f16");
 }
 
@@ -474,6 +526,7 @@
 }
 
 int lb_upconv_halo_check(const LbGemmParams& p) {
+    LB_REQUIRE(!(p.flags & LB_GEMM_GN_A), "halo upconv: LB_GEMM_GN_A is implemented by the whole-tile 3x3 halo conv and the narrow-N conv only");
     LB_REQUIRE(!(p.flags & LB_GEMM_CH_STATS) || (p.ch_stats != nullptr && p.ch_stats_rows == lb_conv_halo_stat_rows_total(p)),
                "halo upconv: LB_GEMM_CH_STATS needs ch_stats with ch_stats_rows = B * lb_gemm_ch_stat_rows()");
     return halo_tiles_check(p, lb_upconv_halo_eligible(p), 2);
@@ -523,6 +576,7 @@
     units = grid = 0;
     split = 0;
     if (!(p.flags & LB_GEMM_HALO_KSPLIT) || (p.flags & LB_GEMM_C64) || g_halo_ksplit_mode == 0) return;
+    if (p.flags & LB_GEMM_GN_A) return;
     const int tw = lb_conv3x3_halo_eligible(p);
     if (!tw || halo3_ragged(p, tw) || p.Cin < 128) return;
     long items, ugrid;
@@ -580,13 +634,45 @@
         LB_REQUIRE(!split || p.partial != nullptr,
                    "halo conv: LB_GEMM_HALO_KSPLIT needs partial = a zeroed workspace of lb_conv_halo_ksplit_workspace_bytes()");
     }
+    if (p.flags & LB_GEMM_GN_A) {
+        LB_REQUIRE(p.gn_table != nullptr, "halo conv: LB_GEMM_GN_A needs gn_table = the [B][Cin] float2 table of lb_groupnorm_affine_from_stats");
+        LB_REQUIRE(!(p.flags & LB_GEMM_HALO_KSPLIT), "halo conv: LB_GEMM_GN_A and LB_GEMM_HALO_KSPLIT exclude each other (the K-split form has no GroupNorm-on-A twin)");
+        LB_REQUIRE(!halo3_ragged(p, lb_conv3x3_halo_eligible(p)), "halo conv: LB_GEMM_GN_A needs an image that divides into whole tiles (no ragged form)");
+        LB_REQUIRE((reinterpret_cast<uintptr_t>(p.gn_table) & 15) == 0, "halo conv: gn_table must be 16-byte aligned");
+    }
     return halo_tiles_check(p, lb_conv3x3_halo_eligible(p), 3);
+}
+
+static constexpr int HALO_GN_A_MAX_BLOCKS = 1;
+static constexpr long HALO_GN_A_MIN_TILES_PER_BLOCK = 32;
+extern "C" void lb_conv_halo_set_gn_a(int mode, int grid) {
+    g_halo_gn_a_mode = mode < 0 ? 1 : mode;
+    g_halo_gn_a_grid = grid > 0 ? grid : 0;
+}
+int lb_conv3x3_halo_gn_a_policy(const LbGemmParams& p) {
+    if (g_halo_gn_a_mode == 0) return 0;
+    if (g_halo_gn_a_mode >= 2) return 1;
+    if ((p.N + 127) / 128 > HALO_GN_A_MAX_BLOCKS) return 0;
+    long items, grid;
+    halo_grid(p, lb_conv3x3_halo_eligible(p), 3, items, grid);
+    return items >= HALO_GN_A_MIN_TILES_PER_BLOCK * grid ? 1 : 0;
+}
+int lb_conv_halo_gn_a_mode() { return g_halo_gn_a_mode; }
+int lb_conv3x3_halo_gn_a_able(const LbGemmParams& p) {
+    const int tw = lb_conv3x3_halo_eligible(p);
+    if (!tw || halo3_ragged(p, tw)) return 0;
+    long units, grid;
+    int split;
+    halo_ksplit_plan(p, units, grid, split);
+    return split ? 0 : 1;
 }
 
 int lb_conv3x3_halo_launch(LbGemmParams p, hipStream_t stream) {
     if (p.alpha == 0.f) p.alpha = 1.f;
     p.splitk = 1;
     const int tw = lb_conv3x3_halo_eligible(p);
+    if (p.flags & LB_GEMM_GN_A)
+        return tw == 32 ? launch_halo<128, 32, 3, false, false, true>(p, stream) : launch_halo<128, 16, 3, false, false, true>(p, stream);
     if (halo3_ragged(p, tw)) return tw == 32 ? launch_halo<128, 32, 3, true>(p, stream) : launch_halo<128, 16, 3, true>(p, stream);
     long units, grid;
     int split;
diff --git a/latentblending_amd/csrc/conv3_narrow.hip b/latentblending_amd/csrc/conv3_narrow.hip
--- a/latentblending_amd/csrc/conv3_narrow.hip
+++ b/latentblending_amd/csrc/conv3_narrow.hip
@@ -10,6 +10,7 @@
 #define NARROW_HRG ((NARROW_HR + 7) / 8)
 #define NARROW_LDS (NARROW_HRG * 8 * 64)
 
+template <bool GNA>
 __global__ void __launch_bounds__(256, 2) conv3x3_narrow_kernel(const LbGemmParams p) {
     __shared__ __attribute__((aligned(16))) f16 halo[NARROW_LDS];
     const int tid = threadIdx.x, lane = tid & 63, wave = tid >> 6;
@@ -62,7 +63,27 @@
 #pragma unroll
             for (int s = 0; s < 2; ++s)
                 wf[tap][s] = n_ok ? *reinterpret_cast<const f16x8*>(wrow + (long)tap * p.Cin + c * 64 + s * 32) : zero8;
+        f32x4 gt[GNA ? 4 : 1];
+        if constexpr (GNA) {
+            const f32x4* tb = reinterpret_cast<const f32x4*>(p.gn_table + ((long)b * p.Cin + c * 64 + cl * 8) * 2);
+#pragma unroll
+            for (int k = 0; k < 4; ++k) gt[k] = tb[k];
+        }
         asm volatile("s_waitcnt vmcnt(0)" ::: "memory");
+        if constexpr (GNA) {
+#pragma unroll
+            for (int j = 0; j < NR; ++j) {
+                const int gidx = j * 4 + wave;
+                if (gidx < NARROW_HRG && h_off[j] >= 0) {
+                    f16* pc = halo + gidx * 8 * 64 + lane * 8;
+                    const f16x8 v = *reinterpret_cast<const f16x8*>(pc);
+                    f16x8 o;
+#pragma unroll
+                    for (int e = 0; e < 8; ++e) o[e] = lb_gn_apply((float)v[e], gt[e >> 1][(e & 1) * 2], gt[e >> 1][(e & 1) * 2 + 1], p.gn_silu);
+                    *reinterpret_cast<f16x8*>(pc) = o;
+                }
+            }
+        }
         __syncthreads();
 #pragma unroll
         for (int tap = 0; tap < 9; ++tap) {
@@ -101,7 +122,7 @@
     if (!p.conv || p.KH != 3 || p.KW != 3 || p.stride != 1 || p.pad != 1 || p.ups || p.scatter) return 0;
     if (p.Hout != p.Hin || p.Wout != p.Win || p.Cin % 64 != 0 || p.K != 9 * p.Cin) return 0;
     if (p.N > 16 || p.N % 4 != 0 || p.zero_page == nullptr) return 0;
-    if (p.flags & ~(LB_GEMM_OUT_F32 | LB_GEMM_HALO_KSPLIT)) return 0;
+    if (p.flags & ~(LB_GEMM_OUT_F32 | LB_GEMM_HALO_KSPLIT | LB_GEMM_GN_A)) return 0;
     if (p.residual != nullptr || p.rowvec != nullptr) return 0;
     if (p.Win % NARROW_T != 0 || p.Hin % NARROW_T != 0 || p.M % (p.Hin * p.Win) != 0) return 0;
     if ((long)p.M * p.ldx >= (1l << 34)) return 0;
@@ -114,13 +135,16 @@
 
 int lb_conv3x3_narrow_check(const LbGemmParams& p) {
     LB_REQUIRE(narrow_tiles(p) < (1l << 31), "conv3x3 narrow: too many tiles for one launch");
+    LB_REQUIRE(!(p.flags & LB_GEMM_GN_A) || (p.gn_table != nullptr && (reinterpret_cast<uintptr_t>(p.gn_table) & 15) == 0),
+               "conv3x3 narrow: LB_GEMM_GN_A needs gn_table = the 16-byte aligned [B][Cin] float2 table of lb_groupnorm_affine_from_stats");
     return 0;
 }
 
 int lb_conv3x3_narrow_launch(LbGemmParams p, hipStream_t stream) {
     if (p.alpha == 0.f) p.alpha = 1.f;
     const long tiles = narrow_tiles(p);
-    hipLaunchKernelGGL(conv3x3_narrow_kernel, dim3((unsigned)tiles), dim3(256), 0, stream, p);
+    if (p.flags & LB_GEMM_GN_A) hipLaunchKernelGGL(conv3x3_narrow_kernel<true>, dim3((unsigned)tiles), dim3(256), 0, stream, p);
+    else hipLaunchKernelGGL(conv3x3_narrow_kernel<false>, dim3((unsigned)tiles), dim3(256), 0, stream, p);
     return lb_check_launch("lb_conv3x3_narrow_f16");
 }
 
diff --git a/latentblending_amd/csrc/gemm.hip b/latentblending_amd/csrc/gemm.hip
--- a/latentblending_amd/csrc/gemm.hip
+++ b/latentblending_amd/csrc/gemm.hip
@@ -473,6 +473,26 @@
     return samples > 0 ? (int)(lb_conv_halo_stat_rows_total(p) / samples) : 0;
 }
 
+int lb_conv3x3_halo_gn_a_able(const LbGemmParams& p);
+int lb_conv3x3_halo_gn_a_policy(const LbGemmParams& p);
+int lb_conv_halo_gn_a_mode();
+extern "C" void lb_conv_halo_gn_a_plan(const LbGemmParams* pp, int* fuse, int* kind) {
+    int f = 0, k = 0;
+    if (pp != nullptr && pp->conv && pp->M > 0 && pp->N > 0 && pp->Hin > 0 && pp->Win > 0 && pp->scatter == 0 &&
+        !(pp->flags & (LB_GEMM_C64 | LB_GEMM_GN_A))) {
+        const LbGemmParams& p = *pp;
+        if (g_halo != 0 && !g_force_tile && lb_conv3x3_narrow_eligible(p)) {
+            k = 8;
+            f = lb_conv_halo_gn_a_mode() != 0;
+        } else if (use_halo(p) && lb_conv3x3_halo_gn_a_able(p)) {
+            k = 3;
+            f = lb_conv3x3_halo_gn_a_policy(p);
+        }
+    }
+    if (fuse) *fuse = f;
+    if (kind) *kind = k;
+}
+
 extern "C" int lb_gemm_f16(const LbGemmParams* pp, void* stream) {
     LbGemmParams p = *pp;
     const bool geglu = (p.flags & LB_GEMM_GEGLU) != 0;
@@ -499,6 +519,7 @@
     if (p.alpha == 0.f) p.alpha = 1.f;
     p.reserved2_ = (g_lb_wide_store & 1) | (g_lb_lean_epilogue ? 2 : 0);
     if (p.flags & LB_GEMM_C64) {
+        LB_REQUIRE(!(p.flags & LB_GEMM_GN_A), "lb_gemm_f16: LB_GEMM_GN_A is implemented by the whole-tile 3x3 halo conv and the narrow-N conv only");
         if (const int rc = lb_conv3_c64_check(p)) return rc;
         LB_DISPATCH("conv3x3_c64", lb_conv3_c64_launch(p, s));
     }
@@ -515,6 +536,8 @@
         if (const int rc = lb_conv3x3_halo_check(p)) return rc;
         LB_DISPATCH("lb_conv3x3_halo_f16", lb_conv3x3_halo_launch(p, s));
     }
+    LB_REQUIRE(!(p.flags & LB_GEMM_GN_A), "lb_gemm_f16: LB_GEMM_GN_A is implemented by the whole-tile 3x3 halo conv and the narrow-N conv only "
+                                          "(ask lb_conv_halo_gn_a_plan before flagging a conv)");
     if (p.flags & LB_GEMM_HALO_KSPLIT) {
         p.flags &= ~LB_GEMM_HALO_KSPLIT;
         p.partial = nullptr;
diff --git a/latentblending_amd/csrc/lb_common.h b/latentblending_amd/csrc/lb_common.h
--- a/latentblending_amd/csrc/lb_common.h
+++ b/latentblending_amd/csrc/lb_common.h
@@ -114,6 +114,17 @@
     return x * __builtin_amdgcn_rcpf(1.0f + __builtin_amdgcn_exp2f(x * -1.44269504088896340736f));
 }
 
+__device__ __forceinline__ void lb_gn_affine(float rstd, float mean, float gamma, float beta, float& sc, float& sh) {
+    const float a = rstd * gamma;
+    sc = a;
+    sh = beta - mean * a;
+}
+__device__ __forceinline__ f16 lb_gn_apply(float x, float sc, float sh, int silu) {
+    float t = __builtin_fmaf(x, sc, sh);
+    if (silu) t = lb_silu(t);
+    return (f16)t;
+}
+
 __device__ __forceinline__ float lb_erf(float x) {
     const float ax = __builtin_fabsf(x);
     const float t = __builtin_amdgcn_rcpf(__builtin_fmaf(0.3275911f, ax, 1.0f));
diff --git a/latentblending_amd/csrc/norm.hip b/latentblending_amd/csrc/norm.hip
--- a/latentblending_amd/csrc/norm.hip
+++ b/latentblending_amd/csrc/norm.hip
@@ -138,20 +138,14 @@
 #pragma unroll
         for (int e = 0; e < 8; ++e) {
             const int grp = (c0 + e) / cpg;
-            const float a = rstd_s[grp] * gamma[c0 + e];
-            sc[e] = a;
-            sh[e] = beta[c0 + e] - mean_s[grp] * a;
+            lb_gn_affine(rstd_s[grp], mean_s[grp], gamma[c0 + e], beta[c0 + e], sc[e], sh[e]);
         }
         const T* src = x + ((long)b * HW) * ldx + c0;
         f16* dst = y + ((long)b * HW) * ldy + c0;
         auto finish = [&](const float (&val)[8], int px) {
             f16x8 o;
 #pragma unroll
-            for (int e = 0; e < 8; ++e) {
-                float t = __builtin_fmaf(val[e], sc[e], sh[e]);
-                if (silu) t = lb_silu(t);
-                o[e] = (f16)t;
-            }
+            for (int e = 0; e < 8; ++e) o[e] = lb_gn_apply(val[e], sc[e], sh[e], silu);
             *reinterpret_cast<f16x8*>(dst + (long)px * ldy) = o;
         };
         int px = px_begin + r;
@@ -440,6 +434,58 @@
                                                                      groups, eps, silu, x_is_f32, stat_rows_per_sample, s));
 }
 
+__global__ void __launch_bounds__(256) gn_affine_table_kernel(const float2* __restrict__ ch_stats, const float* __restrict__ gamma,
+                                                              const float* __restrict__ beta, float2* __restrict__ table, int HW, int C,
+                                                              int groups, float eps, int rows_per_sample, long total_rows) {
+    __shared__ double red_s[256], red_q[256];
+    __shared__ float stat[2];
+    const int grp = blockIdx.x, b = blockIdx.y, tid = threadIdx.x;
+    const int cpg = C / groups;
+    double s = 0, q = 0;
+    for (int c = 0; c < cpg; ++c) {
+        const float2* run = ch_stats + (long)(grp * cpg + c) * total_rows + (long)b * rows_per_sample;
+        for (int r = tid; r < rows_per_sample; r += 256) {
+            const float2 v = run[r];
+            s += (double)v.x;
+            q += (double)v.y;
+        }
+    }
+    red_s[tid] = s;
+    red_q[tid] = q;
+    __syncthreads();
+    for (int w = 128; w > 0; w >>= 1) {
+        if (tid < w) { red_s[tid] += red_s[tid + w]; red_q[tid] += red_q[tid + w]; }
+        __syncthreads();
+    }
+    if (tid == 0) {
+        const double fs = 0.0 + red_s[0], fq = 0.0 + red_q[0];
+        const double cnt = (double)HW * cpg;
+        const double mean = fs / cnt;
+        double var = fq / cnt - mean * mean;
+        if (var < 0) var = 0;
+        stat[0] = (float)mean;
+        stat[1] = (float)(1.0 / sqrt(var + (double)eps));
+    }
+    __syncthreads();
+    for (int c = tid; c < cpg; c += 256) {
+        const int ch = grp * cpg + c;
+        float2 t;
+        lb_gn_affine(stat[1], stat[0], gamma[ch], beta[ch], t.x, t.y);
+        table[(long)b * C + ch] = t;
+    }
+}
+
+extern "C" int lb_groupnorm_affine_from_stats(const float* ch_stats, const float* gamma, const float* beta, float* table, int B,
+                                              int HW, int C, int groups, float eps, int stat_rows_per_sample, void* stream) {
+    LB_REQUIRE(B > 0 && HW > 0 && C > 0 && stat_rows_per_sample > 0 && ch_stats != nullptr && table != nullptr,
+               "lb_groupnorm_affine_from_stats: sizes");
+    LB_REQUIRE(C % 8 == 0 && C <= 4096, "lb_groupnorm_affine_from_stats: C multiple of 8, C <= 4096");
+    LB_REQUIRE(groups > 0 && groups <= GN_MAX_GROUPS && C % groups == 0, "lb_groupnorm_affine_from_stats: groups");
+    LB_DISPATCH_STMT("lb_groupnorm_affine_from_stats",
+                     hipLaunchKernelGGL(gn_affine_table_kernel, dim3(groups, B), dim3(256), 0, s, (const float2*)ch_stats, gamma, beta,
+                                        (float2*)table, HW, C, groups, eps, stat_rows_per_sample, (long)B * stat_rows_per_sample));
+}
+
 __global__ void __launch_bounds__(256) layernorm_kernel(const f16* __restrict__ x,
                                                         const float* __restrict__ gamma,
                                                         const float* __restrict__ beta,
diff --git a/latentblending_amd/hip/lib.py b/latentblending_amd/hip/lib.py
--- a/latentblending_amd/hip/lib.py
+++ b/latentblending_amd/hip/lib.py
@@ -25,6 +25,7 @@
         ("splitk", C.c_int), ("zero_page", C.c_void_p),
         ("scatter", C.c_int), ("sc_py", C.c_int), ("sc_px", C.c_int), ("reserved_", C.c_int),
         ("ln_colsum", C.c_void_p), ("ln_eps", C.c_float), ("reserved2_", C.c_int), ("ch_stats", C.c_void_p), ("ch_stats_rows", C.c_int),
+        ("gn_table", C.c_void_p), ("gn_silu", C.c_int),
     ]
 
 
@@ -41,6 +42,7 @@
 GEMM_QUICK_GELU, GEMM_GELU, GEMM_CH_STATS = 128, 256, 512
 GEMM_HALO_RAGGED = 1024
 GEMM_HALO_KSPLIT = 4096
+GEMM_GN_A = 8192
 GEMM_C64 = 2048
 
 _vp, _i, _l, _f, _d = C.c_void_p, C.c_int, C.c_long, C.c_float, C.c_double
@@ -136,6 +138,12 @@
     "lb_conv_halo_set_ksplit": (None, [_i, _i]),
 }
 
+GN_A_SIGNATURES = {
+    "lb_groupnorm_affine_from_stats": (_i, [_vp, _vp, _vp, _vp, _i, _i, _i, _i, _f, _i, _vp]),
+    "lb_conv_halo_gn_a_plan": (None, [C.POINTER(LbGemmParams), C.POINTER(C.c_int), C.POINTER(C.c_int)]),
+    "lb_conv_halo_set_gn_a": (None, [_i, _i]),
+}
+
 _NO_CHECK = {"lb_version", "lb_last_error_string", "lb_gemm_workspace_bytes", "lb_jpeg_coefficient_count", "lb_jpeg_workspace_bytes",
              "lb_groupnorm_workspace_bytes", "lb_groupnorm_set_l3_chunk", "lb_conv_halo_set_persistent", "lb_conv_halo_plan","lb_gemm_ch_stat_rows", "lb_conv_halo_set_study", "lb_gemm_set_tuning", "lb_gemm_set_depth", "lb_gemm_set_variant", "lb_gemm_set_wide_store", "lb_gemm_set_lean_epilogue", "lb_gemm_set_t192_waves8", "lb_gemm_set_kgroups", "lb_gemm_pp_set_group", "lb_gemm_set_pp_auto", "lb_gemm_set_policy", "lb_gemm_set_halo", "lb_attn_set_tuning", "lb_layernorm_set_form", "lb_groupnorm_set_fused", "lb_groupnorm_plan", "lb_slerp_set_study", "lb_program_create",
              "lb_program_destroy", "lb_program_recording", "lb_program_num_ops", "lb_program_op_name"}
@@ -179,6 +187,11 @@
     _fn.restype = _res
     _fn.argtypes = _args
     setattr(api, _name, _fn)
+for _name, (_res, _args) in GN_A_SIGNATURES.items():
+    _fn = getattr(_lib, _name)
+    _fn.restype = _res
+    _fn.argtypes = _args
+    setattr(api, _name, _wrap(_name, _fn) if _res is _i else _fn)
 for _name, (_res, _args) in STUDY_SIGNATURES.items():
     _fn = getattr(_lib, _name, None)
     if _fn is not None:
diff --git a/latentblending_amd/hip/ops.py b/latentblending_amd/hip/ops.py
--- a/latentblending_amd/hip/ops.py
+++ b/latentblending_amd/hip/ops.py
@@ -341,6 +341,15 @@
     return y
 
 
+def groupnorm_affine_from_stats(gamma: torch.Tensor, beta: torch.Tensor, groups: int, eps: float, ch_stats: torch.Tensor,
+                                rows_per_sample: int, B: int, HW: int, out: Optional[torch.Tensor] = None) -> torch.Tensor:
+    C_ = gamma.numel()
+    table = torch.empty(B, C_, 2, dtype=F32, device=gamma.device) if out is None else out
+    api.lb_groupnorm_affine_from_stats(ch_stats.data_ptr(), gamma.data_ptr(), beta.data_ptr(), table.data_ptr(), B, HW, C_, groups,
+                                       eps, rows_per_sample, stream_ptr())
+    return table
+
+
 def layernorm(x: torch.Tensor, gamma: torch.Tensor, beta: torch.Tensor, eps: float = 1e-5) -> torch.Tensor:
     M, Cc = x.shape
     y = torch.empty_like(x)
diff --git a/latentblending_amd/native/runtime.py b/latentblending_amd/native/runtime.py
--- a/latentblending_amd/native/runtime.py
+++ b/latentblending_amd/native/runtime.py
@@ -114,6 +114,14 @@
     return None if t is None else t.data_ptr()
 
 
+class GnOperand:
+
+    def __init__(self, x: torch.Tensor, args: dict):
+        self.x, self.args = x, args
+        self.table: Optional[torch.Tensor] = None
+        self.scratch: Optional[torch.Tensor] = None
+
+
 class Emitter:
 
     def __init__(self, arena: Arena):
@@ -129,6 +137,7 @@
         self.ragged_halo = False
         self.halo_ksplit = True
         self.ws_ksplit: Optional[torch.Tensor] = None
+        self.gn_a = True
 
     def _ragged_flag(self, p: LbGemmParams) -> int:
         if not self.ragged_halo or not p.conv or p.KH != 3 or p.KW != 3 or p.stride != 1 or p.scatter or p.ups or p.N <= 16:
@@ -184,6 +193,15 @@
         p.partial = self.ws_ksplit.data_ptr() + self._KSPLIT_COUNTER_BYTES - counters
         return True
 
+    def _gn_a_fuse(self, p: LbGemmParams, x: torch.Tensor, gn: dict) -> bool:
+        if not self.gn_a or gn.get("ch_stats") is None or x.dtype != F16 or not p.conv:
+            return False
+        if p.Cin != int(gn["C_"]) or p.ldx != p.Cin or gn.get("ldx") not in (None, p.Cin):
+            return False
+        fuse, kind = C.c_int(), C.c_int()
+        api.lb_conv_halo_gn_a_plan(C.byref(p), C.byref(fuse), C.byref(kind))
+        return bool(fuse.value)
+
     def _gn_ws(self, B: int, groups: int) -> torch.Tensor:
         need = api.lb_groupnorm_workspace_bytes(B, groups) // 8
         if self.ws_gn is None or self.ws_gn.numel() < need:
@@ -196,7 +214,48 @@
              residual=None, rowvec=None, rows_per_batch: int = 0, flags: int = 0, alpha: float = 1.0,
              lda: Optional[int] = None, ldc: Optional[int] = None, ldr: Optional[int] = None,
              ld_rowvec: Optional[int] = None, conv: Optional[dict] = None, splitk: bool = True,
-             ln: Optional[Tuple[torch.Tensor, float]] = None, ch_stats: Optional[torch.Tensor] = None):
+             ln: Optional[Tuple[torch.Tensor, float]] = None, ch_stats: Optional[torch.Tensor] = None,
+             gn: Optional["GnOperand"] = None):
+        p = self._gemm_params(A, W, out, M=M, bias=bias, residual=residual, rowvec=rowvec, rows_per_batch=rows_per_batch, flags=flags,
+                              alpha=alpha, lda=lda, ldc=ldc, ldr=ldr, ld_rowvec=ld_rowvec, conv=conv, splitk=splitk, ln=ln,
+                              ch_stats=ch_stats)
+        N, K = W.shape
+        n_out = N // 2 if flags & lib.GEMM_GEGLU else N
+        if gn is not None:
+            if gn.table is not None:
+                if not self._gn_a_fuse(p, gn.x, gn.args):
+                    raise RuntimeError("Emitter.gemm: the conv is not the one gn_operand planned the GroupNorm fold for")
+                p.flags |= lib.GEMM_GN_A
+                p.gn_table, p.gn_silu = gn.table.data_ptr(), int(bool(gn.args["silu"]))
+            else:
+                p.A = gn.scratch.data_ptr()
+        api.lb_gemm_f16(C.byref(p), _stream())
+        if gn is not None:
+            self.arena.release(gn.scratch)
+            self.arena.release(gn.table)
+            gn.scratch = gn.table = None
+        mult = 4.0 if p.scatter == 2 else 1.0
+        self.gemm_log.append({"M": M, "N": N, "K": K, "flops": mult * 2.0 * M * N * K, "conv": conv is not None,
+                              "bytes": mult * 2.0 * (N * K + M * n_out) + (2.0 * M * K if conv is None else 0.0)})
+        return out
+
+    def gn_operand(self, x: torch.Tensor, W: torch.Tensor, *, M: int, conv: dict, flags: int = 0, has_residual: bool = False,
+                   **gn) -> "GnOperand":
+        op = GnOperand(x, dict(gn))
+        plan = self._gemm_params(x, W, x, M=M, residual=x if has_residual else None, flags=flags, conv=conv)
+        if self._gn_a_fuse(plan, x, gn):
+            B_, C_, st = int(gn["B"]), int(gn["C_"]), gn["ch_stats"]
+            op.table = self.arena.alloc((B_, C_, 2), F32)
+            api.lb_groupnorm_affine_from_stats(st[0].data_ptr(), gn["gamma"].data_ptr(), gn["beta"].data_ptr(), op.table.data_ptr(),
+                                               B_, int(gn["HW"]), C_, int(gn.get("groups", 32)), float(gn["eps"]), int(st[1]),
+                                               _stream())
+        else:
+            op.scratch = self.arena.alloc(tuple(x.shape[:-1]) + (int(gn["C_"]),))
+            self.groupnorm(x, op.scratch, gn["gamma"], gn["beta"], **{k: v for k, v in gn.items() if k not in ("gamma", "beta")})
+        return op
+
+    def _gemm_params(self, A, W, out, *, M, bias=None, residual=None, rowvec=None, rows_per_batch=0, flags=0, alpha=1.0, lda=None,
+                     ldc=None, ldr=None, ld_rowvec=None, conv=None, splitk=True, ln=None, ch_stats=None) -> LbGemmParams:
         p = LbGemmParams()
         N, K = W.shape
         p.A, p.W, p.C = A.data_ptr(), W.data_ptr(), out.data_ptr()
@@ -232,11 +291,7 @@
             p.flags |= self._ragged_flag(p)
         if conv is not None:
             self._halo_ksplit(p)
-        api.lb_gemm_f16(C.byref(p), _stream())
-        mult = 4.0 if p.scatter == 2 else 1.0
-        self.gemm_log.append({"M": M, "N": N, "K": K, "flops": mult * 2.0 * M * N * K, "conv": conv is not None,
-                              "bytes": mult * 2.0 * (N * K + M * n_out) + (2.0 * M * K if conv is None else 0.0)})
-        return out
+        return p
 
     def plan(self, M: int, N: int, K: int, flags: int = 0) -> Tuple[int, int]:
         p = LbGemmParams()
diff --git a/latentblending_amd/native/vae.py b/latentblending_amd/native/vae.py
--- a/latentblending_amd/native/vae.py
+++ b/latentblending_amd/native/vae.py
@@ -145,7 +145,20 @@
         out._lb_chstats = (buf, rows)
         return buf
 
-    def _stream_conv(self, x, name, B, H, W, cin, cout, *, residual=None, out=None, stats=True):
+    def _stream_conv_args(self, name, B, H, W, cin, residual):
+        sc = self.scaled
+        cin_p = _pad(cin, 8)
+        flags = 0 if sc else (lib.GEMM_OUT_F32 | (lib.GEMM_RES_F32 if residual else 0))
+        return flags, dict(Hin=H, Win=W, Cin=cin_p, Hout=H, Wout=W, KH=3, KW=3, stride=1, pad=1, ups=0, ldx=cin_p)
+
+    def _gn_for_conv(self, x, norm, silu, name, B, H, W, cin, *, residual=False):
+        flags, conv = self._stream_conv_args(name, B, H, W, cin, residual)
+        op = self.em.gn_operand(x, self.net.w[name + ".weight"], M=B * H * W, conv=conv, flags=flags, has_residual=residual,
+                                **self._gn_args(x, norm, B, H * W, cin, silu))
+        self._gn_done(x)
+        return op
+
+    def _stream_conv(self, x, name, B, H, W, cin, cout, *, residual=None, out=None, stats=True, gn=None):
         w, sc = self.net.w, self.scaled
         cin_p, cout_p = _pad(cin, 8), _pad(cout, 4)
         if out is None:
@@ -154,8 +167,21 @@
         st = self._stats_for(out, B, H, W, cin_p, cout_p) if stats else None
         self.em.gemm(x, w[name + ".weight"], out, M=B * H * W, bias=w[name + (".bias_s" if sc else ".bias")],
                      residual=residual, flags=flags, alpha=STREAM_SCALE if sc else 1.0, ch_stats=st,
-                     conv=dict(Hin=H, Win=W, Cin=cin_p, Hout=H, Wout=W, KH=3, KW=3, stride=1, pad=1, ups=0, ldx=cin_p))
+                     conv=dict(Hin=H, Win=W, Cin=cin_p, Hout=H, Wout=W, KH=3, KW=3, stride=1, pad=1, ups=0, ldx=cin_p),
+                     gn=gn)
         return out
+
+    def _gn_args(self, x, name, B, HW, c, silu):
+        w = self.net.w
+        eps = 1e-6 * (STREAM_SCALE * STREAM_SCALE if self.scaled else 1.0)
+        return dict(gamma=w[name + ".weight"], beta=w[name + ".bias"], B=B, HW=HW, C_=c, eps=eps, silu=silu,
+                    groups=self.net.cfg.norm_groups, ch_stats=getattr(x, "_lb_chstats", None))
+
+    def _gn_done(self, x):
+        st = getattr(x, "_lb_chstats", None)
+        if st is not None:
+            self.arena.release(st[0])
+            x._lb_chstats = None
 
     def _gn(self, x, out, name, B, HW, c, silu):
         w = self.net.w
@@ -176,13 +202,9 @@
 
     def _resnet(self, x, p, B, H, W, cin, cout):
         em, w, ar, sc = self.em, self.net.w, self.arena, self.scaled
-        n1 = ar.alloc((B, H, W, cin))
-        self._gn(x, n1, p + ".norm1", B, H * W, cin, True)
-        h = self._stream_conv(n1, p + ".conv1", B, H, W, cin, cout)
-        ar.release(n1)
-        n2 = ar.alloc((B, H, W, cout))
-        self._gn(h, n2, p + ".norm2", B, H * W, cout, True)
-        ar.release(h)
+        g1 = self._gn_for_conv(x, p + ".norm1", True, p + ".conv1", B, H, W, cin)
+        h = self._stream_conv(x, p + ".conv1", B, H, W, cin, cout, gn=g1)
+        g2 = self._gn_for_conv(h, p + ".norm2", True, p + ".conv2", B, H, W, cout, residual=True)
         if cin != cout:
             x16, owned = self._stream_as_operand(x, B, H, W, cin)
             xs = ar.alloc((B, H, W, cout), F16 if sc else F32)
@@ -193,8 +215,8 @@
                 ar.release(x16)
         else:
             xs = x
-        out = self._stream_conv(n2, p + ".conv2", B, H, W, cout, cout, residual=xs)
-        ar.release(n2)
+        out = self._stream_conv(h, p + ".conv2", B, H, W, cout, cout, residual=xs, gn=g2)
+        ar.release(h)
         if xs is not x:
             ar.release(xs)
         return out
@@ -283,14 +305,14 @@
                 ar.release(h)
                 h = up
                 sh, sw = 2 * sh, 2 * sw
-        n = ar.alloc((B, sh, sw, rev[-1]))
-        self._gn(h, n, "decoder.conv_norm_out", B, sh * sw, rev[-1], True)
+        cin_p = _pad(rev[-1], 8)
+        conv_out = dict(Hin=sh, Win=sw, Cin=cin_p, Hout=sh, Wout=sw, KH=3, KW=3, stride=1, pad=1, ups=0, ldx=cin_p)
+        g = em.gn_operand(h, w["decoder.conv_out.weight"], M=B * sh * sw, conv=conv_out, flags=lib.GEMM_OUT_F32,
+                          **self._gn_args(h, "decoder.conv_norm_out", B, sh * sw, rev[-1], True))
+        self._gn_done(h)
+        em.gemm(h, w["decoder.conv_out.weight"], self.image_f32, M=B * sh * sw, bias=w["decoder.conv_out.bias"],
+                flags=lib.GEMM_OUT_F32, conv=conv_out, gn=g)
         ar.release(h)
-        cin_p = _pad(rev[-1], 8)
-        em.gemm(n, w["decoder.conv_out.weight"], self.image_f32, M=B * sh * sw, bias=w["decoder.conv_out.bias"],
-                flags=lib.GEMM_OUT_F32,
-                conv=dict(Hin=sh, Win=sw, Cin=cin_p, Hout=sh, Wout=sw, KH=3, KW=3, stride=1, pad=1, ups=0, ldx=cin_p))
-        ar.release(n)
         api.lb_postprocess_u8(self.image_f32.data_ptr(), self.frames.data_ptr(), B * sh * sw,
                               _pad(cfg.out_channels, 4), 1, _stream())
 
```
